# GrumpyZhou/patch2pix

Measured on NVIDIA H100. Metric: image-pairs/sec, higher is better.
Workload: dtype f16 tensor-core operands (mid: 3-pass hi/lo split on the risk band, 1-pass elsewhere, fine: 1-pass, correlation + NC conv: 3-pass), f32 accumulate

## Files before the change

### include/p2p_b200.h

```cpp
#ifndef P2P_B200_H_
#define P2P_B200_H_

#include <stdint.h>

#ifdef __cplusplus
extern "C" {
#endif

#define P2P_API __attribute__((visibility("default")))

typedef struct p2p_handle_s* p2p_handle_t;

typedef struct p2p_bn_s {
  const float* weight;
  const float* bias;
  const float* running_mean;
  const float* running_var;
} p2p_bn_t;

typedef struct p2p_regressor_weights_s {
  const float* conv0_weight;
  p2p_bn_t conv1_bn;
  const float* conv2_weight;
  p2p_bn_t conv3_bn;
  const float* fc0_weight;
  const float* fc0_bias;
  p2p_bn_t fc1_bn;
  const float* fc3_weight;
  const float* fc3_bias;
  p2p_bn_t fc4_bn;
  const float* fc6_weight;
  const float* fc6_bias;
  float bn_eps;
} p2p_regressor_weights_t;

P2P_API const char* p2p_last_error(void);
P2P_API int p2p_version(void);

P2P_API int p2p_create(int device, p2p_handle_t* out);
P2P_API int p2p_destroy(p2p_handle_t h);

P2P_API int p2p_set_ncn_weights(p2p_handle_t h, const float* w1, const float* b1, const float* w2, const float* b2);

P2P_API int p2p_set_regressor_weights(p2p_handle_t h, int which, const p2p_regressor_weights_t* w);

P2P_API int p2p_set_option(p2p_handle_t h, const char* key, int value);
P2P_API int p2p_get_option(p2p_handle_t h, const char* key, int* value);
P2P_API int p2p_launch_count(p2p_handle_t h, long long* count);

enum {
  P2P_PROF_L2NORM = 0, P2P_PROF_CORR = 1, P2P_PROF_MUTUAL = 2, P2P_PROF_NC = 3, P2P_PROF_PROPOSALS = 4,
  P2P_PROF_PREP = 5, P2P_PROF_GATHER_MID = 6, P2P_PROF_CONV1_MID = 7, P2P_PROF_CONV2_MID = 8, P2P_PROF_FC_MID = 9,
  P2P_PROF_GATHER_FINE = 10, P2P_PROF_CONV1_FINE = 11, P2P_PROF_CONV2_FINE = 12, P2P_PROF_FC_FINE = 13,
  P2P_PROF_GATHER_BAND = 14, P2P_PROF_CONV1_BAND = 15, P2P_PROF_CONV2_BAND = 16, P2P_PROF_FC_BAND = 17,
  P2P_PROF_FLAG = 18, P2P_PROF_KINDS = 19
};
P2P_API int p2p_profile_read(p2p_handle_t h, float* ms_by_kind, int* count_by_kind, int nkinds);

P2P_API int p2p_coarse(p2p_handle_t h, const float* feat1, const float* feat2, int c, int h1, int w1, int h2, int w2,
               int ksize, float* corr4d_out, uint8_t* delta_code_out, float* pooled_out, float* ncn_out,
               void* stream);

P2P_API int p2p_coarse_nhwc16(p2p_handle_t h, const void* feat1_nhwc16, const void* feat2_nhwc16, int c, int h1, int w1, int h2,
               int w2, int ksize, float* corr4d_out, uint8_t* delta_code_out, float* pooled_out, float* ncn_out,
               void* stream);

P2P_API int p2p_delta_unpack(p2p_handle_t h, const uint8_t* code, long long n, int ksize, int64_t* di, int64_t* dj,
                     int64_t* dk, int64_t* dl, void* stream);
P2P_API int p2p_delta_pack(p2p_handle_t h, const int64_t* di, const int64_t* dj, const int64_t* dk, const int64_t* dl,
                   long long n, int ksize, uint8_t* code, void* stream);

P2P_API int p2p_mutual_matching(p2p_handle_t h, const float* in, int nA, int nB, float* out, void* stream);
P2P_API int p2p_neigh_consensus(p2p_handle_t h, const float* in, int hA, int wA, int hB, int wB, float* out, void* stream);

P2P_API int p2p_proposals(p2p_handle_t h, const float* corr4d, const uint8_t* delta_code, int hA, int wA, int hB, int wB,
                  int ksize, int upsample, int center, int do_softmax, int64_t* matches_out, float* scores_out,
                  void* stream);

P2P_API int p2p_unique_rows(p2p_handle_t h, const int64_t* rows, int n, int mutual, const float* scores, float thres,
                    int32_t* ids_out, int32_t* count_out, void* stream);

P2P_API int p2p_select_anchor(p2p_handle_t h, const int64_t* rows, const float* scores, const int32_t* ids,
                      const int32_t* sel, int m, int panc, int pshift, int64_t* matches_out, float* scores_out,
                      int64_t* anchors_out, void* stream);

P2P_API int p2p_refine_prepare(p2p_handle_t h, const float* const* feats1, const float* const* feats2, int H1, int W1,
                       int H2, int W2, void* stream);
P2P_API int p2p_refine_prepare_nhwc16(p2p_handle_t h, const void* const* feats1, const void* const* feats2, int H1, int W1,
                       int H2, int W2, void* stream);
P2P_API int p2p_refine(p2p_handle_t h, int which, const void* matches_in, int is_float, int n, float* matches_out,
               float* probs_out, void* stream);

P2P_API int p2p_finalize_matches(p2p_handle_t h, const float* fine, const float* scores, const int64_t* coarse, int n,
                         float io_thres, const double* upscale4, double* packed_out, void* stream);

P2P_API int p2p_preprocess_image(p2p_handle_t h, const uint8_t* rgb_hwc, int ho, int wo, int ht, int wt, float* out_chw,
                         uint8_t* resized_hwc_out, void* stream);

P2P_API int p2p_find_model(p2p_handle_t h, int model, const double* rows, int row_stride, int n, const double* n_dev,
                   double px_th, double conf, int max_iters, unsigned long long seed, double* model_out, uint8_t* mask_out,
                   int32_t* n_inliers_out, void* stream);
P2P_API int p2p_sampson_distance(p2p_handle_t h, const double* rows, int row_stride, int n, const double* F,
                         double* dist_out, void* stream);
P2P_API int p2p_epipolar_histograms(p2p_handle_t h, const double* rows, int row_stride, int n, const double* n_dev,
                                    int coarse_col, const double* F, const uint8_t* mask, const double* edges,
                                    int n_edges, int32_t* counts_out, void* stream);
P2P_API int p2p_overlap_scores(p2p_handle_t h, const int64_t* point3D_ids, const int64_t* offsets,
                               const int64_t* offsets_host, int n_images, int words, uint32_t* bits_out,
                               int32_t* counts_out, double* scores_out, void* stream);
P2P_API int p2p_test_hypotheses(p2p_handle_t h, int model, const double* rows, int row_stride, int n, double px_th,
                        unsigned long long seed, int count, double* models_out, int32_t* counts_out, void* stream);
P2P_API int p2p_test_degeneracy(p2p_handle_t h, const double* rows, int row_stride, int n, double px_th,
                                unsigned long long seed, int count, int32_t* triplet_out, double* H_out, void* stream);

P2P_API int p2p_find_essential(p2p_handle_t h, const double* rows, int row_stride, int n, const double* n_dev,
                               const double* intr, double px_th, double conf, int max_iters, unsigned long long seed,
                               double* E_out, uint8_t* mask_out, int32_t* n_inliers_out, void* stream);
P2P_API int p2p_recover_pose(p2p_handle_t h, const double* rows, int row_stride, int n, const double* n_dev,
                             const double* intr, const double* E, const uint8_t* mask_in, double dist_th,
                             double* Rt_out, uint8_t* mask_out, int32_t* n_good_out, void* stream);
P2P_API int p2p_test_essential_hypotheses(p2p_handle_t h, const double* rows, int row_stride, int n, const double* intr,
                                          double px_th, unsigned long long seed, int count, double* models_out,
                                          int32_t* counts_out, void* stream);

P2P_API int p2p_find_model_batch(p2p_handle_t h, int model, const double* rows, int row_stride, const int64_t* offsets,
                                 const int64_t* offsets_host, int K, const double* n_dev, double px_th, double conf,
                                 int max_iters, unsigned long long seed, double* models_out, uint8_t* mask_out,
                                 int32_t* n_inliers_out, void* stream);
P2P_API int p2p_find_essential_batch(p2p_handle_t h, const double* rows, int row_stride, const int64_t* offsets,
                                     const int64_t* offsets_host, int K, const double* n_dev, const double* intr,
                                     double px_th, double conf, int max_iters, unsigned long long seed, double* E_out,
                                     uint8_t* mask_out, int32_t* n_inliers_out, void* stream);
P2P_API int p2p_recover_pose_batch(p2p_handle_t h, const double* rows, int row_stride, const int64_t* offsets,
                                   const int64_t* offsets_host, int K, const double* n_dev, const double* intr,
                                   const double* E, const uint8_t* mask_in, double dist_th, double* Rt_out,
                                   uint8_t* mask_out, int32_t* n_good_out, void* stream);
P2P_API int p2p_batch_chunk_pairs(p2p_handle_t h, int entry, int* pairs_out);

P2P_API int p2p_test_gemm(p2p_handle_t h, const float* a, const float* b, float* c, int M, int N, int K, int passes,
                  int seg_len, float in_scale, void* stream);

#ifdef __cplusplus
}
#endif
#endif
```

### patch2pix_b200/_lib.py

```python
import ctypes as C
import os

import torch

_HERE = os.path.dirname(os.path.abspath(__file__))
LIB_PATH = os.path.join(_HERE, 'libp2p_b200.so')
_lib = None


class BN(C.Structure):
    _fields_ = [('weight', C.c_void_p), ('bias', C.c_void_p), ('running_mean', C.c_void_p), ('running_var', C.c_void_p)]


class RegressorWeights(C.Structure):
    _fields_ = [('conv0_weight', C.c_void_p), ('conv1_bn', BN), ('conv2_weight', C.c_void_p), ('conv3_bn', BN),
                ('fc0_weight', C.c_void_p), ('fc0_bias', C.c_void_p), ('fc1_bn', BN),
                ('fc3_weight', C.c_void_p), ('fc3_bias', C.c_void_p), ('fc4_bn', BN),
                ('fc6_weight', C.c_void_p), ('fc6_bias', C.c_void_p), ('bn_eps', C.c_float)]


_P, _I, _LL, _F = C.c_void_p, C.c_int, C.c_longlong, C.c_float
_SIGNATURES = {
    'p2p_last_error': (C.c_char_p, []),
    'p2p_version': (_I, []),
    'p2p_create': (_I, [_I, C.POINTER(_P)]),
    'p2p_destroy': (_I, [_P]),
    'p2p_set_ncn_weights': (_I, [_P, _P, _P, _P, _P]),
    'p2p_set_regressor_weights': (_I, [_P, _I, C.POINTER(RegressorWeights)]),
    'p2p_set_option': (_I, [_P, C.c_char_p, _I]),
    'p2p_get_option': (_I, [_P, C.c_char_p, C.POINTER(_I)]),
    'p2p_launch_count': (_I, [_P, C.POINTER(_LL)]),
    'p2p_coarse': (_I, [_P, _P, _P, _I, _I, _I, _I, _I, _I, _P, _P, _P, _P, _P]),
    'p2p_coarse_nhwc16': (_I, [_P, _P, _P, _I, _I, _I, _I, _I, _I, _P, _P, _P, _P, _P]),
    'p2p_delta_unpack': (_I, [_P, _P, _LL, _I, _P, _P, _P, _P, _P]),
    'p2p_delta_pack': (_I, [_P, _P, _P, _P, _P, _LL, _I, _P, _P]),
    'p2p_mutual_matching': (_I, [_P, _P, _I, _I, _P, _P]),
    'p2p_neigh_consensus': (_I, [_P, _P, _I, _I, _I, _I, _P, _P]),
    'p2p_proposals': (_I, [_P, _P, _P, _I, _I, _I, _I, _I, _I, _I, _I, _P, _P, _P]),
    'p2p_unique_rows': (_I, [_P, _P, _I, _I, _P, _F, _P, _P, _P]),
    'p2p_select_anchor': (_I, [_P, _P, _P, _P, _P, _I, _I, _I, _P, _P, _P, _P]),
    'p2p_refine_prepare': (_I, [_P, C.POINTER(_P), C.POINTER(_P), _I, _I, _I, _I, _P]),
    'p2p_refine_prepare_nhwc16': (_I, [_P, C.POINTER(_P), C.POINTER(_P), _I, _I, _I, _I, _P]),
    'p2p_refine': (_I, [_P, _I, _P, _I, _I, _P, _P, _P]),
    'p2p_finalize_matches': (_I, [_P, _P, _P, _P, _I, _F, C.POINTER(C.c_double), _P, _P]),
    'p2p_preprocess_image': (_I, [_P, _P, _I, _I, _I, _I, _P, _P, _P]),
    'p2p_profile_read': (_I, [_P, C.POINTER(C.c_float), C.POINTER(_I), _I]),
    'p2p_test_gemm': (_I, [_P, _P, _P, _P, _I, _I, _I, _I, _I, _F, _P]),
    'p2p_find_model': (_I, [_P, _I, _P, _I, _I, _P, C.c_double, C.c_double, _I, C.c_ulonglong, _P, _P, _P, _P]),
    'p2p_sampson_distance': (_I, [_P, _P, _I, _I, _P, _P, _P]),
    'p2p_epipolar_histograms': (_I, [_P, _P, _I, _I, _P, _I, C.POINTER(C.c_double), _P, C.POINTER(C.c_double), _I, _P,
                                     _P]),
    'p2p_overlap_scores': (_I, [_P, _P, _P, C.POINTER(C.c_int64), _I, _I, _P, _P, _P, _P]),
    'p2p_test_hypotheses': (_I, [_P, _I, _P, _I, _I, C.c_double, C.c_ulonglong, _I, _P, _P, _P]),
    'p2p_test_degeneracy': (_I, [_P, _P, _I, _I, C.c_double, C.c_ulonglong, _I, _P, _P, _P]),
    'p2p_find_essential': (_I, [_P, _P, _I, _I, _P, _P, C.c_double, C.c_double, _I, C.c_ulonglong, _P, _P, _P, _P]),
    'p2p_recover_pose': (_I, [_P, _P, _I, _I, _P, _P, _P, _P, C.c_double, _P, _P, _P, _P]),
    'p2p_test_essential_hypotheses': (_I, [_P, _P, _I, _I, _P, C.c_double, C.c_ulonglong, _I, _P, _P, _P]),
    'p2p_find_model_batch': (_I, [_P, _I, _P, _I, _P, C.POINTER(C.c_int64), _I, _P, C.c_double, C.c_double, _I,
                                  C.c_ulonglong, _P, _P, _P, _P]),
    'p2p_find_essential_batch': (_I, [_P, _P, _I, _P, C.POINTER(C.c_int64), _I, _P, _P, C.c_double, C.c_double, _I,
                                      C.c_ulonglong, _P, _P, _P, _P]),
    'p2p_recover_pose_batch': (_I, [_P, _P, _I, _P, C.POINTER(C.c_int64), _I, _P, _P, _P, _P, C.c_double, _P, _P, _P,
                                    _P]),
    'p2p_batch_chunk_pairs': (_I, [_P, _I, C.POINTER(_I)]),
}
EXPORTED_SYMBOLS = tuple(_SIGNATURES)
PROF_KINDS = ('l2norm', 'corr', 'mutual', 'nc', 'proposals', 'prep', 'gather_mid', 'conv1_mid', 'conv2_mid', 'fc_mid',
              'gather_fine', 'conv1_fine', 'conv2_fine', 'fc_fine', 'gather_band', 'conv1_band', 'conv2_band', 'fc_band',
              'flag')


def load():
    global _lib
    if _lib is None:
        if not os.path.exists(LIB_PATH):
            raise RuntimeError(f'{LIB_PATH} not found: the CUDA extension is required (no CPU fallback). '
                               f'Build it with `python -m patch2pix_b200.build`.')
        lib = C.CDLL(LIB_PATH)
        for name, (res, args) in _SIGNATURES.items():
            fn = getattr(lib, name)
            fn.restype = res
            fn.argtypes = args
        _lib = lib
    return _lib


def check(rc):
    if rc != 0:
        msg = load().p2p_last_error()
        raise RuntimeError(f'libp2p_b200 error {rc}: {msg.decode() if msg else "?"}')


def ptr(t):
    return None if t is None else C.c_void_p(t.data_ptr())


def stream_ptr(device):
    return C.c_void_p(torch.cuda.current_stream(device).cuda_stream)


class Handle:

    def __init__(self, device):
        device = torch.device(device)
        if device.type != 'cuda':
            raise RuntimeError('patch2pix_b200 runs on CUDA (sm_90a) devices only; got device ' + str(device))
        self.device = torch.device('cuda', device.index if device.index is not None else torch.cuda.current_device())
        self.lib = load()
        h = C.c_void_p()
        check(self.lib.p2p_create(self.device.index, C.byref(h)))
        self.h = h
        for kv in filter(None, os.environ.get('P2P_OPTIONS', '').split(',')):
            k, _, v = kv.partition('=')
            self.set_option(k.strip(), int(v))

    def __del__(self):
        try:
            if getattr(self, 'h', None):
                self.lib.p2p_destroy(self.h)
                self.h = None
        except Exception:
            pass

    def set_option(self, key, value):
        check(self.lib.p2p_set_option(self.h, key.encode(), int(value)))

    def get_option(self, key):
        v = C.c_int()
        check(self.lib.p2p_get_option(self.h, key.encode(), C.byref(v)))
        return v.value

    def launch_count(self):
        v = C.c_longlong()
        check(self.lib.p2p_launch_count(self.h, C.byref(v)))
        return v.value

    def stream(self):
        return stream_ptr(self.device)

    def profile_read(self):
        n = len(PROF_KINDS)
        ms = (C.c_float * n)()
        cnt = (C.c_int * n)()
        check(self.lib.p2p_profile_read(self.h, ms, cnt, n))
        return {PROF_KINDS[i]: (ms[i], cnt[i]) for i in range(n)}


_default_handles = {}


def default_handle(device):
    device = torch.device(device)
    idx = device.index if device.index is not None else torch.cuda.current_device()
    if idx not in _default_handles:
        _default_handles[idx] = Handle(torch.device('cuda', idx))
    return _default_handles[idx]
```

### patch2pix_b200/csrc/api.cu

```cuda
#include <math.h>
#include <stdlib.h>

#include <algorithm>
#include <vector>

#include "../../include/p2p_b200.h"
#include "kernels.h"
#include "umma_gemm.h"

namespace p2p {

static thread_local std::string g_last_error;
void set_last_error(const std::string& msg) { g_last_error = msg; }
long long g_launch_count = 0;

int ensure_dyn_smem(const void* kernel, int bytes) {
  struct Key { const void* k; int dev; };
  static thread_local std::vector<std::pair<Key, int>> granted;
  int dev = 0;
  cudaGetDevice(&dev);
  for (auto& g : granted)
    if (g.first.k == kernel && g.first.dev == dev) {
      if (g.second >= bytes) return 0;
      if (cudaFuncSetAttribute(kernel, cudaFuncAttributeMaxDynamicSharedMemorySize, bytes) != cudaSuccess) {
        set_last_error(std::string("cudaFuncSetAttribute(MaxDynamicSharedMemorySize) failed: ") + cudaGetErrorString(cudaGetLastError()));
        return -2;
      }
      g.second = bytes;
      return 0;
    }
  if (cudaFuncSetAttribute(kernel, cudaFuncAttributeMaxDynamicSharedMemorySize, bytes) != cudaSuccess) {
    set_last_error(std::string("cudaFuncSetAttribute(MaxDynamicSharedMemorySize) failed: ") + cudaGetErrorString(cudaGetLastError()));
    return -2;
  }
  granted.push_back({Key{kernel, dev}, bytes});
  return 0;
}

int Arena::reserve(size_t bytes) {
  off = 0;
  if (bytes <= cap) return 0;
  if (base != nullptr) {
    cudaDeviceSynchronize();
    cudaFree(base);
    base = nullptr;
    cap = 0;
  }
  bytes = align_up(bytes + (bytes >> 3), 1 << 20);
  if (cudaMalloc(&base, bytes) != cudaSuccess) {
    cudaGetLastError();
    set_last_error("out of device memory reserving " + std::to_string(bytes >> 20) + " MiB of scratch");
    return -3;
  }
  cap = bytes;
  return 0;
}
void Arena::release() {
  if (base != nullptr) cudaFree(base);
  base = nullptr;
  cap = off = 0;
}

struct Regressor {
  bool set = false;
  __half *w1_hi = nullptr, *w1_lo = nullptr;
  __half *w2_hi = nullptr, *w2_lo = nullptr;
  float *scale1 = nullptr, *bias1 = nullptr, *scale2 = nullptr, *bias2 = nullptr;
  float y_scale = 1.f;
  FcWeights fc = {nullptr, nullptr, nullptr, nullptr, nullptr, nullptr};
  __half *f1_hi = nullptr, *f1_lo = nullptr, *f2_hi = nullptr, *f2_lo = nullptr;
  float *fa1 = nullptr, *fa2 = nullptr;
  KStep steps1[kConv1Steps];
  KStep steps2[kConv2Steps];
  KStep *d_steps1 = nullptr, *d_steps2 = nullptr;
  char* blob = nullptr;
};

}

using namespace p2p;

struct p2p_handle_s {
  int device = 0;
  int num_sms = 132;
  int opt_mid_passes = 3, opt_fine_passes = 1, opt_corr_passes = 3, opt_seg_len = 3, opt_gemm_impl = 0, opt_num_sms = 0;
  int opt_mid_band = 26;
  int opt_fc_impl = 1;
  int opt_fuse_gather = 3;
  int opt_share_windows = 1;
  const int* last_band_count = nullptr;
  int* share_rows = nullptr;
  bool last_mid_shared = false;
  unsigned long long* band_totals = nullptr;
  bool nc_set = false;
  float *nc_w1p = nullptr, *nc_b1p = nullptr, *nc_w2p = nullptr;
  float nc_b2 = 0.f;
  NcUmmaWeights ncw;
  void* dbg_nc[4] = {nullptr, nullptr, nullptr, nullptr};
  int opt_unique_impl = 1;
  int* uniq_rank = nullptr;
  int opt_nc_l2_mode = 0;
  int opt_nc_impl = 1;
  Regressor reg[2];
  Arena coarse, refine, feat, misc, uniq, pre, verify;
  std::vector<PreprocessCoefs> pre_coefs;
  PairFeatures pf[2];
  bool prepared = false;
  int opt_profile = 0;
  struct ProfEntry { cudaEvent_t a, b; int kind; };
  std::vector<ProfEntry> prof;
  std::vector<cudaEvent_t> event_pool;
};

namespace {

struct DeviceGuard {
  int prev = -1;
  bool ok = true;
  explicit DeviceGuard(int dev) {
    if (cudaGetDevice(&prev) != cudaSuccess) ok = false;
    if (ok && prev != dev && cudaSetDevice(dev) != cudaSuccess) ok = false;
  }
  ~DeviceGuard() {
    if (prev >= 0) cudaSetDevice(prev);
  }
};

#define P2P_ENTER(h)                                                  \
  P2P_REQUIRE((h) != nullptr, "null handle");                         \
  DeviceGuard _guard((h)->device);                                    \
  if (!_guard.ok) {                                                   \
    set_last_error("cannot select CUDA device of the handle");        \
    return -2;                                                        \
  }

float pow2_floor_scale(float maxabs, float target_hi) {
  if (!(maxabs > 0.f) || !isfinite(maxabs)) return 1.f;
  int e;
  frexpf(maxabs, &e);
  int et;
  frexpf(target_hi, &et);
  return ldexpf(1.f, et - 1 - e);
}

void split_half(float v, __half& hi, __half& lo) {
  hi = __float2half_rn(v);
  lo = __float2half_rn(v - __half2float(hi));
}

template <typename T>
T* carve(char*& p, size_t count) {
  T* r = reinterpret_cast<T*>(p);
  p += align_up(count * sizeof(T), 256);
  return r;
}

void fold_bn(const p2p_bn_t& bn, int n, float eps, std::vector<float>& g, std::vector<float>& b) {
  g.resize(n);
  b.resize(n);
  for (int i = 0; i < n; ++i) {
    g[i] = bn.weight[i] / sqrtf(bn.running_var[i] + eps);
    b[i] = bn.bias[i] - bn.running_mean[i] * g[i];
  }
}

int tap_plane(int t, int& start) {
  if (t == 0) { start = -1; return 0; }
  if (t == 1) { start = 0; return 1; }
  start = 0;
  return 0;
}

int pack_regressor(p2p_handle_s* h, Regressor& R, const p2p_regressor_weights_t& w) {
  const int K1 = kConv1Steps * 64, K2 = kConv2Steps * 64;
  std::vector<float> g1, b1, g2, b2, gf1, bf1, gf2, bf2;
  fold_bn(w.conv1_bn, 512, w.bn_eps, g1, b1);
  fold_bn(w.conv3_bn, 512, w.bn_eps, g2, b2);
  fold_bn(w.fc1_bn, 512, w.bn_eps, gf1, bf1);
  fold_bn(w.fc4_bn, 256, w.bn_eps, gf2, bf2);

  std::vector<__half> w1h((size_t)512 * K1), w1l((size_t)512 * K1), w2h((size_t)512 * K2), w2l((size_t)512 * K2);
  std::vector<float> sc1(512), sc2(512), bi1(b1), bi2(b2);
  float max_bound = 0.f;
  std::vector<float> sw1(512), sw2(512);
  for (int o = 0; o < 512; ++o) {
    const float* wo = w.conv0_weight + (size_t)o * 518 * 9;
    float m = 0.f;
    double tapn[9] = {0};
    for (int c = 0; c < 518; ++c)
      for (int t = 0; t < 9; ++t) {
        const float v = wo[c * 9 + t] * g1[o];
        m = fmaxf(m, fabsf(v));
        tapn[t] += (double)v * v;
      }
    float bound = fabsf(b1[o]);
    for (int t = 0; t < 9; ++t) bound += 1.41421357f * (float)sqrt(tapn[t]);
    max_bound = fmaxf(max_bound, bound);
    sw1[o] = pow2_floor_scale(m, 1024.f);
    sc1[o] = 1.f / (kActScale * sw1[o]);
    __half* dh = w1h.data() + (size_t)o * K1;
    __half* dl = w1l.data() + (size_t)o * K1;
    for (int s = 0; s < 72; ++s) {
      const int tap = s / 8, chunk = s % 8;
      for (int kk = 0; kk < 64; ++kk) {
        const int c512 = chunk * 64 + kk;
        const int orig = (c512 / 256) * 259 + 3 + (c512 % 256);
        split_half(wo[orig * 9 + tap] * g1[o] * sw1[o], dh[s * 64 + kk], dl[s * 64 + kk]);
      }
    }
    for (int kk = 0; kk < 64; ++kk) {
      float v = 0.f;
      if (kk < 54) {
        const int tap = kk / 6, r = kk % 6;
        const int orig = (r / 3) * 259 + (r % 3);
        v = wo[orig * 9 + tap] * g1[o] * sw1[o];
      }
      split_half(v, dh[72 * 64 + kk], dl[72 * 64 + kk]);
    }
  }
  R.y_scale = pow2_floor_scale(max_bound, 32768.f);
  for (int o = 0; o < 512; ++o) {
    const float* wo = w.conv2_weight + (size_t)o * 512 * 9;
    float m = 0.f;
    for (int i = 0; i < 512 * 9; ++i) m = fmaxf(m, fabsf(wo[i] * g2[o]));
    sw2[o] = pow2_floor_scale(m, 1024.f);
    sc2[o] = 1.f / (R.y_scale * sw2[o]);
    __half* dh = w2h.data() + (size_t)o * K2;
    __half* dl = w2l.data() + (size_t)o * K2;
    for (int s = 0; s < 72; ++s) {
      const int tap = s / 8, chunk = s % 8;
      for (int kk = 0; kk < 64; ++kk)
        split_half(wo[(chunk * 64 + kk) * 9 + tap] * g2[o] * sw2[o], dh[s * 64 + kk], dl[s * 64 + kk]);
    }
  }
  for (int s = 0; s < 72; ++s) {
    const int tap = s / 8, chunk = s % 8, ty = tap / 3, tx = tap % 3;
    int sx, sy;
    const int px = tap_plane(tx, sx), py = tap_plane(ty, sy);
    R.steps1[s] = KStep{(short)(chunk * 64), (signed char)sx, (signed char)sy, (signed char)(py * 2 + px), 0, 0, s * 64};
    R.steps2[s] = KStep{(short)(chunk * 64), (signed char)(tx - 1), (signed char)(ty - 1), 0, 0, 0, s * 64};
  }
  R.steps1[72] = KStep{0, 0, 0, 0, 1, 0, 72 * 64};
  std::vector<float> f1t((size_t)512 * 512), f1b(512), f2t((size_t)512 * 256), f2b(256), f3t(256 * 5), f3b(5);
  for (int o = 0; o < 512; ++o) {
    for (int k = 0; k < 512; ++k) f1t[(size_t)k * 512 + o] = w.fc0_weight[(size_t)o * 512 + k] * gf1[o];
    f1b[o] = w.fc0_bias[o] * gf1[o] + bf1[o];
  }
  for (int o = 0; o < 256; ++o) {
    for (int k = 0; k < 512; ++k) f2t[(size_t)k * 256 + o] = w.fc3_weight[(size_t)o * 512 + k] * gf2[o];
    f2b[o] = w.fc3_bias[o] * gf2[o] + bf2[o];
  }
  for (int o = 0; o < 5; ++o) {
    for (int k = 0; k < 256; ++k) f3t[k * 5 + o] = w.fc6_weight[o * 256 + k];
    f3b[o] = w.fc6_bias[o];
  }
  std::vector<__half> f1h((size_t)512 * 512), f1l((size_t)512 * 512), f2h((size_t)256 * 512), f2l((size_t)256 * 512);
  std::vector<float> fa1(512), fa2(256);
  for (int o = 0; o < 512; ++o) {
    float m = 0.f;
    for (int k = 0; k < 512; ++k) m = fmaxf(m, fabsf(w.fc0_weight[(size_t)o * 512 + k] * gf1[o]));
    const float sw = pow2_floor_scale(m, 1024.f);
    fa1[o] = 1.f / (kFcActScale * sw);
    for (int k = 0; k < 512; ++k)
      split_half(w.fc0_weight[(size_t)o * 512 + k] * gf1[o] * sw, f1h[(size_t)o * 512 + k], f1l[(size_t)o * 512 + k]);
  }
  for (int o = 0; o < 256; ++o) {
    float m = 0.f;
    for (int k = 0; k < 512; ++k) m = fmaxf(m, fabsf(w.fc3_weight[(size_t)o * 512 + k] * gf2[o]));
    const float sw = pow2_floor_scale(m, 1024.f);
    fa2[o] = 1.f / (kFcActScale * sw);
    for (int k = 0; k < 512; ++k)
      split_half(w.fc3_weight[(size_t)o * 512 + k] * gf2[o] * sw, f2h[(size_t)o * 512 + k], f2l[(size_t)o * 512 + k]);
  }
  const size_t total = 2 * 1024 * 1024 + 65536 + 4 * align_up((size_t)512 * K1 * 2, 256) + 8 * 4096 + align_up(f1t.size() * 4, 256) +
                       align_up(f2t.size() * 4, 256) + 8 * 8192 + 65536;
  if (R.blob == nullptr) {
    if (cudaMalloc(&R.blob, total) != cudaSuccess) {
      cudaGetLastError();
      set_last_error("out of device memory packing regressor weights");
      return -3;
    }
  }
  char* p = R.blob;
  R.w1_hi = carve<__half>(p, (size_t)512 * K1);
  R.w1_lo = carve<__half>(p, (size_t)512 * K1);
  R.w2_hi = carve<__half>(p, (size_t)512 * K2);
  R.w2_lo = carve<__half>(p, (size_t)512 * K2);
  R.scale1 = carve<float>(p, 512);
  R.bias1 = carve<float>(p, 512);
  R.scale2 = carve<float>(p, 512);
  R.bias2 = carve<float>(p, 512);
  R.fc.w1t = carve<float>(p, f1t.size());
  R.fc.b1 = carve<float>(p, 512);
  R.fc.w2t = carve<float>(p, f2t.size());
  R.fc.b2 = carve<float>(p, 256);
  R.fc.w3t = carve<float>(p, f3t.size());
  R.fc.b3 = carve<float>(p, 5);
  R.d_steps1 = carve<KStep>(p, kConv1Steps);
  R.d_steps2 = carve<KStep>(p, kConv2Steps);
  R.f1_hi = carve<__half>(p, f1h.size());
  R.f1_lo = carve<__half>(p, f1l.size());
  R.f2_hi = carve<__half>(p, f2h.size());
  R.f2_lo = carve<__half>(p, f2l.size());
  R.fa1 = carve<float>(p, 512);
  R.fa2 = carve<float>(p, 256);
#define UP(dst, src, bytes) P2P_CUDA_OK(cudaMemcpy(dst, src, bytes, cudaMemcpyHostToDevice))
  UP(R.w1_hi, w1h.data(), w1h.size() * 2);
  UP(R.w1_lo, w1l.data(), w1l.size() * 2);
  UP(R.w2_hi, w2h.data(), w2h.size() * 2);
  UP(R.w2_lo, w2l.data(), w2l.size() * 2);
  UP(R.scale1, sc1.data(), 2048);
  UP(R.bias1, bi1.data(), 2048);
  UP(R.scale2, sc2.data(), 2048);
  UP(R.bias2, bi2.data(), 2048);
  UP(R.fc.w1t, f1t.data(), f1t.size() * 4);
  UP(R.fc.b1, f1b.data(), 2048);
  UP(R.fc.w2t, f2t.data(), f2t.size() * 4);
  UP(R.fc.b2, f2b.data(), 1024);
  UP(R.fc.w3t, f3t.data(), f3t.size() * 4);
  UP(R.fc.b3, f3b.data(), 20);
  UP(R.d_steps1, R.steps1, sizeof(R.steps1));
  UP(R.d_steps2, R.steps2, sizeof(R.steps2));
  UP(R.f1_hi, f1h.data(), f1h.size() * 2);
  UP(R.f1_lo, f1l.data(), f1l.size() * 2);
  UP(R.f2_hi, f2h.data(), f2h.size() * 2);
  UP(R.f2_lo, f2l.data(), f2l.size() * 2);
  UP(R.fa1, fa1.data(), 2048);
  UP(R.fa2, fa2.data(), 1024);
#undef UP
  R.set = true;
  (void)h;
  return 0;
}

int sms(const p2p_handle_s* h) { return h->opt_num_sms > 0 ? h->opt_num_sms : h->num_sms; }

struct ProfScope {
  p2p_handle_s* h;
  cudaStream_t st;
  cudaEvent_t a = nullptr, b = nullptr;
  int kind;
  static cudaEvent_t get(p2p_handle_s* h) {
    if (!h->event_pool.empty()) {
      cudaEvent_t e = h->event_pool.back();
      h->event_pool.pop_back();
      return e;
    }
    cudaEvent_t e = nullptr;
    cudaEventCreate(&e);
    return e;
  }
  ProfScope(p2p_handle_s* h_, int kind_, cudaStream_t st_) : h(h_), st(st_), kind(kind_) {
    if (h->opt_profile) {
      a = get(h);
      b = get(h);
      cudaEventRecord(a, st);
    }
  }
  ~ProfScope() {
    if (a != nullptr) {
      cudaEventRecord(b, st);
      h->prof.push_back({a, b, kind});
    }
  }
};

}

extern "C" {

const char* p2p_last_error(void) { return g_last_error.c_str(); }
int p2p_version(void) { return 100; }

int p2p_create(int device, p2p_handle_t* out) {
  P2P_REQUIRE(out != nullptr, "out is null");
  int ndev = 0;
  P2P_CUDA_OK(cudaGetDeviceCount(&ndev));
  P2P_REQUIRE(device >= 0 && device < ndev, "device index out of range");
  cudaDeviceProp prop;
  P2P_CUDA_OK(cudaGetDeviceProperties(&prop, device));
  if (prop.major != 9 || prop.minor != 0) {
    set_last_error(std::string("libp2p_b200 targets sm_90a (H100) only; device is sm_") + std::to_string(prop.major) +
                   std::to_string(prop.minor));
    return -2;
  }
  p2p_handle_s* h = new p2p_handle_s();
  h->device = device;
  h->num_sms = prop.multiProcessorCount;
  {
    DeviceGuard g(device);
    if (cudaMalloc(&h->band_totals, 2 * sizeof(unsigned long long)) == cudaSuccess)
      cudaMemset(h->band_totals, 0, 2 * sizeof(unsigned long long));
    else
      h->band_totals = nullptr;
    if (cudaMalloc(&h->share_rows, sizeof(int)) == cudaSuccess)
      cudaMemset(h->share_rows, 0, sizeof(int));
    else
      h->share_rows = nullptr;
  }
  *out = h;
  return 0;
}

int p2p_destroy(p2p_handle_t h) {
  if (h == nullptr) return 0;
  DeviceGuard g(h->device);
  cudaDeviceSynchronize();
  h->coarse.release();
  h->refine.release();
  h->feat.release();
  h->misc.release();
  h->uniq.release();
  h->pre.release();
  h->verify.release();
  for (auto& c : h->pre_coefs)
    if (c.d) cudaFree(c.d);
  for (auto& e : h->prof) { cudaEventDestroy(e.a); cudaEventDestroy(e.b); }
  for (auto e : h->event_pool) cudaEventDestroy(e);
  if (h->nc_w1p) cudaFree(h->nc_w1p);
  if (h->ncw.blob) cudaFree(h->ncw.blob);
  if (h->band_totals) cudaFree(h->band_totals);
  if (h->share_rows) cudaFree(h->share_rows);
  if (h->uniq_rank) cudaFree(h->uniq_rank);
  for (int i = 0; i < 2; ++i)
    if (h->reg[i].blob) cudaFree(h->reg[i].blob);
  delete h;
  return 0;
}

int p2p_set_ncn_weights(p2p_handle_t h, const float* w1, const float* b1, const float* w2, const float* b2) {
  P2P_ENTER(h);
  P2P_REQUIRE(w1 && b1 && w2 && b2, "null weight pointer");
  std::vector<float> w1p(81 * 32), b1p(32), w2p(81 * 32);
  for (int a = 0; a < 3; ++a)
    for (int b = 0; b < 3; ++b)
      for (int d = 0; d < 3; ++d)
        for (int e = 0; e < 3; ++e) {
          const int tap = ((a * 3 + b) * 3 + d) * 3 + e;
          for (int c = 0; c < 16; ++c) {
            w1p[tap * 32 + c] = w1[((a * 16 + c) * 1 + 0) * 27 + (b * 3 + d) * 3 + e];
            w1p[tap * 32 + 16 + c] = w1[((d * 16 + c) * 1 + 0) * 27 + (e * 3 + a) * 3 + b];
            w2p[tap * 32 + c] = w2[((a * 1 + 0) * 16 + c) * 27 + (b * 3 + d) * 3 + e];
            w2p[tap * 32 + 16 + c] = w2[((d * 1 + 0) * 16 + c) * 27 + (e * 3 + a) * 3 + b];
          }
        }
  for (int c = 0; c < 16; ++c) b1p[c] = b1p[16 + c] = b1[c];
  if (h->nc_w1p == nullptr) P2P_CUDA_OK(cudaMalloc(&h->nc_w1p, sizeof(float) * (81 * 32 * 2 + 32)));
  h->nc_w2p = h->nc_w1p + 81 * 32;
  h->nc_b1p = h->nc_w2p + 81 * 32;
  P2P_CUDA_OK(cudaMemcpy(h->nc_w1p, w1p.data(), sizeof(float) * 81 * 32, cudaMemcpyHostToDevice));
  P2P_CUDA_OK(cudaMemcpy(h->nc_w2p, w2p.data(), sizeof(float) * 81 * 32, cudaMemcpyHostToDevice));
  P2P_CUDA_OK(cudaMemcpy(h->nc_b1p, b1p.data(), sizeof(float) * 32, cudaMemcpyHostToDevice));
  h->nc_b2 = b2[0];
  {
    int rc = nc_umma_pack(w1p.data(), b1p.data(), w2p.data(), h->ncw);
    if (rc) return rc;
  }
  h->nc_set = true;
  return 0;
}

int p2p_set_regressor_weights(p2p_handle_t h, int which, const p2p_regressor_weights_t* w) {
  P2P_ENTER(h);
  P2P_REQUIRE(which == 0 || which == 1, "which must be 0 (mid) or 1 (fine)");
  P2P_REQUIRE(w != nullptr && w->conv0_weight && w->conv2_weight && w->fc0_weight && w->fc3_weight && w->fc6_weight,
              "null weight pointer");
  return pack_regressor(h, h->reg[which], *w);
}

static int* option_slot(p2p_handle_t h, const char* key) {
  if (!strcmp(key, "mid_passes")) return &h->opt_mid_passes;
  if (!strcmp(key, "fine_passes")) return &h->opt_fine_passes;
  if (!strcmp(key, "corr_passes")) return &h->opt_corr_passes;
  if (!strcmp(key, "seg_len")) return &h->opt_seg_len;
  if (!strcmp(key, "gemm_impl")) return &h->opt_gemm_impl;
  if (!strcmp(key, "num_sms")) return &h->opt_num_sms;
  if (!strcmp(key, "profile")) return &h->opt_profile;
  if (!strcmp(key, "mid_band")) return &h->opt_mid_band;
  if (!strcmp(key, "fuse_gather")) return &h->opt_fuse_gather;
  if (!strcmp(key, "share_windows")) return &h->opt_share_windows;
  if (!strcmp(key, "fc_impl")) return &h->opt_fc_impl;
  if (!strcmp(key, "nc_impl")) return &h->opt_nc_impl;
  if (!strcmp(key, "nc_l2_mode")) return &h->opt_nc_l2_mode;
  if (!strcmp(key, "unique_impl")) return &h->opt_unique_impl;
  return nullptr;
}

int p2p_set_option(p2p_handle_t h, const char* key, int value) {
  P2P_REQUIRE(h != nullptr && key != nullptr, "null argument");
  int* s = option_slot(h, key);
  P2P_REQUIRE(s != nullptr, std::string("unknown option ") + key);
  if (s == &h->opt_mid_passes || s == &h->opt_fine_passes) P2P_REQUIRE(value == 1 || value == 3, "passes must be 1 or 3");
  if (s == &h->opt_corr_passes) P2P_REQUIRE(value == 0 || value == 1 || value == 3, "corr_passes must be 0, 1 or 3");
  if (s == &h->opt_share_windows) P2P_REQUIRE(value == 0 || value == 1, "share_windows must be 0 or 1");
  P2P_REQUIRE(value >= 0, "option values are non-negative");
  *s = value;
  return 0;
}

int p2p_get_option(p2p_handle_t h, const char* key, int* value) {
  P2P_REQUIRE(h != nullptr && key != nullptr && value != nullptr, "null argument");
  if (!strcmp(key, "band_rows")) {
    *value = 0;
    if (h->last_band_count != nullptr) {
      DeviceGuard g(h->device);
      P2P_CUDA_OK(cudaDeviceSynchronize());
      P2P_CUDA_OK(cudaMemcpy(value, h->last_band_count, sizeof(int), cudaMemcpyDeviceToHost));
    }
    return 0;
  }
  if (!strcmp(key, "shared_rows")) {
    *value = 0;
    if (h->last_mid_shared && h->share_rows != nullptr) {
      DeviceGuard g(h->device);
      P2P_CUDA_OK(cudaDeviceSynchronize());
      P2P_CUDA_OK(cudaMemcpy(value, h->share_rows, sizeof(int), cudaMemcpyDeviceToHost));
    }
    return 0;
  }
  if (!strcmp(key, "band_rows_total") || !strcmp(key, "band_calls_rows_total")) {
    *value = 0;
    if (h->band_totals != nullptr) {
      DeviceGuard g(h->device);
      P2P_CUDA_OK(cudaDeviceSynchronize());
      unsigned long long t[2] = {0, 0};
      P2P_CUDA_OK(cudaMemcpy(t, h->band_totals, sizeof(t), cudaMemcpyDeviceToHost));
      const bool rows = !strcmp(key, "band_calls_rows_total");
      *value = (int)(rows ? t[1] : t[0]);
      if (rows) P2P_CUDA_OK(cudaMemset(h->band_totals, 0, sizeof(t)));
    }
    return 0;
  }
  int* s = option_slot(h, key);
  P2P_REQUIRE(s != nullptr, std::string("unknown option ") + key);
  *value = *s;
  return 0;
}

int p2p_launch_count(p2p_handle_t h, long long* count) {
  P2P_REQUIRE(h != nullptr && count != nullptr, "null argument");
  *count = g_launch_count;
  return 0;
}

int p2p_profile_read(p2p_handle_t h, float* ms_by_kind, int* count_by_kind, int nkinds) {
  P2P_ENTER(h);
  P2P_REQUIRE(ms_by_kind && count_by_kind && nkinds >= P2P_PROF_KINDS, "need room for P2P_PROF_KINDS entries");
  for (int i = 0; i < nkinds; ++i) {
    ms_by_kind[i] = 0.f;
    count_by_kind[i] = 0;
  }
  for (auto& e : h->prof) {
    P2P_CUDA_OK(cudaEventSynchronize(e.b));
    float ms = 0.f;
    P2P_CUDA_OK(cudaEventElapsedTime(&ms, e.a, e.b));
    ms_by_kind[e.kind] += ms;
    count_by_kind[e.kind] += 1;
    h->event_pool.push_back(e.a);
    h->event_pool.push_back(e.b);
  }
  h->prof.clear();
  return 0;
}

static int corr_umma(p2p_handle_s* h, const __half* a_hi, const __half* a_lo, const __half* b_hi, const __half* b_lo,
                     int C, int n1, int n2, int n1pad, int n2pad, int ksize, float* out, uint8_t* code,
                     cudaStream_t st) {
  UmmaGemmParams p;
  memset(&p, 0, sizeof(p));
  const uint64_t ad[5] = {(uint64_t)C, 1, 1, 1, (uint64_t)n1pad};
  const uint64_t as[4] = {(uint64_t)C * 2, (uint64_t)C * 2, (uint64_t)C * 2, (uint64_t)C * 2};
  const uint32_t ab[5] = {64, 1, 1, 1, 128};
  const uint64_t bd[2] = {(uint64_t)C, (uint64_t)n2pad};
  const uint64_t bs[1] = {(uint64_t)C * 2};
  const uint32_t bb[2] = {64, 128};
  int rc;
  if ((rc = make_tmap_fp16(&p.a_main_hi, a_hi, 5, ad, as, ab))) return rc;
  if ((rc = make_tmap_fp16(&p.b_hi, b_hi, 2, bd, bs, bb))) return rc;
  if (h->opt_corr_passes == 3) {
    if ((rc = make_tmap_fp16(&p.a_main_lo, a_lo, 5, ad, as, ab))) return rc;
    if ((rc = make_tmap_fp16(&p.b_lo, b_lo, 2, bd, bs, bb))) return rc;
  }
  p.a_rgb_hi = p.a_main_hi;
  p.a_rgb_lo = p.a_main_hi;
  p.nsteps = C / 64;
  for (int s = 0; s < p.nsteps; ++s) p.steps[s] = KStep{(short)(s * 64), 0, 0, 0, 0, 0, s * 64};
  p.m_tiles = n1pad / 128;
  p.n_tiles = n2pad / 256;
  p.a_units_per_tile = 128;
  p.seg_len = h->opt_seg_len > 0 ? 1 : 0;
  p.epi.c = out;
  p.epi.alpha = 1.f / (kActScale * kActScale);
  if (ksize == 2) {
    p.epi.code = code;
    p.epi.np1 = n1 / 4;
    p.epi.np2 = n2 / 4;
    return launch_umma_gemm(p, EPI_CORR, h->opt_corr_passes, sms(h), st);
  }
  p.epi.ldc = n2;
  p.epi.m_rows = n1;
  p.epi.n_cols = n2;
  return launch_umma_gemm(p, EPI_PLAIN, h->opt_corr_passes, sms(h), st);
}

static int coarse_impl(p2p_handle_t h, const float* feat1, const float* feat2, int fmt, int c, int h1, int w1, int h2, int w2,
                       int ksize, float* corr4d_out, uint8_t* delta_code_out, float* pooled_out, float* ncn_out,
                       void* stream) {
  P2P_ENTER(h);
  cudaStream_t st = reinterpret_cast<cudaStream_t>(stream);
  P2P_REQUIRE(h->nc_set, "p2p_set_ncn_weights has not been called");
  P2P_REQUIRE(feat1 && feat2 && corr4d_out, "null tensor pointer");
  P2P_REQUIRE(ksize == 1 || ksize == 2, "ksize must be 1 or 2");
  P2P_REQUIRE(c > 0 && h1 > 0 && w1 > 0 && h2 > 0 && w2 > 0, "empty feature map");
  if (ksize == 2) {
    P2P_REQUIRE(h1 % 2 == 0 && w1 % 2 == 0 && h2 % 2 == 0 && w2 % 2 == 0, "ksize 2 needs even feature sizes");
    P2P_REQUIRE(delta_code_out != nullptr, "delta_code_out is required for ksize 2");
  }
  const int n1 = h1 * w1, n2 = h2 * w2;
  const int hA = h1 / ksize, wA = w1 / ksize, hB = h2 / ksize, wB = w2 / ksize;
  const int nA = hA * wA, nB = hB * wB;
  const size_t V = (size_t)nA * nB;
  const bool tc = h->opt_corr_passes > 0;
  if (tc) P2P_REQUIRE(c % 64 == 0 && c / 64 <= kMaxKSteps, "tensor-core correlation needs C % 64 == 0");
  P2P_REQUIRE(fmt == 0 || tc, "channels-last fp16 features need the tensor-core correlation (corr_passes 1 or 3)");
  const int n1pad = (int)align_up(n1, 128), n2pad = (int)align_up(n2, 256);
  size_t need = 4 * V * 4 + nc_umma_scratch_bytes(V) + nc_umma_xp_bytes(hA, wA, hB, wB) + (size_t)(nA + nB) * 8 + (1 << 16);
  need += tc ? (size_t)(n1pad + n2pad) * c * 4 : (size_t)(n1 + n2) * c * 4;
  int rc = h->coarse.reserve(need);
  if (rc) return rc;
  Arena& A = h->coarse;
  float* pooled = pooled_out ? pooled_out : (float*)A.take(V * 4);
  float* m1 = (float*)A.take(V * 4);
  float* nc = ncn_out ? ncn_out : (float*)A.take(V * 4);
  float* hidden = (float*)A.take(V * 128);
  float* partial = (float*)A.take(18 * V * 4);
  uint32_t* xp = (uint32_t*)A.take(nc_umma_xp_bytes(hA, wA, hB, wB));
  float* rowmax = (float*)A.take((size_t)nA * 4);
  unsigned int* colmax = (unsigned int*)A.take((size_t)nB * 4 + 16);
  unsigned int* xmax = colmax != nullptr ? colmax + nB : nullptr;
  if (tc) {
    __half* a_hi = (__half*)A.take((size_t)n1pad * c * 2);
    __half* a_lo = (__half*)A.take((size_t)n1pad * c * 2);
    __half* b_hi = (__half*)A.take((size_t)n2pad * c * 2);
    __half* b_lo = (__half*)A.take((size_t)n2pad * c * 2);
    P2P_REQUIRE(a_hi && a_lo && b_hi && b_lo && hidden && colmax, "scratch carve failed");
    const bool lo = h->opt_corr_passes == 3;
    {
      ProfScope ps(h, P2P_PROF_L2NORM, st);
      if (fmt == 1)
        rc = launch_l2norm_perm_kmajor_pair_nhwc16(reinterpret_cast<const __half*>(feat1), reinterpret_cast<const __half*>(feat2),
                                                   a_hi, lo ? a_lo : nullptr, b_hi, lo ? b_lo : nullptr, c, h1, w1, h2, w2, ksize, st);
      else
        rc = launch_l2norm_perm_kmajor_pair(feat1, feat2, a_hi, lo ? a_lo : nullptr, b_hi, lo ? b_lo : nullptr, c, h1, w1, h2,
                                            w2, ksize, st);
      if (rc) return rc;
    }
    ProfScope ps(h, P2P_PROF_CORR, st);
    if ((rc = corr_umma(h, a_hi, a_lo, b_hi, b_lo, c, n1, n2, n1pad, n2pad, ksize, pooled, delta_code_out, st)))
      return rc;
  } else {
    float* fa = (float*)A.take((size_t)n1 * c * 4);
    float* fb = (float*)A.take((size_t)n2 * c * 4);
    P2P_REQUIRE(fa && fb && hidden && colmax, "scratch carve failed");
    {
      ProfScope ps(h, P2P_PROF_L2NORM, st);
      if ((rc = launch_l2norm_perm(feat1, fa, c, h1, w1, ksize, st))) return rc;
      if ((rc = launch_l2norm_perm(feat2, fb, c, h2, w2, ksize, st))) return rc;
    }
    ProfScope ps(h, P2P_PROF_CORR, st);
    if ((rc = launch_corr_pool_simt(fa, fb, c, n1, n2, ksize, pooled, delta_code_out, st))) return rc;
  }
  P2P_REQUIRE(partial != nullptr && xmax != nullptr && xp != nullptr, "scratch carve failed");
  if (h->opt_nc_impl == 1) {
    {
      ProfScope ps(h, P2P_PROF_MUTUAL, st);
      if ((rc = launch_mutual_matching(pooled, nA, nB, rowmax, colmax, m1, xmax, st))) return rc;
    }
    {
      ProfScope ps(h, P2P_PROF_NC, st);
      if ((rc = launch_neigh_consensus_umma(m1, hA, wA, hB, wB, h->ncw, h->nc_b1p, h->nc_b2, xmax, xp, (__half*)hidden, partial,
                                            nc, rowmax, colmax, h->opt_nc_l2_mode, sms(h), st)))
        return rc;
    }
    ProfScope ps(h, P2P_PROF_MUTUAL, st);
    return launch_mutual_apply(nc, nA, nB, rowmax, colmax, corr4d_out, nullptr, st);
  }
  {
    ProfScope ps(h, P2P_PROF_MUTUAL, st);
    if ((rc = launch_mutual_matching(pooled, nA, nB, rowmax, colmax, m1, nullptr, st))) return rc;
  }
  {
    ProfScope ps(h, P2P_PROF_NC, st);
    if ((rc = launch_neigh_consensus(m1, hA, wA, hB, wB, h->nc_w1p, h->nc_b1p, h->nc_w2p, h->nc_b2, hidden, nc, st)))
      return rc;
  }
  ProfScope ps(h, P2P_PROF_MUTUAL, st);
  if ((rc = launch_mutual_matching(nc, nA, nB, rowmax, colmax, corr4d_out, nullptr, st))) return rc;
  return 0;
}

int p2p_coarse(p2p_handle_t h, const float* feat1, const float* feat2, int c, int h1, int w1, int h2, int w2,
               int ksize, float* corr4d_out, uint8_t* delta_code_out, float* pooled_out, float* ncn_out,
               void* stream) {
  return coarse_impl(h, feat1, feat2, 0, c, h1, w1, h2, w2, ksize, corr4d_out, delta_code_out, pooled_out, ncn_out, stream);
}

int p2p_coarse_nhwc16(p2p_handle_t h, const void* feat1_nhwc16, const void* feat2_nhwc16, int c, int h1, int w1, int h2, int w2,
                      int ksize, float* corr4d_out, uint8_t* delta_code_out, float* pooled_out, float* ncn_out,
                      void* stream) {
  return coarse_impl(h, reinterpret_cast<const float*>(feat1_nhwc16), reinterpret_cast<const float*>(feat2_nhwc16), 1, c, h1, w1,
                     h2, w2, ksize, corr4d_out, delta_code_out, pooled_out, ncn_out, stream);
}

int p2p_delta_unpack(p2p_handle_t h, const uint8_t* code, long long n, int ksize, int64_t* di, int64_t* dj,
                     int64_t* dk, int64_t* dl, void* stream) {
  P2P_ENTER(h);
  P2P_REQUIRE(code && di && dj && dk && dl && n >= 0 && ksize >= 1 && ksize <= 3, "bad argument");
  if (n == 0) return 0;
  return launch_delta_unpack(code, (size_t)n, ksize, (long long*)di, (long long*)dj, (long long*)dk, (long long*)dl,
                             reinterpret_cast<cudaStream_t>(stream));
}

int p2p_delta_pack(p2p_handle_t h, const int64_t* di, const int64_t* dj, const int64_t* dk, const int64_t* dl,
                   long long n, int ksize, uint8_t* code, void* stream) {
  P2P_ENTER(h);
  P2P_REQUIRE(code && di && dj && dk && dl && n >= 0 && ksize >= 1 && ksize <= 3, "bad argument");
  if (n == 0) return 0;
  return launch_delta_pack((const long long*)di, (const long long*)dj, (const long long*)dk, (const long long*)dl,
                           (size_t)n, ksize, code, reinterpret_cast<cudaStream_t>(stream));
}

int p2p_mutual_matching(p2p_handle_t h, const float* in, int nA, int nB, float* out, void* stream) {
  P2P_ENTER(h);
  P2P_REQUIRE(in && out && nA > 0 && nB > 0, "bad argument");
  int rc = h->misc.reserve((size_t)(nA + nB) * 4 + 4096);
  if (rc) return rc;
  float* rowmax = (float*)h->misc.take((size_t)nA * 4);
  unsigned int* colmax = (unsigned int*)h->misc.take((size_t)nB * 4);
  return launch_mutual_matching(in, nA, nB, rowmax, colmax, out, nullptr, reinterpret_cast<cudaStream_t>(stream));
}

int p2p_neigh_consensus(p2p_handle_t h, const float* in, int hA, int wA, int hB, int wB, float* out, void* stream) {
  P2P_ENTER(h);
  P2P_REQUIRE(h->nc_set, "p2p_set_ncn_weights has not been called");
  P2P_REQUIRE(in && out && hA > 0 && wA > 0 && hB > 0 && wB > 0, "bad argument");
  const size_t V = (size_t)hA * wA * hB * wB;
  int rc = h->misc.reserve(nc_umma_scratch_bytes(V) + nc_umma_xp_bytes(hA, wA, hB, wB) + 8192);
  if (rc) return rc;
  float* hidden = (float*)h->misc.take(V * 128);
  float* partial = (float*)h->misc.take(18 * V * 4);
  uint32_t* xp = (uint32_t*)h->misc.take(nc_umma_xp_bytes(hA, wA, hB, wB));
  unsigned int* xmax = (unsigned int*)h->misc.take(16);
  P2P_REQUIRE(hidden && partial && xmax && xp, "scratch carve failed");
  h->dbg_nc[0] = hidden; h->dbg_nc[1] = partial; h->dbg_nc[2] = xp; h->dbg_nc[3] = xmax;
  cudaStream_t st = reinterpret_cast<cudaStream_t>(stream);
  if (h->opt_nc_impl == 1) {
    if ((rc = launch_absmax(in, V, xmax, st))) return rc;
    return launch_neigh_consensus_umma(in, hA, wA, hB, wB, h->ncw, h->nc_b1p, h->nc_b2, xmax, xp, (__half*)hidden, partial, out,
                                       nullptr, nullptr, h->opt_nc_l2_mode, sms(h), st);
  }
  return launch_neigh_consensus(in, hA, wA, hB, wB, h->nc_w1p, h->nc_b1p, h->nc_w2p, h->nc_b2, hidden, out, st);
}

P2P_API int p2p_debug_nc_scratch(p2p_handle_t h, int which, void* host_dst, size_t bytes) {
  P2P_ENTER(h);
  P2P_REQUIRE(which >= 0 && which < 4 && host_dst != nullptr && h->dbg_nc[which] != nullptr, "bad argument");
  P2P_CUDA_OK(cudaDeviceSynchronize());
  P2P_CUDA_OK(cudaMemcpy(host_dst, h->dbg_nc[which], bytes, cudaMemcpyDeviceToHost));
  return 0;
}

int p2p_proposals(p2p_handle_t h, const float* corr4d, const uint8_t* delta_code, int hA, int wA, int hB, int wB,
                  int ksize, int upsample, int center, int do_softmax, int64_t* matches_out, float* scores_out,
                  void* stream) {
  P2P_ENTER(h);
  P2P_REQUIRE(corr4d && matches_out && scores_out, "null tensor pointer");
  P2P_REQUIRE(hA > 0 && wA > 0 && hB > 0 && wB > 0 && ksize >= 1 && ksize <= 3 && upsample > 0, "bad dims");
  P2P_REQUIRE(ksize == 1 || delta_code != nullptr, "delta_code is required for ksize > 1");
  ProfScope ps(h, P2P_PROF_PROPOSALS, reinterpret_cast<cudaStream_t>(stream));
  return launch_proposals(corr4d, ksize > 1 ? delta_code : nullptr, hA, wA, hB, wB, ksize, upsample, center,
                          do_softmax, (long long*)matches_out, scores_out, reinterpret_cast<cudaStream_t>(stream));
}

int p2p_unique_rows(p2p_handle_t h, const int64_t* rows, int n, int mutual, const float* scores, float thres,
                    int32_t* ids_out, int32_t* count_out, void* stream) {
  P2P_ENTER(h);
  P2P_REQUIRE(rows && ids_out && count_out, "null tensor pointer");
  unsigned char* scratch = nullptr;
  const size_t sb = unique_rows_scratch_bytes(n);
  if (sb > 0) {
    int rc = h->uniq.reserve(sb + 4096);
    if (rc) return rc;
    scratch = (unsigned char*)h->uniq.take(sb);
  }
  if (h->uniq_rank == nullptr && h->opt_unique_impl == 1) {
    P2P_CUDA_OK(cudaMalloc(&h->uniq_rank, unique_rank_scratch_bytes()));
    P2P_CUDA_OK(cudaMemset(h->uniq_rank, 0, unique_rank_scratch_bytes()));
  }
  ProfScope ps(h, P2P_PROF_PROPOSALS, reinterpret_cast<cudaStream_t>(stream));
  return launch_unique_rows((const long long*)rows, n, mutual, scores, thres, ids_out, count_out, scratch,
                            h->opt_unique_impl == 1 ? h->uniq_rank : nullptr, reinterpret_cast<cudaStream_t>(stream));
}

int p2p_select_anchor(p2p_handle_t h, const int64_t* rows, const float* scores, const int32_t* ids, const int32_t* sel,
                      int m, int panc, int pshift, int64_t* matches_out, float* scores_out, int64_t* anchors_out,
                      void* stream) {
  P2P_ENTER(h);
  P2P_REQUIRE(m >= 0 && rows != nullptr, "bad argument");
  P2P_REQUIRE(panc == 1 || panc == 8, "panc must be 1 or 8 (networks/patch2pix.py:377-402)");
  P2P_REQUIRE(scores_out == nullptr || scores != nullptr, "scores_out needs scores");
  P2P_REQUIRE(panc == 1 || anchors_out != nullptr, "anchors_out is required for panc 8");
  ProfScope ps(h, P2P_PROF_PROPOSALS, reinterpret_cast<cudaStream_t>(stream));
  return launch_select_anchor((const long long*)rows, scores, ids, sel, m, panc, pshift, (long long*)matches_out,
                              scores_out, (long long*)anchors_out, reinterpret_cast<cudaStream_t>(stream));
}

static int refine_prepare_impl(p2p_handle_t h, const float* const* feats1, const float* const* feats2, int fmt, int H1, int W1,
                               int H2, int W2, void* stream) {
  P2P_ENTER(h);
  cudaStream_t st = reinterpret_cast<cudaStream_t>(stream);
  P2P_REQUIRE(feats1 && feats2, "null feature list");
  for (int l = 0; l < 4; ++l) P2P_REQUIRE(feats1[l] && feats2[l], "null feature level");
  P2P_REQUIRE(H1 >= 8 && W1 >= 8 && H2 >= 8 && W2 >= 8 && H1 % 8 == 0 && W1 % 8 == 0 && H2 % 8 == 0 && W2 % 8 == 0,
              "image sizes must be positive multiples of 8");
  const int Hs[2] = {H1, H2}, Ws[2] = {W1, W2};
  size_t need = 1 << 16;
  for (int s = 0; s < 2; ++s) {
    const size_t px = (size_t)Hs[s] * Ws[s];
    need += (px / 4 * 64 + px / 16 * 64 + px / 64 * 128) * 6 + (px + px / 4 + px / 16 + px / 64) * 4 + 32768;
  }
  const bool want_map = h->opt_fuse_gather == 3;
  if (want_map)
    for (int s = 0; s < 2; ++s) need += (size_t)(Hs[s] + 2 * kMapPad) * (Ws[s] + 2 * kMapPad) * (512 + 8) + 4096;
  int rc = h->feat.reserve(need);
  if (rc) return rc;
  const int chans[3] = {64, 64, 128};
  for (int s = 0; s < 2; ++s) {
    PairFeatures& pf = h->pf[s];
    for (int l = 0; l < 4; ++l) {
      const int ds = 1 << l;
      pf.nsq[l] = (float*)h->feat.take((size_t)(Hs[s] / ds) * (Ws[s] / ds) * 4);
      P2P_REQUIRE(pf.nsq[l] != nullptr, "scratch carve failed");
    }
    for (int l = 0; l < 3; ++l) {
      const int ds = 2 << l;
      pf.nhwc[l] = (float*)h->feat.take((size_t)(Hs[s] / ds) * (Ws[s] / ds) * chans[l] * 4);
      pf.nhwc16[l] = (__half*)h->feat.take((size_t)(Hs[s] / ds) * (Ws[s] / ds) * chans[l] * 2);
      P2P_REQUIRE(pf.nhwc[l] != nullptr && pf.nhwc16[l] != nullptr, "scratch carve failed");
    }
    pf.wmap = pf.rgbn = nullptr;
    if (want_map) {
      const size_t pxp = (size_t)(Hs[s] + 2 * kMapPad) * (Ws[s] + 2 * kMapPad);
      pf.wmap = (__half*)h->feat.take(pxp * 512);
      pf.rgbn = (__half*)h->feat.take(pxp * 8);
      P2P_REQUIRE(pf.wmap != nullptr && pf.rgbn != nullptr, "scratch carve failed");
    }
  }
  {
    ProfScope ps(h, P2P_PROF_PREP, st);
    if ((rc = launch_feature_prep_pair(feats1, feats2, Hs, Ws, h->pf, fmt, st))) return rc;
    if (want_map && (rc = launch_window_map(h->pf, st))) return rc;
  }
  h->prepared = true;
  return 0;
}

int p2p_refine_prepare(p2p_handle_t h, const float* const* feats1, const float* const* feats2, int H1, int W1,
                       int H2, int W2, void* stream) {
  return refine_prepare_impl(h, feats1, feats2, 0, H1, W1, H2, W2, stream);
}

int p2p_refine_prepare_nhwc16(p2p_handle_t h, const void* const* feats1, const void* const* feats2, int H1, int W1,
                              int H2, int W2, void* stream) {
  return refine_prepare_impl(h, reinterpret_cast<const float* const*>(feats1), reinterpret_cast<const float* const*>(feats2), 1,
                             H1, W1, H2, W2, stream);
}

namespace {

struct RefineBuffers {
  __half *p_hi, *p_lo, *r_hi, *r_lo, *y_hi, *y_lo;
  __half *q_hi, *q_lo, *h1_hi, *h1_lo, *h2_hi, *h2_lo;
  float *pooled, *raw;
  int *rowmap, *d_count;
  int *sh_prefix, *sh_cont, *sh_unsh, *sh_cnt;
  float* part;
  __half* r_unsh;
  int npad;
};

int image_steps(const Regressor& R, int si, KStep* out) {
  int k = 0;
  for (int s = 0; s < 72; ++s)
    if ((R.steps1[s].c0 >> 6) >> 2 == si) out[k++] = R.steps1[s];
  return k;
}

int run_regressor(p2p_handle_s* h, Regressor& R, int which, int passes, const RefineBuffers& B, const void* matches_in,
                  int is_float, int n, const int* rowmap, const int* d_count, float* matches_out, float* probs_out,
                  float* raw_out, cudaStream_t st) {
  const bool lo = passes == 3;
  const int kb = rowmap != nullptr ? P2P_PROF_GATHER_BAND : (which == 0 ? P2P_PROF_GATHER_MID : P2P_PROF_GATHER_FINE);
  int rc;
  const bool mapped = passes == 1 && rowmap == nullptr && h->opt_fuse_gather == 3 && h->opt_gemm_impl == 0;
  const bool fused = passes == 1 && rowmap == nullptr && h->opt_fuse_gather && h->opt_gemm_impl == 0 && !mapped;
  if (mapped) P2P_REQUIRE(h->pf[0].wmap != nullptr && h->pf[1].wmap != nullptr,
                          "fuse_gather = 3 needs p2p_refine_prepare to have run with the same option");
  const bool share = mapped && which == 0 && h->opt_share_windows;
  if (which == 0 && rowmap == nullptr) h->last_mid_shared = share;
  if (!fused && !mapped) {
    ProfScope ps(h, kb, st);
    if ((rc = launch_patch_gather(h->pf[0], h->pf[1], matches_in, is_float, n, B.p_hi, lo ? B.p_lo : nullptr, B.r_hi,
                                  lo ? B.r_lo : nullptr, rowmap, d_count, st)))
      return rc;
  }
  if (h->opt_gemm_impl == 1) {
    P2P_REQUIRE(rowmap == nullptr, "the CUDA-core checker GEMM does not support row subsets");
    GemmOperands g1 = {B.p_hi, B.p_lo, B.r_hi, B.r_lo, R.w1_hi, R.w1_lo, 4, kConv1Steps * 64, n, passes, R.d_steps1, kConv1Steps};
    ConvEpilogue e1 = {R.scale1, R.bias1, 0, R.y_scale, B.y_hi, lo ? B.y_lo : nullptr, nullptr};
    {
      ProfScope ps(h, kb + 1, st);
      if ((rc = launch_conv_gemm_simt(g1, e1, st))) return rc;
    }
    ProfScope ps(h, kb + 2, st);
    GemmOperands g2 = {B.y_hi, B.y_lo, nullptr, nullptr, R.w2_hi, R.w2_lo, 1, kConv2Steps * 64, n, passes, R.d_steps2, kConv2Steps};
    ConvEpilogue e2 = {R.scale2, R.bias2, 1, 1.f, nullptr, nullptr, B.pooled};
    if ((rc = launch_conv_gemm_simt(g2, e2, st))) return rc;
  } else {
    UmmaGemmParams p;
    memset(&p, 0, sizeof(p));
    const uint32_t abox[5] = {64, 8, 8, 1, 2};
    const uint32_t bbox[2] = {64, 128};
    const uint64_t npad = (uint64_t)B.npad;
    {
      const uint64_t ad[5] = {512, 8, 8, 4, npad};
      const uint64_t as[4] = {1024, 8192, 65536, 262144};
      const uint64_t rd[5] = {64, 8, 8, 1, npad};
      const uint64_t rs[4] = {128, 1024, 8192, 8192};
      const uint64_t bd[2] = {(uint64_t)kConv1Steps * 64, 512};
      const uint64_t bs[1] = {(uint64_t)kConv1Steps * 64 * 2};
      if ((rc = make_tmap_fp16(&p.a_main_hi, B.p_hi, 5, ad, as, abox))) return rc;
      if ((rc = make_tmap_fp16(&p.a_rgb_hi, B.r_hi, 5, rd, rs, abox))) return rc;
      if ((rc = make_tmap_fp16(&p.b_hi, R.w1_hi, 2, bd, bs, bbox))) return rc;
      if ((rc = make_tmap_fp16(&p.a_main_lo, lo ? B.p_lo : B.p_hi, 5, ad, as, abox))) return rc;
      if ((rc = make_tmap_fp16(&p.a_rgb_lo, lo ? B.r_lo : B.r_hi, 5, rd, rs, abox))) return rc;
      if ((rc = make_tmap_fp16(&p.b_lo, R.w1_lo, 2, bd, bs, bbox))) return rc;
      p.nsteps = kConv1Steps;
      memcpy(p.steps, R.steps1, sizeof(R.steps1));
      p.m_tiles = (n + 1) / 2;
      p.n_tiles = 2;
      p.a_units_per_tile = 2;
      p.seg_len = lo ? h->opt_seg_len : 0;
      p.d_units = d_count;
      p.epi.scale = R.scale1;
      p.epi.bias = R.bias1;
      p.epi.y_scale = R.y_scale;
      p.epi.y_hi = B.y_hi;
      p.epi.y_lo = lo ? B.y_lo : nullptr;
      p.epi.pooled = B.pooled;
      p.epi.n_patches = n;
      if (fused) {
        for (int s2 = 0; s2 < 2; ++s2) {
          p.fg.img[s2] = h->pf[s2].img;
          for (int l = 0; l < 3; ++l) p.fg.nhwc16[s2][l] = h->pf[s2].nhwc16[l];
          for (int l = 0; l < 4; ++l) p.fg.nsq[s2][l] = h->pf[s2].nsq[l];
          p.fg.H[s2] = h->pf[s2].H;
          p.fg.W[s2] = h->pf[s2].W;
        }
        p.fg.matches = matches_in;
        p.fg.is_float = is_float;
      }
      if (mapped) {
        for (int s2 = 0; s2 < 2; ++s2) {
          const uint64_t Wp = (uint64_t)h->pf[s2].W + 2 * kMapPad, Hp = (uint64_t)h->pf[s2].H + 2 * kMapPad;
          const uint64_t md[3] = {256, Wp, Hp};
          const uint64_t ms[2] = {512, Wp * 512};
          const uint32_t mb[3] = {64, 16, 16};
          const uint32_t me[3] = {1, 2, 2};
          if ((rc = make_tmap_fp16(&p.wm.map[s2], h->pf[s2].wmap, 3, md, ms, mb, me))) return rc;
          p.wm.rgbn[s2] = h->pf[s2].rgbn;
          p.wm.H[s2] = h->pf[s2].H;
          p.wm.W[s2] = h->pf[s2].W;
        }
        p.wm.matches = matches_in;
        p.wm.is_float = is_float;
        ProfScope ps(h, kb, st);
        if (share) {
          P2P_REQUIRE(B.part != nullptr && B.r_unsh != nullptr, "share_windows: buffers not carved");
          if ((rc = launch_window_share_classify(p.wm, n, B.sh_prefix, B.sh_cont, B.sh_unsh, B.sh_cnt, h->share_rows, st)))
            return rc;
          if ((rc = launch_window_rgb(p.wm, n, B.npad, B.r_hi, st, B.sh_cont, B.sh_cnt + 3))) return rc;
          if ((rc = launch_window_rgb(p.wm, n, B.npad, B.r_unsh, st, B.sh_unsh, B.sh_cnt + 6))) return rc;
        } else if ((rc = launch_window_rgb(p.wm, n, B.npad, B.r_hi, st))) {
          return rc;
        }
      }
      ProfScope ps(h, kb + 1, st);
      const int amode = mapped ? AMODE_WINDOW : (fused ? AMODE_GATHER : AMODE_TMA);
      if (share) {
        float* part = B.part;
        KStep img[2][36];
        image_steps(R, 0, img[0]);
        image_steps(R, 1, img[1]);
        UmmaGemmParams q = p;
        memcpy(q.steps, img[1], sizeof(img[1]));
        memcpy(q.steps + 36, img[0], sizeof(img[0]));
        q.nsteps = 36;
        q.m_tiles = (n / 4 + 3) / 2;
        q.d_units = B.sh_cnt;
        q.ws = WindowShare{B.sh_prefix, B.sh_cnt + 1, 36, part, nullptr};
        if ((rc = launch_umma_gemm(q, EPI_CONV1, passes, sms(h), st, amode))) return rc;
        memcpy(q.steps, img[0], sizeof(img[0]));
        q.steps[36] = R.steps1[72];
        memcpy(q.steps + 37, img[1], sizeof(img[1]));
        q.steps[73] = R.steps1[72];
        q.nsteps = 37;
        q.m_tiles = (n + 1) / 2;
        q.d_units = B.sh_cnt + 3;
        q.ws = WindowShare{B.sh_cont, B.sh_cnt + 4, 37, nullptr, part};
        if ((rc = launch_umma_gemm(q, EPI_CONV1, passes, sms(h), st, amode))) return rc;
        q = p;
        if ((rc = make_tmap_fp16(&q.a_rgb_hi, B.r_unsh, 5, rd, rs, abox))) return rc;
        q.d_units = B.sh_cnt + 6;
        q.ws = WindowShare{B.sh_unsh, nullptr, 0, nullptr, nullptr};
        if ((rc = launch_umma_gemm(q, EPI_CONV1, passes, sms(h), st, amode))) return rc;
      } else if ((rc = launch_umma_gemm(p, EPI_CONV1, passes, sms(h), st, amode))) {
        return rc;
      }
    }
    {
      const uint64_t ad[5] = {512, 8, 8, 1, npad};
      const uint64_t as[4] = {1024, 8192, 65536, 65536};
      const uint64_t bd[2] = {(uint64_t)kConv2Steps * 64, 512};
      const uint64_t bs[1] = {(uint64_t)kConv2Steps * 64 * 2};
      if ((rc = make_tmap_fp16(&p.a_main_hi, B.y_hi, 5, ad, as, abox))) return rc;
      if ((rc = make_tmap_fp16(&p.a_main_lo, lo ? B.y_lo : B.y_hi, 5, ad, as, abox))) return rc;
      if ((rc = make_tmap_fp16(&p.b_hi, R.w2_hi, 2, bd, bs, bbox))) return rc;
      if ((rc = make_tmap_fp16(&p.b_lo, R.w2_lo, 2, bd, bs, bbox))) return rc;
      p.a_rgb_hi = p.a_main_hi;
      p.a_rgb_lo = p.a_main_lo;
      p.nsteps = kConv2Steps;
      memcpy(p.steps, R.steps2, sizeof(R.steps2));
      p.epi.scale = R.scale2;
      p.epi.bias = R.bias2;
      p.epi.pooled = B.pooled;
      ProfScope ps(h, kb + 2, st);
      if ((rc = launch_umma_gemm(p, EPI_CONV2, passes, sms(h), st))) return rc;
    }
  }
  ProfScope ps(h, kb + 3, st);
  if (h->opt_fc_impl == 0 || h->opt_gemm_impl == 1)
    return launch_fc_parse(B.pooled, R.fc, matches_in, is_float, n, h->pf[0].W, h->pf[0].H, h->pf[1].W, h->pf[1].H,
                           matches_out, probs_out, raw_out, rowmap, d_count, st);
  if ((rc = launch_pooled_split(B.pooled, n, B.q_hi, B.q_lo, d_count, st))) return rc;
  const uint64_t m128 = align_up(n, 128);
  const uint32_t abx[5] = {64, 1, 1, 1, 128};
  const uint32_t bbx[2] = {64, 128};
  for (int layer = 0; layer < 2; ++layer) {
    UmmaGemmParams p;
    memset(&p, 0, sizeof(p));
    const int nout = layer == 0 ? 512 : 256;
    const uint64_t ad[5] = {512, 1, 1, 1, m128};
    const uint64_t as[4] = {1024, 1024, 1024, 1024};
    const uint64_t bd[2] = {512, (uint64_t)nout};
    const uint64_t bs[1] = {1024};
    const __half* a_hi = layer == 0 ? B.q_hi : B.h1_hi;
    const __half* a_lo = layer == 0 ? B.q_lo : B.h1_lo;
    if ((rc = make_tmap_fp16(&p.a_main_hi, a_hi, 5, ad, as, abx))) return rc;
    if ((rc = make_tmap_fp16(&p.a_main_lo, a_lo, 5, ad, as, abx))) return rc;
    if ((rc = make_tmap_fp16(&p.b_hi, layer == 0 ? R.f1_hi : R.f2_hi, 2, bd, bs, bbx))) return rc;
    if ((rc = make_tmap_fp16(&p.b_lo, layer == 0 ? R.f1_lo : R.f2_lo, 2, bd, bs, bbx))) return rc;
    p.a_rgb_hi = p.a_main_hi;
    p.a_rgb_lo = p.a_main_lo;
    p.nsteps = 8;
    for (int s2 = 0; s2 < 8; ++s2) p.steps[s2] = KStep{(short)(s2 * 64), 0, 0, 0, 0, 0, s2 * 64};
    p.m_tiles = (int)(m128 / 128);
    p.n_tiles = nout / 256;
    p.a_units_per_tile = 128;
    p.seg_len = 2;
    p.d_units = d_count;
    p.epi.scale = layer == 0 ? R.fa1 : R.fa2;
    p.epi.bias = layer == 0 ? R.fc.b1 : R.fc.b2;
    p.epi.y_scale = kFcActScale;
    p.epi.y_hi = layer == 0 ? B.h1_hi : B.h2_hi;
    p.epi.y_lo = layer == 0 ? B.h1_lo : B.h2_lo;
    p.epi.ldc = nout;
    p.epi.n_patches = n;
    if ((rc = launch_umma_gemm(p, EPI_FC, 3, sms(h), st))) return rc;
  }
  return launch_fc3_parse(B.h2_hi, B.h2_lo, R.fc.w3t, R.fc.b3, matches_in, is_float, n, h->pf[0].W, h->pf[0].H,
                          h->pf[1].W, h->pf[1].H, matches_out, probs_out, raw_out, rowmap, d_count, st);
}

}

int p2p_refine(p2p_handle_t h, int which, const void* matches_in, int is_float, int n, float* matches_out,
               float* probs_out, void* stream) {
  P2P_ENTER(h);
  cudaStream_t st = reinterpret_cast<cudaStream_t>(stream);
  P2P_REQUIRE(which == 0 || which == 1, "which must be 0 (mid) or 1 (fine)");
  P2P_REQUIRE(h->reg[which].set, "p2p_set_regressor_weights has not been called for this regressor");
  P2P_REQUIRE(h->prepared, "p2p_refine_prepare has not been called");
  P2P_REQUIRE(n >= 0, "negative match count");
  if (n == 0) return 0;
  P2P_REQUIRE(matches_in && matches_out && probs_out, "null tensor pointer");
  Regressor& R = h->reg[which];
  const int passes = which == 0 ? h->opt_mid_passes : h->opt_fine_passes;
  const bool band = which == 0 && passes == 3 && h->opt_mid_band > 0 && h->opt_gemm_impl == 0;
  const int npad = (int)align_up(n, 2);
  const size_t pbytes = (size_t)npad * kPatchPos * kMainCh * 2, rbytes = (size_t)npad * 4096 * 2,
               ybytes = (size_t)npad * 64 * 512 * 2, qbytes = (size_t)npad * 512 * 4;
  const size_t n128 = align_up(n, 128);
  const size_t shbytes = ((size_t)n * 2 + n / 4 + 2 + 8) * 4;
  const bool share_bufs = which == 0 && h->opt_share_windows;
  const size_t partbytes = share_bufs ? ((size_t)n / 4 + 2) * 64 * 512 * 4 : 0, runshbytes = share_bufs ? rbytes : 0;
  int rc = h->refine.reserve(2 * (pbytes + rbytes + ybytes) + qbytes + (size_t)n * 24 + n128 * (512 + 512 + 256) * 4 +
                             shbytes + partbytes + runshbytes + (1 << 16));
  if (rc) return rc;
  Arena& A = h->refine;
  RefineBuffers B;
  B.npad = npad;
  B.p_hi = (__half*)A.take(pbytes);
  B.p_lo = (__half*)A.take(pbytes);
  B.r_hi = (__half*)A.take(rbytes);
  B.r_lo = (__half*)A.take(rbytes);
  B.y_hi = (__half*)A.take(ybytes);
  B.y_lo = (__half*)A.take(ybytes);
  B.pooled = (float*)A.take(qbytes);
  B.q_hi = (__half*)A.take(n128 * 512 * 2);
  B.q_lo = (__half*)A.take(n128 * 512 * 2);
  B.h1_hi = (__half*)A.take(n128 * 512 * 2);
  B.h1_lo = (__half*)A.take(n128 * 512 * 2);
  B.h2_hi = (__half*)A.take(n128 * 256 * 2);
  B.h2_lo = (__half*)A.take(n128 * 256 * 2);
  B.raw = (float*)A.take((size_t)n * 5 * 4);
  B.rowmap = (int*)A.take((size_t)n * 4 + 16);
  B.sh_cnt = (int*)A.take(shbytes);
  B.part = share_bufs ? (float*)A.take(partbytes) : nullptr;
  B.r_unsh = share_bufs ? (__half*)A.take(runshbytes) : nullptr;
  P2P_REQUIRE(B.p_hi && B.p_lo && B.r_hi && B.r_lo && B.y_hi && B.y_lo && B.pooled && B.raw && B.rowmap && B.q_hi &&
                  B.q_lo && B.h1_hi && B.h1_lo && B.h2_hi && B.h2_lo && B.sh_cnt &&
                  (!share_bufs || (B.part && B.r_unsh)),
              "scratch carve failed");
  B.sh_prefix = B.sh_cnt + 8;
  B.sh_cont = B.sh_prefix + n / 4 + 2;
  B.sh_unsh = B.sh_cont + n;
  B.d_count = B.rowmap + n;
  if (which == 0) h->last_band_count = band ? B.d_count : nullptr;
  if (!band)
    return run_regressor(h, R, which, passes, B, matches_in, is_float, n, nullptr, nullptr, matches_out, probs_out,
                         nullptr, st);
  if ((rc = run_regressor(h, R, which, 1, B, matches_in, is_float, n, nullptr, nullptr, matches_out, probs_out, B.raw,
                          st)))
    return rc;
  {
    ProfScope ps(h, P2P_PROF_FLAG, st);
    if ((rc = launch_flag_risky(matches_in, is_float, B.raw, n, h->opt_mid_band * 1e-3f, 0.02f, h->pf[0].W, h->pf[0].H,
                                h->pf[1].W, h->pf[1].H, B.rowmap, B.d_count, h->band_totals, st)))
      return rc;
  }
  return run_regressor(h, R, which, 3, B, matches_in, is_float, n, B.rowmap, B.d_count, matches_out, probs_out,
                       nullptr, st);
}

int p2p_finalize_matches(p2p_handle_t h, const float* fine, const float* scores, const int64_t* coarse, int n, float io_thres,
                         const double* upscale4, double* packed_out, void* stream) {
  P2P_ENTER(h);
  P2P_REQUIRE(scores && coarse && upscale4 && packed_out && n >= 0, "bad argument");
  return launch_finalize_matches(fine, scores, (const long long*)coarse, n, io_thres, upscale4, packed_out,
                                 reinterpret_cast<cudaStream_t>(stream));
}

int p2p_preprocess_image(p2p_handle_t h, const uint8_t* rgb_hwc, int ho, int wo, int ht, int wt, float* out_chw,
                         uint8_t* resized_hwc_out, void* stream) {
  P2P_ENTER(h);
  P2P_REQUIRE(rgb_hwc && out_chw && ho > 0 && wo > 0 && ht > 0 && wt > 0, "bad argument");
  P2P_REQUIRE((long long)ho * wo < (1ll << 28) && (long long)ht * wt < (1ll << 28), "image too large");
  const PreprocessCoefs* C = nullptr;
  for (const auto& c : h->pre_coefs)
    if (c.ho == ho && c.wo == wo && c.ht == ht && c.wt == wt) C = &c;
  if (C == nullptr) {
    if (h->pre_coefs.size() >= 32) {
      P2P_CUDA_OK(cudaDeviceSynchronize());
      if (h->pre_coefs.front().d) cudaFree(h->pre_coefs.front().d);
      h->pre_coefs.erase(h->pre_coefs.begin());
    }
    PreprocessCoefs c;
    int rc = preprocess_build_coefs(ho, wo, ht, wt, c);
    if (rc) return rc;
    h->pre_coefs.push_back(c);
    C = &h->pre_coefs.back();
  }
  int rc = h->pre.reserve((size_t)ho * wt * 3 + 4096);
  if (rc) return rc;
  uint8_t* tmp = (uint8_t*)h->pre.take((size_t)ho * wt * 3);
  P2P_REQUIRE(tmp != nullptr, "scratch carve failed");
  const float mean[3] = {0.485f, 0.456f, 0.406f}, stdv[3] = {0.229f, 0.224f, 0.225f};
  return launch_preprocess(rgb_hwc, *C, mean, stdv, out_chw, resized_hwc_out, tmp, reinterpret_cast<cudaStream_t>(stream));
}

int p2p_find_model(p2p_handle_t h, int model, const double* rows, int row_stride, int n, const double* n_dev, double px_th,
                   double conf, int max_iters, unsigned long long seed, double* model_out, uint8_t* mask_out,
                   int32_t* n_inliers_out, void* stream) {
  P2P_ENTER(h);
  P2P_REQUIRE(model >= 0 && model <= 2, "model must be 0 (F), 1 (H) or 2 (F with the DEGENSAC degeneracy check)");
  P2P_REQUIRE(model_out && mask_out && n_inliers_out && (rows || n == 0), "null tensor pointer");
  P2P_REQUIRE(n >= 0 && n <= (1 << 26) && row_stride >= 4, "bad row count or stride");
  P2P_REQUIRE(px_th > 0.0 && isfinite(px_th), "px_th must be positive");
  P2P_REQUIRE(conf > 0.0 && conf < 1.0, "conf must lie in (0, 1)");
  P2P_REQUIRE(max_iters > 0 && max_iters <= (1 << 24), "max_iters must lie in [1, 2^24]");
  int rc = h->verify.reserve(verify_scratch_bytes(1, n, true) + 4096);
  if (rc) return rc;
  void* scratch = h->verify.take(verify_scratch_bytes(1, n, true));
  return launch_find_model(model, single_pair(rows, row_stride, n, n_dev), px_th, conf, max_iters, seed, scratch,
                           model_out, mask_out, n_inliers_out, reinterpret_cast<cudaStream_t>(stream));
}

static int check_batch(const double* rows, int row_stride, const int64_t* offsets, const int64_t* offsets_host, int K) {
  P2P_REQUIRE(K >= 0, "K must be non-negative");
  P2P_REQUIRE(row_stride >= 4, "row_stride must be at least 4");
  if (K == 0) return 0;
  P2P_REQUIRE(offsets && offsets_host, "null offsets pointer");
  P2P_REQUIRE(offsets_host[0] >= 0, "offsets must be non-negative");
  for (int k = 0; k < K; ++k) {
    const int64_t len = offsets_host[k + 1] - offsets_host[k];
    P2P_REQUIRE(len >= 0, "offsets must be non-decreasing");
    P2P_REQUIRE(len <= (1 << 26), "a pair has more than 2^26 rows");
  }
  P2P_REQUIRE(offsets_host[K] - offsets_host[0] < ((int64_t)1 << 31), "a batch must have fewer than 2^31 rows");
  P2P_REQUIRE(rows || offsets_host[K] == offsets_host[0], "null rows pointer");
  return 0;
}

static PairBatch batch_chunk(const double* rows, int row_stride, const int64_t* offsets, const int64_t* offsets_host,
                             const double* n_dev, int k0, int pairs) {
  return PairBatch{rows, row_stride, reinterpret_cast<const long long*>(offsets) + k0, 0,
                   n_dev ? n_dev + k0 : nullptr, (long long)offsets_host[k0],
                   (long long)(offsets_host[k0 + pairs] - offsets_host[k0]), pairs};
}

static size_t batch_scratch(const int64_t* offsets_host, int K, int chunk, size_t (*bytes)(int, long long)) {
  size_t need = 0;
  for (int k0 = 0; k0 < K; k0 += chunk) {
    const int pairs = std::min(chunk, K - k0);
    need = std::max(need, bytes(pairs, (long long)(offsets_host[k0 + pairs] - offsets_host[k0])));
  }
  return need;
}

int p2p_batch_chunk_pairs(p2p_handle_t h, int entry, int* pairs_out) {
  P2P_ENTER(h);
  P2P_REQUIRE(pairs_out != nullptr, "null pointer");
  P2P_REQUIRE(entry >= 0 && entry <= 2, "entry must be 0 (find_model), 1 (find_essential) or 2 (recover_pose)");
  *pairs_out = entry == 0 ? verify_chunk_pairs() : entry == 1 ? essential_chunk_pairs() : pose_chunk_pairs();
  return 0;
}

int p2p_find_model_batch(p2p_handle_t h, int model, const double* rows, int row_stride, const int64_t* offsets,
                         const int64_t* offsets_host, int K, const double* n_dev, double px_th, double conf, int max_iters,
                         unsigned long long seed, double* models_out, uint8_t* mask_out, int32_t* n_inliers_out,
                         void* stream) {
  P2P_ENTER(h);
  P2P_REQUIRE(model >= 0 && model <= 2, "model must be 0 (F), 1 (H) or 2 (F with the DEGENSAC degeneracy check)");
  int rc = check_batch(rows, row_stride, offsets, offsets_host, K);
  if (rc) return rc;
  P2P_REQUIRE(px_th > 0.0 && isfinite(px_th), "px_th must be positive");
  P2P_REQUIRE(conf > 0.0 && conf < 1.0, "conf must lie in (0, 1)");
  P2P_REQUIRE(max_iters > 0 && max_iters <= (1 << 24), "max_iters must lie in [1, 2^24]");
  if (K == 0) return 0;
  P2P_REQUIRE(models_out && mask_out && n_inliers_out, "null tensor pointer");
  const int chunk = verify_chunk_pairs();
  const size_t need = batch_scratch(offsets_host, K, chunk, [](int p, long long r) { return verify_scratch_bytes(p, r, true); });
  if ((rc = h->verify.reserve(need + 4096))) return rc;
  void* scratch = h->verify.take(need);
  for (int k0 = 0; k0 < K; k0 += chunk) {
    const PairBatch B = batch_chunk(rows, row_stride, offsets, offsets_host, n_dev, k0, std::min(chunk, K - k0));
    if ((rc = launch_find_model(model, B, px_th, conf, max_iters, seed, scratch, models_out + 9 * (size_t)k0, mask_out,
                                n_inliers_out + k0, reinterpret_cast<cudaStream_t>(stream))))
      return rc;
  }
  return 0;
}

int p2p_sampson_distance(p2p_handle_t h, const double* rows, int row_stride, int n, const double* F, double* dist_out,
                         void* stream) {
  P2P_ENTER(h);
  P2P_REQUIRE(F && dist_out && (rows || n == 0), "null tensor pointer");
  P2P_REQUIRE(n >= 0 && row_stride >= 4, "bad row count or stride");
  return launch_sampson_distance(rows, row_stride, n, F, dist_out, reinterpret_cast<cudaStream_t>(stream));
}

int p2p_epipolar_histograms(p2p_handle_t h, const double* rows, int row_stride, int n, const double* n_dev,
                            int coarse_col, const double* F, const uint8_t* mask, const double* edges, int n_edges,
                            int32_t* counts_out, void* stream) {
  P2P_ENTER(h);
  P2P_REQUIRE(F && edges && counts_out && (rows || n == 0), "null pointer");
  P2P_REQUIRE(n >= 0 && row_stride >= 4, "bad row count or stride");
  P2P_REQUIRE(coarse_col == -1 || (coarse_col >= 0 && coarse_col + 4 <= row_stride),
              "coarse_col must be -1 or a column with 4 columns of the row from it");
  P2P_REQUIRE(n_edges >= 2 && n_edges <= kMaxHistEdges, "n_edges must be in 2..16");
  EpiHistArgs a{};
  for (int j = 0; j < 9; ++j) a.F[j] = F[j];
  for (int i = 0; i < n_edges; ++i) {
    P2P_REQUIRE(std::isfinite(edges[i]) && (i == 0 || edges[i] > edges[i - 1]), "edges must be finite and increasing");
    a.edges[i] = edges[i];
  }
  a.n_edges = n_edges;
  return launch_epipolar_histograms(rows, row_stride, n, n_dev, coarse_col, mask, a, counts_out,
                                    reinterpret_cast<cudaStream_t>(stream));
}

int p2p_overlap_scores(p2p_handle_t h, const int64_t* point3D_ids, const int64_t* offsets,
                       const int64_t* offsets_host, int n_images, int words, uint32_t* bits_out, int32_t* counts_out,
                       double* scores_out, void* stream) {
  P2P_ENTER(h);
  P2P_REQUIRE(n_images >= 0 && n_images <= kMaxOverlapImages, "n_images must be in 0 .. 2^20");
  P2P_REQUIRE(words >= 0 && words <= (int)((kMaxOverlapPoints + 31) / 32), "words must be in 0 .. 2^26");
  P2P_REQUIRE(offsets_host != nullptr, "offsets_host is null");
  if (n_images == 0) return 0;
  P2P_REQUIRE(offsets && counts_out && scores_out && (bits_out || words == 0), "null pointer");
  P2P_REQUIRE(offsets_host[0] >= 0, "offsets must be non-negative");
  for (int i = 0; i < n_images; ++i) {
    const int64_t len = offsets_host[i + 1] - offsets_host[i];
    P2P_REQUIRE(len >= 0, "offsets must be non-decreasing");
    P2P_REQUIRE(len <= kMaxOverlapPoints, "an image has 2^31 or more 2D points");
    P2P_REQUIRE((len + 31) / 32 <= words, "words is smaller than ceil(n2d / 32) of an image");
  }
  P2P_REQUIRE(point3D_ids || offsets_host[n_images] == offsets_host[0], "point3D_ids is null");
  return launch_overlap_scores(reinterpret_cast<const long long*>(point3D_ids),
                               reinterpret_cast<const long long*>(offsets), n_images, words,
                               reinterpret_cast<unsigned*>(bits_out), counts_out, scores_out,
                               reinterpret_cast<cudaStream_t>(stream));
}

int p2p_test_hypotheses(p2p_handle_t h, int model, const double* rows, int row_stride, int n, double px_th,
                        unsigned long long seed, int count, double* models_out, int32_t* counts_out, void* stream) {
  P2P_ENTER(h);
  P2P_REQUIRE(model == 0 || model == 1, "model must be 0 (F) or 1 (H)");
  P2P_REQUIRE(rows && models_out && counts_out && count > 0 && row_stride >= 4, "bad argument");
  P2P_REQUIRE(n >= (model == 0 ? 7 : 4) && n <= (1 << 26), "fewer rows than a minimal sample");
  int rc = h->verify.reserve(verify_scratch_bytes(1, n, false) + 4096);
  if (rc) return rc;
  void* scratch = h->verify.take(verify_scratch_bytes(1, n, false));
  return launch_test_hypotheses(model, rows, row_stride, n, px_th, seed, count, scratch, models_out, counts_out,
                                reinterpret_cast<cudaStream_t>(stream));
}

int p2p_test_degeneracy(p2p_handle_t h, const double* rows, int row_stride, int n, double px_th, unsigned long long seed,
                        int count, int32_t* triplet_out, double* H_out, void* stream) {
  P2P_ENTER(h);
  P2P_REQUIRE(rows && triplet_out && H_out && count > 0 && count <= (1 << 20) && row_stride >= 4, "bad argument");
  P2P_REQUIRE(n >= 7 && n <= (1 << 26), "fewer rows than a minimal sample");
  P2P_REQUIRE(px_th > 0.0 && isfinite(px_th), "px_th must be positive");
  int rc = h->verify.reserve(verify_degeneracy_scratch_bytes(n, count) + 4096);
  if (rc) return rc;
  void* scratch = h->verify.take(verify_degeneracy_scratch_bytes(n, count));
  return launch_test_degeneracy(rows, row_stride, n, px_th, seed, count, scratch, triplet_out, H_out,
                                reinterpret_cast<cudaStream_t>(stream));
}

static bool intrinsics_ok(const double* intr, Intrinsics& K) {
  if (intr == nullptr) return false;
  for (int i = 0; i < 8; ++i)
    if (!isfinite(intr[i])) return false;
  K = Intrinsics{intr[0], intr[1], intr[2], intr[3], intr[4], intr[5], intr[6], intr[7]};
  return K.fx1 > 0.0 && K.fy1 > 0.0 && K.fx2 > 0.0 && K.fy2 > 0.0;
}

int p2p_find_essential(p2p_handle_t h, const double* rows, int row_stride, int n, const double* n_dev, const double* intr,
                       double px_th, double conf, int max_iters, unsigned long long seed, double* E_out, uint8_t* mask_out,
                       int32_t* n_inliers_out, void* stream) {
  P2P_ENTER(h);
  P2P_REQUIRE(E_out && mask_out && n_inliers_out && (rows || n == 0), "null tensor pointer");
  P2P_REQUIRE(n >= 0 && n <= (1 << 26) && row_stride >= 4, "bad row count or stride");
  Intrinsics K;
  P2P_REQUIRE(intrinsics_ok(intr, K), "intr must be 8 finite values with positive focal lengths");
  P2P_REQUIRE(px_th > 0.0 && isfinite(px_th), "px_th must be positive");
  P2P_REQUIRE(conf > 0.0 && conf < 1.0, "conf must lie in (0, 1)");
  P2P_REQUIRE(max_iters > 0 && max_iters <= (1 << 24), "max_iters must lie in [1, 2^24]");
  int rc = h->verify.reserve(essential_scratch_bytes(1, n, true) + 4096);
  if (rc) return rc;
  void* scratch = h->verify.take(essential_scratch_bytes(1, n, true));
  return launch_find_essential(single_pair(rows, row_stride, n, n_dev), nullptr, K, px_th, conf, max_iters, seed, scratch,
                               E_out, mask_out, n_inliers_out, reinterpret_cast<cudaStream_t>(stream));
}

int p2p_find_essential_batch(p2p_handle_t h, const double* rows, int row_stride, const int64_t* offsets,
                             const int64_t* offsets_host, int K, const double* n_dev, const double* intr, double px_th,
                             double conf, int max_iters, unsigned long long seed, double* E_out, uint8_t* mask_out,
                             int32_t* n_inliers_out, void* stream) {
  P2P_ENTER(h);
  int rc = check_batch(rows, row_stride, offsets, offsets_host, K);
  if (rc) return rc;
  P2P_REQUIRE(px_th > 0.0 && isfinite(px_th), "px_th must be positive");
  P2P_REQUIRE(conf > 0.0 && conf < 1.0, "conf must lie in (0, 1)");
  P2P_REQUIRE(max_iters > 0 && max_iters <= (1 << 24), "max_iters must lie in [1, 2^24]");
  if (K == 0) return 0;
  P2P_REQUIRE(intr && E_out && mask_out && n_inliers_out, "null tensor pointer");
  const int chunk = essential_chunk_pairs();
  const size_t need =
      batch_scratch(offsets_host, K, chunk, [](int p, long long r) { return essential_scratch_bytes(p, r, true); });
  if ((rc = h->verify.reserve(need + 4096))) return rc;
  void* scratch = h->verify.take(need);
  for (int k0 = 0; k0 < K; k0 += chunk) {
    const PairBatch B = batch_chunk(rows, row_stride, offsets, offsets_host, n_dev, k0, std::min(chunk, K - k0));
    if ((rc = launch_find_essential(B, intr + 8 * (size_t)k0, Intrinsics{}, px_th, conf, max_iters, seed, scratch,
                                    E_out + 9 * (size_t)k0, mask_out, n_inliers_out + k0,
                                    reinterpret_cast<cudaStream_t>(stream))))
      return rc;
  }
  return 0;
}

int p2p_recover_pose(p2p_handle_t h, const double* rows, int row_stride, int n, const double* n_dev, const double* intr,
                     const double* E, const uint8_t* mask_in, double dist_th, double* Rt_out, uint8_t* mask_out,
                     int32_t* n_good_out, void* stream) {
  P2P_ENTER(h);
  P2P_REQUIRE(E && Rt_out && mask_out && n_good_out && (rows || n == 0), "null tensor pointer");
  P2P_REQUIRE(n >= 0 && n <= (1 << 26) && row_stride >= 4, "bad row count or stride");
  Intrinsics K;
  P2P_REQUIRE(intrinsics_ok(intr, K), "intr must be 8 finite values with positive focal lengths");
  P2P_REQUIRE(dist_th > 0.0 && isfinite(dist_th), "dist_th must be positive");
  int rc = h->verify.reserve(pose_scratch_bytes(1, n) + 4096);
  if (rc) return rc;
  void* scratch = h->verify.take(pose_scratch_bytes(1, n));
  return launch_recover_pose(single_pair(rows, row_stride, n, n_dev), nullptr, K, E, mask_in, dist_th, scratch, Rt_out,
                             mask_out, n_good_out, reinterpret_cast<cudaStream_t>(stream));
}

int p2p_recover_pose_batch(p2p_handle_t h, const double* rows, int row_stride, const int64_t* offsets,
                           const int64_t* offsets_host, int K, const double* n_dev, const double* intr, const double* E,
                           const uint8_t* mask_in, double dist_th, double* Rt_out, uint8_t* mask_out, int32_t* n_good_out,
                           void* stream) {
  P2P_ENTER(h);
  int rc = check_batch(rows, row_stride, offsets, offsets_host, K);
  if (rc) return rc;
  P2P_REQUIRE(dist_th > 0.0 && isfinite(dist_th), "dist_th must be positive");
  if (K == 0) return 0;
  P2P_REQUIRE(intr && E && Rt_out && mask_out && n_good_out, "null tensor pointer");
  const int chunk = pose_chunk_pairs();
  const size_t need = batch_scratch(offsets_host, K, chunk, [](int p, long long r) { return pose_scratch_bytes(p, r); });
  if ((rc = h->verify.reserve(need + 4096))) return rc;
  void* scratch = h->verify.take(need);
  for (int k0 = 0; k0 < K; k0 += chunk) {
    const PairBatch B = batch_chunk(rows, row_stride, offsets, offsets_host, n_dev, k0, std::min(chunk, K - k0));
    if ((rc = launch_recover_pose(B, intr + 8 * (size_t)k0, Intrinsics{}, E + 9 * (size_t)k0, mask_in, dist_th, scratch,
                                  Rt_out + 12 * (size_t)k0, mask_out, n_good_out + k0,
                                  reinterpret_cast<cudaStream_t>(stream))))
      return rc;
  }
  return 0;
}

int p2p_test_essential_hypotheses(p2p_handle_t h, const double* rows, int row_stride, int n, const double* intr,
                                  double px_th, unsigned long long seed, int count, double* models_out,
                                  int32_t* counts_out, void* stream) {
  P2P_ENTER(h);
  P2P_REQUIRE(rows && models_out && counts_out && count > 0 && row_stride >= 4, "bad argument");
  P2P_REQUIRE(n >= 5 && n <= (1 << 26), "fewer rows than a minimal sample");
  Intrinsics K;
  P2P_REQUIRE(intrinsics_ok(intr, K), "intr must be 8 finite values with positive focal lengths");
  P2P_REQUIRE(px_th > 0.0 && isfinite(px_th), "px_th must be positive");
  int rc = h->verify.reserve(essential_scratch_bytes(1, n, false) + 4096);
  if (rc) return rc;
  void* scratch = h->verify.take(essential_scratch_bytes(1, n, false));
  return launch_test_essential_hypotheses(rows, row_stride, n, K, px_th, seed, count, scratch, models_out, counts_out,
                                          reinterpret_cast<cudaStream_t>(stream));
}

int p2p_test_gemm(p2p_handle_t h, const float* a, const float* b, float* c, int M, int N, int K, int passes,
                  int seg_len, float in_scale, void* stream) {
  P2P_ENTER(h);
  cudaStream_t st = reinterpret_cast<cudaStream_t>(stream);
  P2P_REQUIRE(a && b && c && M > 0 && N > 0 && K > 0, "bad argument");
  P2P_REQUIRE(K % 64 == 0 && K / 64 <= kMaxKSteps, "K must be a multiple of 64 and at most 6144");
  P2P_REQUIRE(passes == 1 || passes == 3, "passes must be 1 or 3");
  const int mpad = (int)align_up(M, 128), npad = (int)align_up(N, 256);
  const size_t ab = (size_t)mpad * K * 2, bb = (size_t)npad * K * 2;
  int rc = h->misc.reserve(2 * (ab + bb) + (1 << 16));
  if (rc) return rc;
  __half* a_hi = (__half*)h->misc.take(ab);
  __half* a_lo = (__half*)h->misc.take(ab);
  __half* b_hi = (__half*)h->misc.take(bb);
  __half* b_lo = (__half*)h->misc.take(bb);
  P2P_CUDA_OK(cudaMemsetAsync(a_hi, 0, 2 * ab, st));
  P2P_CUDA_OK(cudaMemsetAsync(b_hi, 0, 2 * bb, st));
  if ((rc = launch_split_rows(a, a_hi, a_lo, (size_t)M * K, in_scale, st))) return rc;
  if ((rc = launch_split_rows(b, b_hi, b_lo, (size_t)N * K, in_scale, st))) return rc;
  UmmaGemmParams p;
  memset(&p, 0, sizeof(p));
  const uint64_t ad[5] = {(uint64_t)K, 1, 1, 1, (uint64_t)mpad};
  const uint64_t as[4] = {(uint64_t)K * 2, (uint64_t)K * 2, (uint64_t)K * 2, (uint64_t)K * 2};
  const uint32_t abx[5] = {64, 1, 1, 1, 128};
  const uint64_t bd[2] = {(uint64_t)K, (uint64_t)npad};
  const uint64_t bs[1] = {(uint64_t)K * 2};
  const uint32_t bbx[2] = {64, 128};
  if ((rc = make_tmap_fp16(&p.a_main_hi, a_hi, 5, ad, as, abx))) return rc;
  if ((rc = make_tmap_fp16(&p.a_main_lo, a_lo, 5, ad, as, abx))) return rc;
  if ((rc = make_tmap_fp16(&p.b_hi, b_hi, 2, bd, bs, bbx))) return rc;
  if ((rc = make_tmap_fp16(&p.b_lo, b_lo, 2, bd, bs, bbx))) return rc;
  p.a_rgb_hi = p.a_main_hi;
  p.a_rgb_lo = p.a_main_lo;
  p.nsteps = K / 64;
  for (int s = 0; s < p.nsteps; ++s) p.steps[s] = KStep{(short)(s * 64), 0, 0, 0, 0, 0, s * 64};
  p.m_tiles = mpad / 128;
  p.n_tiles = npad / 256;
  p.a_units_per_tile = 128;
  p.seg_len = seg_len;
  p.epi.c = c;
  p.epi.ldc = N;
  p.epi.m_rows = M;
  p.epi.n_cols = N;
  p.epi.alpha = 1.f / (in_scale * in_scale);
  return launch_umma_gemm(p, EPI_PLAIN, passes, sms(h), st);
}

}
```

### patch2pix_b200/csrc/umma_gemm.cu

```cuda
#include <cuda.h>

#include <vector>

#include "kernels.h"
#include "umma_gemm.h"
#include "umma_ptx.cuh"

namespace p2p {

__device__ __forceinline__ size_t part_offset(int unit, int row64, int col) {
  return (((size_t)unit * 2 + (col >> 8)) * 64 + row64) * 256 + (col & 255);
}
__device__ __forceinline__ int part_unit(int slot, int split_slot, int split_unit) {
  return slot < split_slot ? slot >> 2 : split_unit + ((slot - split_slot) >> 2);
}
__device__ __forceinline__ void share_piece(const WindowShare& ws, int split_slot, int split_unit, int n_patches, int m_tile,
                                            int row, int col0, float* srow) {
  const int n = m_tile * 2 + (row >> 6);
  if (n >= n_patches) return;
  if (ws.part_out != nullptr) {
    float4* dst = reinterpret_cast<float4*>(ws.part_out + part_offset(n, row & 63, col0));
#pragma unroll 1
    for (int q = 0; q < 8; ++q) dst[q] = make_float4(srow[4 * q], srow[4 * q + 1], srow[4 * q + 2], srow[4 * q + 3]);
  } else {
    const float4* src = reinterpret_cast<const float4*>(ws.part_in + part_offset(part_unit(n, split_slot, split_unit), row & 63, col0));
    float4 a8[8];
#pragma unroll
    for (int q = 0; q < 8; ++q) a8[q] = __ldg(src + q);
#pragma unroll
    for (int q = 0; q < 8; ++q) {
      const float4 a = a8[q];
      srow[4 * q] += a.x;
      srow[4 * q + 1] += a.y;
      srow[4 * q + 2] += a.z;
      srow[4 * q + 3] += a.w;
    }
  }
}

template <int EPI, bool SHARE>
__device__ __forceinline__ void epilogue_piece(const UmmaEpilogue& e, const WindowShare& ws, int n_patches, int m_tile,
                                               int row, int col0, const float* v) {
  if (EPI == EPI_PLAIN) {
    const int r = m_tile * 128 + row;
    if (r < e.m_rows) {
      float* dst = e.c + (size_t)r * e.ldc + col0;
#pragma unroll
      for (int i = 0; i < 32; ++i)
        if (col0 + i < e.n_cols) dst[i] = v[i] * e.alpha;
    }
  } else if (EPI == EPI_CONV1) {
    const int n = m_tile * 2 + (row >> 6);
    if (n < n_patches) {
      const int r = SHARE && ws.slot_row != nullptr ? __ldg(ws.slot_row + n) : n;
      __align__(16) __half h[32];
      __align__(16) __half l[32];
#pragma unroll
      for (int i = 0; i < 32; ++i) {
        const float y = fmaf(v[i], __ldg(e.scale + col0 + i), __ldg(e.bias + col0 + i)) * e.y_scale;
        h[i] = __float2half_rn(y);
        l[i] = __float2half_rn(y - __half2float(h[i]));
      }
      const size_t o = ((size_t)r * 64 + (row & 63)) * 512 + col0;
#pragma unroll
      for (int q = 0; q < 4; ++q) reinterpret_cast<uint4*>(e.y_hi + o)[q] = reinterpret_cast<const uint4*>(h)[q];
      if (e.y_lo != nullptr) {
#pragma unroll
        for (int q = 0; q < 4; ++q) reinterpret_cast<uint4*>(e.y_lo + o)[q] = reinterpret_cast<const uint4*>(l)[q];
      }
      if (e.pooled != nullptr && (row & 63) == 0) {
        float4* z = reinterpret_cast<float4*>(e.pooled + (size_t)r * 512 + col0);
#pragma unroll
        for (int q = 0; q < 8; ++q) z[q] = make_float4(0.f, 0.f, 0.f, 0.f);
      }
    }
  } else if (EPI == EPI_CONV2) {
    const int n = m_tile * 2 + (row >> 6);
    const int lane = threadIdx.x & 31;
    unsigned int mine = 0;
#pragma unroll
    for (int i = 0; i < 32; ++i) {
      const float y = fmaxf(fmaf(v[i], __ldg(e.scale + col0 + i), __ldg(e.bias + col0 + i)), 0.f);
      const unsigned int m = __reduce_max_sync(0xffffffffu, __float_as_uint(y));
      if (lane == i) mine = m;
    }
    if (n < n_patches) atomicMax(reinterpret_cast<unsigned int*>(e.pooled) + (size_t)n * 512 + col0 + lane, mine);
  } else if (EPI == EPI_FC) {
    const int r = m_tile * 128 + row;
    if (r < n_patches) {
      __align__(16) __half h[32];
      __align__(16) __half l[32];
#pragma unroll
      for (int i = 0; i < 32; ++i) {
        const float y = fminf(fmaxf(fmaf(v[i], __ldg(e.scale + col0 + i), __ldg(e.bias + col0 + i)), 0.f) * e.y_scale, 65504.f);
        h[i] = __float2half_rn(y);
        l[i] = __float2half_rn(y - __half2float(h[i]));
      }
      const size_t o = (size_t)r * e.ldc + col0;
#pragma unroll
      for (int q = 0; q < 4; ++q) {
        reinterpret_cast<uint4*>(e.y_hi + o)[q] = reinterpret_cast<const uint4*>(h)[q];
        reinterpret_cast<uint4*>(e.y_lo + o)[q] = reinterpret_cast<const uint4*>(l)[q];
      }
    }
  } else if (EPI == EPI_CORR) {
    const int lane = threadIdx.x & 31;
    const int pa = m_tile * 128 + row;
    const int ca = pa >> 2, mi = pa & 3;
#pragma unroll
    for (int cell = 0; cell < 8; ++cell) {
      float best = v[cell * 4];
      int code = mi * 4;
#pragma unroll
      for (int j = 1; j < 4; ++j)
        if (v[cell * 4 + j] > best) {
          best = v[cell * 4 + j];
          code = mi * 4 + j;
        }
#pragma unroll
      for (int o = 1; o <= 2; o <<= 1) {
        const float b2 = __shfl_xor_sync(0xffffffffu, best, o);
        const int c2 = __shfl_xor_sync(0xffffffffu, code, o);
        if (b2 > best || (b2 == best && c2 < code)) {
          best = b2;
          code = c2;
        }
      }
      const int cb = (col0 >> 2) + cell;
      if ((lane & 3) == 0 && ca < e.np1 && cb < e.np2) {
        e.c[(size_t)ca * e.np2 + cb] = best * e.alpha;
        e.code[(size_t)ca * e.np2 + cb] = (uint8_t)code;
      }
    }
  }
}

constexpr int kATile = 128 * 128;
constexpr int kBTile = 128 * 128;
constexpr int kEpiPitch = 65;
constexpr int kEpiBytes = 64 * kEpiPitch * 4;
constexpr int kMaxSmemPerBlock = 232448;

template <int PASSES, bool SEGMENTED, int AMODE>
struct GemmCfg {
  static constexpr int NOP = PASSES == 3 ? 2 : 1;
  static constexpr int THREADS = AMODE == AMODE_GATHER ? 512 : 384;
  static constexpr int BN = PASSES == 1 && !SEGMENTED && THREADS == 384 ? 256 : 128;
  static constexpr int B_BYTES = BN * 128;
  static constexpr int STAGE_BYTES = NOP * (kATile + B_BYTES);
  static constexpr int STAGES = PASSES == 3 ? 3 : (THREADS == 512 ? 4 : (BN == 256 ? 4 : 6));
  static constexpr int SMEM = STAGES * STAGE_BYTES + 2 * kEpiBytes + 1024;
  static constexpr int FG = AMODE == AMODE_GATHER ? 16 : 1;
  static constexpr int STATIC_SMEM = 3 * STAGES * 8 + 2 * 2 * FG * FG * 4 + 2 * 4 * 4;
  static_assert(SMEM + STATIC_SMEM <= kMaxSmemPerBlock, "shared memory over the per-block limit");
  static constexpr int LAUNCH_REGS = (65536 / THREADS) & ~7;
  static constexpr int PRODUCER_REGS = THREADS == 512 || BN == 256 ? 24 : 40;
  static constexpr int AUX_REGS = THREADS == 512 ? 128 : 0;
  static constexpr int CONSUMER_REGS = THREADS == 512 ? 176 : (BN == 256 ? 240 : 232);
  static_assert(PRODUCER_REGS + 2 * CONSUMER_REGS + AUX_REGS <= THREADS / 128 * LAUNCH_REGS, "register budget overcommitted");
  static_assert(PRODUCER_REGS <= LAUNCH_REGS && CONSUMER_REGS >= LAUNCH_REGS && AUX_REGS <= LAUNCH_REGS, "setmaxnreg direction");
};

__device__ __forceinline__ int fg_clamp(int v, int ds, int full) {
  if (v < 0) return 0;
  const int q = v / ds, m = full / ds - 1;
  return q < m ? q : m;
}

__device__ __forceinline__ void named_bar(int id, int threads) {
  asm volatile("bar.sync %0, %1;" ::"r"(id), "r"(threads) : "memory");
}

__device__ __forceinline__ int window_origin(const WindowMaps& wm, int n, int j) {
  int v;
  if (wm.is_float) v = (int)reinterpret_cast<const float*>(wm.matches)[(size_t)n * 4 + j];
  else v = (int)reinterpret_cast<const long long*>(wm.matches)[(size_t)n * 4 + j];
  const int lim = (j & 1) ? wm.H[j >> 1] : wm.W[j >> 1];
  v = v < -7 ? -7 : (v > lim + 8 ? lim + 8 : v);
  return v - 8 + kMapPad;
}

__device__ __forceinline__ int window_row(const WindowShare& ws, int s, int n_units) {
  if (s >= n_units) s = 0;
  return ws.slot_row != nullptr ? __ldg(ws.slot_row + s) : s;
}

template <int PASSES, bool SEGMENTED, int EPI, int AMODE>
__global__ void __launch_bounds__(GemmCfg<PASSES, SEGMENTED, AMODE>::THREADS, 1) umma_gemm_kernel(const __grid_constant__ UmmaGemmParams p) {
  static_assert(AMODE == AMODE_TMA || (PASSES == 1 && !SEGMENTED && EPI == EPI_CONV1), "fused A operand: conv1, 1-pass only");
  using Cfg = GemmCfg<PASSES, SEGMENTED, AMODE>;
  constexpr int STAGES = Cfg::STAGES, NOP = Cfg::NOP, STAGE_BYTES = Cfg::STAGE_BYTES;
  constexpr int BN = Cfg::BN, B_BYTES = Cfg::B_BYTES, NACC = BN / 2;

  extern __shared__ uint8_t smem_raw[];
  uint8_t* smem = reinterpret_cast<uint8_t*>((reinterpret_cast<uintptr_t>(smem_raw) + 1023) & ~(uintptr_t)1023);
  float* epi_smem = reinterpret_cast<float*>(smem + STAGES * STAGE_BYTES);
  __shared__ __align__(8) uint64_t full_bar[STAGES];
  __shared__ __align__(8) uint64_t ready_bar[STAGES];
  __shared__ __align__(8) uint64_t empty_bar[STAGES];
  constexpr int FG = Cfg::FG;
  __shared__ float fg_dinv[2][2][FG][FG];
  __shared__ int fg_org[2][4];

  const int warp = threadIdx.x >> 5, lane = threadIdx.x & 31;
  int m_tiles = p.m_tiles;
  int n_units = p.epi.n_patches;
  if (p.d_units != nullptr) {
    n_units = __ldg(p.d_units);
    m_tiles = (n_units + p.a_units_per_tile - 1) / p.a_units_per_tile;
  }
  const int n_col_tiles = p.n_tiles * (256 / BN);
  const int total_tiles = m_tiles * n_col_tiles;
  const int nsteps = p.nsteps;
  const int seg_len = SEGMENTED ? p.seg_len : nsteps;
  int split_tile = total_tiles, split_unit = 0;
  if (AMODE == AMODE_WINDOW && p.ws.d_split != nullptr) {
    split_tile = __ldg(p.ws.d_split);
    split_unit = __ldg(p.ws.d_split + 1);
  }

  if (warp == 0 && lane == 0) {
    tma_prefetch_desc(&p.b_hi);
    if (AMODE == AMODE_TMA) tma_prefetch_desc(&p.a_main_hi);
    if (AMODE == AMODE_WINDOW) {
      tma_prefetch_desc(&p.wm.map[0]);
      tma_prefetch_desc(&p.wm.map[1]);
      tma_prefetch_desc(&p.a_rgb_hi);
    }
    if (PASSES == 3) {
      tma_prefetch_desc(&p.a_main_lo);
      tma_prefetch_desc(&p.b_lo);
    }
  }
  if (warp == 1 && lane == 0) {
    for (int i = 0; i < STAGES; ++i) {
      mbar_init(&full_bar[i], AMODE == AMODE_GATHER ? 5 : 1);
      mbar_init(&ready_bar[i], 3);
      mbar_init(&empty_bar[i], 2);
    }
    fence_barrier_init();
  }
  __syncthreads();

  const int wgi = warpgroup_index();
  if (wgi == 0) {
    setmaxnreg_dec<Cfg::PRODUCER_REGS>();
    if (warp == 0 && lane == 0) {
      int it = 0;
      auto load_b = [&](const CUtensorMap* map, uint64_t* bar, uint8_t* dst, int bk, int brow) {
#pragma unroll
        for (int h = 0; h < BN / 128; ++h) tma_load_2d(map, bar, dst + h * kBTile, bk, brow + h * 128);
      };
      for (int tile = blockIdx.x; tile < total_tiles; tile += gridDim.x) {
        const int m_tile = tile / n_col_tiles, brow = (tile - m_tile * n_col_tiles) * BN;
        const int a4 = m_tile * p.a_units_per_tile;
        const int kofs = m_tile < split_tile ? 0 : p.ws.class_steps;
        if (AMODE == AMODE_WINDOW && p.ws.part_in != nullptr) {
#pragma unroll 1
          for (int pp = 0; pp < 2; ++pp)
            if (m_tile * 2 + pp < n_units)
              bulk_prefetch_l2(p.ws.part_in + part_offset(part_unit(m_tile * 2 + pp, 2 * split_tile, split_unit), 0, brow),
                               64 * 256 * 4);
        }
        int o[2][4];
        if (AMODE == AMODE_WINDOW) {
#pragma unroll
          for (int pp = 0; pp < 2; ++pp) {
            const int row = window_row(p.ws, m_tile * 2 + pp, n_units);
#pragma unroll
            for (int j = 0; j < 4; ++j) o[pp][j] = window_origin(p.wm, row, j);
          }
        }
        for (int ks = 0; ks < nsteps; ++ks, ++it) {
          const int s = it % STAGES;
          mbar_wait(&empty_bar[s], ((uint32_t)(it / STAGES) & 1u) ^ 1u);
          const KStep k = p.steps[ks + kofs];
          uint8_t* st = smem + (size_t)s * STAGE_BYTES;
          if (AMODE == AMODE_GATHER) {
            mbar_expect_tx(&full_bar[s], B_BYTES);
            load_b(&p.b_hi, &full_bar[s], st + kATile, k.bk, brow);
          } else if (AMODE == AMODE_WINDOW) {
            mbar_expect_tx(&full_bar[s], STAGE_BYTES);
            load_b(&p.b_hi, &full_bar[s], st + kATile, k.bk, brow);
            if (k.kind == 0) {
              const int ty = (k.plane & 2) ? 1 : (k.y < 0 ? 0 : 2), tx = (k.plane & 1) ? 1 : (k.x < 0 ? 0 : 2);
              const int chunk = k.c0 >> 6, si = chunk >> 2, c0 = (chunk & 3) * 64;
#pragma unroll
              for (int pp = 0; pp < 2; ++pp)
                tma_load_3d(&p.wm.map[si], &full_bar[s], st + pp * 8192, c0, o[pp][2 * si] - 1 + tx, o[pp][2 * si + 1] - 1 + ty);
            } else {
              tma_load_5d(&p.a_rgb_hi, &full_bar[s], st, 0, 0, 0, 0, a4);
            }
          } else {
            mbar_expect_tx(&full_bar[s], STAGE_BYTES);
            if (k.kind == 0) {
              tma_load_5d(&p.a_main_hi, &full_bar[s], st, k.c0, k.x, k.y, k.plane, a4);
              if (PASSES == 3) tma_load_5d(&p.a_main_lo, &full_bar[s], st + kATile, k.c0, k.x, k.y, k.plane, a4);
            } else {
              tma_load_5d(&p.a_rgb_hi, &full_bar[s], st, 0, 0, 0, 0, a4);
              if (PASSES == 3) tma_load_5d(&p.a_rgb_lo, &full_bar[s], st + kATile, 0, 0, 0, 0, a4);
            }
            load_b(&p.b_hi, &full_bar[s], st + NOP * kATile, k.bk, brow);
            if (PASSES == 3) load_b(&p.b_lo, &full_bar[s], st + NOP * kATile + B_BYTES, k.bk, brow);
          }
        }
      }
    } else if (AMODE == AMODE_WINDOW && warp > 0) {
      const int t = threadIdx.x - 32;
      int it = 0;
      for (int tile = blockIdx.x; tile < total_tiles; tile += gridDim.x) {
        const int kofs = tile / n_col_tiles < split_tile ? 0 : p.ws.class_steps;
        for (int ks = 0; ks < nsteps; ++ks, ++it) {
          const int s = it % STAGES;
          mbar_wait(&full_bar[s], (uint32_t)(it / STAGES) & 1u);
          const KStep k = p.steps[ks + kofs];
          const bool zx = k.kind == 0 && !(k.plane & 1) && k.x < 0, zy = k.kind == 0 && !(k.plane & 2) && k.y < 0;
          if (zx || zy) {
            uint8_t* st = smem + (size_t)s * STAGE_BYTES;
            for (int i = t; i < 256; i += 96) {
              const int j = i >> 3, pp = (j >> 3) & 1, r8 = j & 7;
              const int row = pp * 64 + (j < 16 ? r8 * 8 : r8);
              if (j < 16 ? zx : zy) *reinterpret_cast<uint4*>(st + row * 128 + (i & 7) * 16) = make_uint4(0, 0, 0, 0);
            }
            fence_proxy_async();
          }
          __syncwarp();
          if (lane == 0) mbar_arrive(&ready_bar[s]);
        }
      }
    }
  } else if (wgi < 3) {
    setmaxnreg_inc<Cfg::CONSUMER_REGS>();
    const int wg = wgi - 1, wl = warp & 3;
    const bool leader = threadIdx.x % 128 == 0;
    uint64_t* ready = AMODE == AMODE_WINDOW ? ready_bar : full_bar;
    float* stg = epi_smem + wg * (64 * kEpiPitch);
    float acc[NACC];
    float tot[SEGMENTED ? NACC : 1];
    int it = 0;
    for (int tile = blockIdx.x; tile < total_tiles; tile += gridDim.x) {
      const int m_tile = tile / n_col_tiles, col0 = (tile - m_tile * n_col_tiles) * BN;
      if (SEGMENTED) {
#pragma unroll
        for (int i = 0; i < NACC; ++i) tot[i] = 0.f;
      }
      for (int ks = 0; ks < nsteps; ++ks, ++it) {
        const int s = it % STAGES;
        mbar_wait(&ready[s], (uint32_t)(it / STAGES) & 1u);
        const uint32_t sa = smem_u32(smem + (size_t)s * STAGE_BYTES);
        const uint64_t a_hi = make_sw128_desc(sa + wg * 8192);
        const uint64_t b_hi = make_sw128_desc(sa + NOP * kATile);
        uint32_t accf = (ks % seg_len) == 0 ? 0u : 1u;
        wgmma_fence();
        if (PASSES == 3) {
          const uint64_t a_lo = make_sw128_desc(sa + kATile + wg * 8192);
          const uint64_t b_lo = make_sw128_desc(sa + NOP * kATile + B_BYTES);
#pragma unroll
          for (int kk = 0; kk < 4; ++kk) {
            wgmma_f16<BN>(acc, a_lo + 2 * kk, b_hi + 2 * kk, accf);
            accf = 1u;
          }
#pragma unroll
          for (int kk = 0; kk < 4; ++kk) wgmma_f16<BN>(acc, a_hi + 2 * kk, b_lo + 2 * kk, 1u);
        }
#pragma unroll
        for (int kk = 0; kk < 4; ++kk) {
          wgmma_f16<BN>(acc, a_hi + 2 * kk, b_hi + 2 * kk, accf);
          accf = 1u;
        }
        wgmma_commit();
        const bool seg_end = SEGMENTED && ((ks + 1) % seg_len) == 0 && (ks + 1) < nsteps;
        const bool prev_pending = SEGMENTED ? (ks % seg_len) != 0 : ks != 0;
        if (seg_end) {
          wgmma_wait<0>();
          wgmma_fence_regs<NACC>(acc);
#pragma unroll
          for (int i = 0; i < NACC; ++i) tot[i] += acc[i];
        } else {
          wgmma_wait<1>();
        }
        mbar_arrive_if(&empty_bar[(s + STAGES - 1) % STAGES], leader && prev_pending);
        mbar_arrive_if(&empty_bar[s], leader && seg_end);
      }
      wgmma_wait<0>();
      wgmma_fence_regs<NACC>(acc);
      mbar_arrive_if(&empty_bar[(it + STAGES - 1) % STAGES], leader);
      if (SEGMENTED) {
#pragma unroll
        for (int i = 0; i < NACC; ++i) tot[i] += acc[i];
      }
      const float* res = SEGMENTED ? tot : acc;
      const int fr = 16 * wl + (lane >> 2), fc = 2 * (lane & 3);
      const int er = (wl & 1) * 32 + lane, ec = (wl >> 1) * 32;
#pragma unroll
      for (int c64 = 0; c64 < BN / 64; ++c64) {
        named_bar(1 + wg, 128);
#pragma unroll
        for (int j = 0; j < 8; ++j) {
          const float* d = res + 4 * (c64 * 8 + j);
          float* o = stg + fr * kEpiPitch + 8 * j + fc;
          o[0] = d[0];
          o[1] = d[1];
          o[8 * kEpiPitch] = d[2];
          o[8 * kEpiPitch + 1] = d[3];
        }
        named_bar(1 + wg, 128);
        if (AMODE == AMODE_WINDOW && (p.ws.part_out != nullptr || p.ws.part_in != nullptr)) {
          share_piece(p.ws, 2 * split_tile, split_unit, n_units, m_tile, wg * 64 + er, col0 + c64 * 64 + ec,
                      stg + er * kEpiPitch + ec);
          if (p.ws.part_out != nullptr) continue;
        }
        float v[32];
#pragma unroll
        for (int i = 0; i < 32; ++i) v[i] = stg[er * kEpiPitch + ec + i];
        epilogue_piece<EPI, AMODE == AMODE_WINDOW>(p.epi, p.ws, n_units, m_tile, wg * 64 + er, col0 + c64 * 64 + ec, v);
      }
    }
  } else if (AMODE == AMODE_GATHER) {
    if constexpr (Cfg::AUX_REGS < Cfg::LAUNCH_REGS) setmaxnreg_dec<Cfg::AUX_REGS>();
    const int ptid = threadIdx.x - 384;
    const int l8 = ptid & 7, r16 = ptid >> 3;
    const FusedGather& g = p.fg;
    int it = 0;
    for (int tile = blockIdx.x; tile < total_tiles; tile += gridDim.x) {
      const int m_tile = tile / n_col_tiles;
      named_bar(3, 128);
      if (ptid < 8) {
        const int pp = ptid >> 2, j = ptid & 3;
        const int n = m_tile * 2 + pp;
        int v = 0;
        if (n < n_units) {
          if (g.is_float)
            v = (int)reinterpret_cast<const float*>(g.matches)[(size_t)n * 4 + j];
          else
            v = (int)reinterpret_cast<const long long*>(g.matches)[(size_t)n * 4 + j];
        }
        fg_org[pp][j] = v - 8;
      }
      named_bar(3, 128);
      for (int i = ptid; i < 1024; i += 128) {
        const int pp = i >> 9, si = (i >> 8) & 1, wy = (i >> 4) & 15, wx = i & 15;
        const int X = fg_org[pp][2 * si] + wx, Y = fg_org[pp][2 * si + 1] + wy;
        float t = 0.f;
#pragma unroll
        for (int l = 0; l < 4; ++l) {
          const int ds = 1 << l;
          const int xi = fg_clamp(X, ds, g.W[si]), yi = fg_clamp(Y, ds, g.H[si]);
          t += __ldg(g.nsq[si][l] + (size_t)yi * (g.W[si] / ds) + xi);
        }
        fg_dinv[pp][si][wy][wx] = (m_tile * 2 + pp < n_units) ? __fdiv_rn(kActScale, sqrtf(t + 1e-6f)) : 0.f;
      }
      named_bar(3, 128);
      for (int ks = 0; ks < nsteps; ++ks, ++it) {
        const int s = it % STAGES;
        const uint32_t ph = (uint32_t)(it / STAGES) & 1u;
        const KStep k = p.steps[ks];
        uint8_t* at = smem + (size_t)s * STAGE_BYTES;
        if (k.kind == 0) {
          const int ty = (k.plane & 2) ? 1 : (k.y < 0 ? 0 : 2), tx = (k.plane & 1) ? 1 : (k.x < 0 ? 0 : 2);
          const int chunk = k.c0 >> 6, si = chunk >> 2, jj = chunk & 3;
          const int lvl = jj == 0 ? 0 : (jj == 1 ? 1 : 2);
          const int sh = lvl + 1, C = lvl == 2 ? 128 : 64;
          const int coff = (jj == 3 ? 64 : 0) + l8 * 8;
          const __half* fmap = g.nhwc16[si][lvl];
          const float* nsq = g.nsq[si][lvl + 1];
          const int wl = g.W[si] >> sh, hl = g.H[si] >> sh;
          uint4 vals[8];
          float sc[8];
#pragma unroll
          for (int ps = 0; ps < 8; ++ps) {
            const int row = ps * 16 + r16;
            const int pp = row >> 6, wy = 2 * ((row >> 3) & 7) - 1 + ty, wx = 2 * (row & 7) - 1 + tx;
            const int X = fg_org[pp][2 * si] + wx, Y = fg_org[pp][2 * si + 1] + wy;
            const int xi = X < 0 ? 0 : min(X >> sh, wl - 1), yi = Y < 0 ? 0 : min(Y >> sh, hl - 1);
            const int px = yi * wl + xi;
            vals[ps] = __ldg(reinterpret_cast<const uint4*>(fmap + (size_t)px * C + coff));
            const float dv = (wy >= 0 && wx >= 0) ? fg_dinv[pp][si][wy & 15][wx & 15] : 0.f;
            sc[ps] = dv * sqrtf(__ldg(nsq + px) + 1e-30f);
          }
          mbar_wait(&empty_bar[s], ph ^ 1u);
#pragma unroll
          for (int ps = 0; ps < 8; ++ps) {
            const int row = ps * 16 + r16;
            __half2* h2 = reinterpret_cast<__half2*>(&vals[ps]);
#pragma unroll
            for (int q = 0; q < 4; ++q) {
              const float2 f = __half22float2(h2[q]);
              h2[q] = __floats2half2_rn(f.x * sc[ps], f.y * sc[ps]);
            }
            *reinterpret_cast<uint4*>(at + row * 128 + ((l8 ^ (row & 7)) << 4)) = vals[ps];
          }
        } else {
          mbar_wait(&empty_bar[s], ph ^ 1u);
#pragma unroll 1
          for (int ps = 0; ps < 8; ++ps) {
            const int row = ps * 16 + r16;
            const int pp = row >> 6, oy = (row >> 3) & 7, ox = row & 7;
            __align__(16) __half hv[8];
#pragma unroll
            for (int i = 0; i < 8; ++i) {
              const int kk = l8 * 8 + i;
              float v = 0.f;
              if (kk < 54) {
                const int tap = kk / 6, r = kk - tap * 6;
                const int si = r / 3, ch = r - si * 3;
                const int wx = 2 * ox - 1 + tap % 3, wy = 2 * oy - 1 + tap / 3;
                if (wx >= 0 && wy >= 0) {
                  const int xi = fg_clamp(fg_org[pp][2 * si] + wx, 1, g.W[si]);
                  const int yi = fg_clamp(fg_org[pp][2 * si + 1] + wy, 1, g.H[si]);
                  v = __ldg(g.img[si] + ((size_t)ch * g.H[si] + yi) * g.W[si] + xi) * fg_dinv[pp][si][wy][wx];
                }
              }
              hv[i] = __float2half_rn(v);
            }
            *reinterpret_cast<uint4*>(at + row * 128 + ((l8 ^ (row & 7)) << 4)) = *reinterpret_cast<const uint4*>(hv);
          }
        }
        fence_proxy_async();
        __syncwarp();
        if (lane == 0) mbar_arrive(&full_bar[s]);
      }
    }
  }
}

__global__ void __launch_bounds__(256) window_rgb_kernel(const __grid_constant__ WindowMaps wm, int n_units, int npad,
                                                         __half* __restrict__ out, const int* __restrict__ slot_row,
                                                         const int* __restrict__ d_count) {
  const int row = blockIdx.x * 256 + threadIdx.x;
  if (row >= npad * 64) return;
  const int n = row >> 6, oy = (row >> 3) & 7, ox = row & 7;
  if (d_count != nullptr) {
    n_units = __ldg(d_count);
    if (n >= n_units + (n_units & 1)) return;
  }
  __align__(16) __half hv[64];
#pragma unroll
  for (int i = 0; i < 64; ++i) hv[i] = __float2half_rn(0.f);
  if (n < n_units) {
    const int r = slot_row != nullptr ? __ldg(slot_row + n) : n;
#pragma unroll
    for (int si = 0; si < 2; ++si) {
      const int bx = window_origin(wm, r, 2 * si), by = window_origin(wm, r, 2 * si + 1);
      const int Wp = wm.W[si] + 2 * kMapPad;
#pragma unroll
      for (int tap = 0; tap < 9; ++tap) {
        const int wx = 2 * ox - 1 + tap % 3, wy = 2 * oy - 1 + tap / 3;
        if (wx >= 0 && wy >= 0) {
          const uint2 q = __ldg(reinterpret_cast<const uint2*>(wm.rgbn[si] + ((size_t)(by + wy) * Wp + bx + wx) * 4));
          const __half* hq = reinterpret_cast<const __half*>(&q);
          hv[tap * 6 + si * 3 + 0] = hq[0];
          hv[tap * 6 + si * 3 + 1] = hq[1];
          hv[tap * 6 + si * 3 + 2] = hq[2];
        }
      }
    }
  }
  uint4* dst = reinterpret_cast<uint4*>(out + (size_t)row * 64);
#pragma unroll
  for (int c = 0; c < 8; ++c) dst[c] = reinterpret_cast<const uint4*>(hv)[c];
}

int launch_window_rgb(const WindowMaps& wm, int n, int npad, __half* out, cudaStream_t st, const int* slot_row,
                      const int* d_count) {
  P2P_REQUIRE(n >= 0 && npad >= n, "window rgb: bad patch count");
  if (npad == 0) return 0;
  window_rgb_kernel<<<(unsigned)cdiv(npad * 64, 256), 256, 0, st>>>(wm, n, npad, out, slot_row, d_count);
  P2P_LAUNCH_OK();
  return 0;
}

__device__ __forceinline__ void block_scan3(const int (&v)[3], int (&ex)[3], int (&tot)[3], int (*s_warp)[32]) {
  const int lane = threadIdx.x & 31, wid = threadIdx.x >> 5;
  int inc[3];
#pragma unroll
  for (int c = 0; c < 3; ++c) {
    inc[c] = v[c];
#pragma unroll
    for (int o = 1; o < 32; o <<= 1) {
      const int t = __shfl_up_sync(0xffffffffu, inc[c], o);
      if (lane >= o) inc[c] += t;
    }
    if (lane == 31) s_warp[c][wid] = inc[c];
  }
  __syncthreads();
#pragma unroll
  for (int c = 0; c < 3; ++c) {
    int woff = 0, t = 0;
    for (int w = 0; w < 32; ++w) {
      const int x = s_warp[c][w];
      if (w < wid) woff += x;
      t += x;
    }
    ex[c] = woff + inc[c] - v[c];
    tot[c] = t;
  }
  __syncthreads();
}

__global__ void __launch_bounds__(1024) window_share_classify_kernel(const __grid_constant__ WindowMaps wm, int n,
                                                                     int* __restrict__ prefix, int* __restrict__ cont,
                                                                     int* __restrict__ unsh, int* __restrict__ cnt,
                                                                     int* __restrict__ shared_out) {
  __shared__ int s_warp[3][32];
  __shared__ int s_base[3];
  __shared__ int s_na;
  const int tid = threadIdx.x, groups = (n + 7) / 8;
  auto shared_half = [&](int g, int h) {
    if (8 * g + 8 > n) return 0;
    const int si = 1 - h, r0 = 8 * g + 4 * h;
    const int x = window_origin(wm, r0, 2 * si), y = window_origin(wm, r0, 2 * si + 1);
    for (int i = 1; i < 4; ++i)
      if (window_origin(wm, r0 + i, 2 * si) != x || window_origin(wm, r0 + i, 2 * si + 1) != y) return 0;
    return 1;
  };
  if (tid == 0) s_na = s_base[0] = s_base[1] = s_base[2] = 0;
  __syncthreads();
  int na = 0;
  for (int g = tid; g < groups; g += 1024) na += shared_half(g, 0);
  atomicAdd(&s_na, na);
  __syncthreads();
  const int nA = s_na, ubase = nA + (nA & 1);
  for (int g0 = 0; g0 < groups; g0 += 1024) {
    const int g = g0 + tid;
    int v[3] = {0, 0, 0};
    if (g < groups) {
      v[0] = shared_half(g, 0);
      v[1] = shared_half(g, 1);
      v[2] = min(8, n - 8 * g) - 4 * (v[0] + v[1]);
    }
    int ex[3], tot[3];
    block_scan3(v, ex, tot, s_warp);
    if (g < groups) {
      const int ia = s_base[0] + ex[0], ib = s_base[1] + ex[1];
      int iu = s_base[2] + ex[2];
      if (v[0]) {
        prefix[ia] = 8 * g;
        for (int i = 0; i < 4; ++i) cont[4 * ia + i] = 8 * g + i;
      }
      if (v[1]) {
        prefix[ubase + ib] = 8 * g + 4;
        for (int i = 0; i < 4; ++i) cont[4 * (nA + ib) + i] = 8 * g + 4 + i;
      }
      for (int r = 8 * g; r < min(8 * g + 8, n); ++r)
        if (!(r - 8 * g < 4 ? v[0] : v[1])) unsh[iu++] = r;
    }
    __syncthreads();
    if (tid == 0)
      for (int c = 0; c < 3; ++c) s_base[c] += tot[c];
    __syncthreads();
  }
  if (tid == 0) {
    const int nB = s_base[1];
    if (nA & 1) prefix[nA] = prefix[nA - 1];
    cnt[0] = ubase + nB;
    cnt[1] = ubase / 2;
    cnt[2] = 0;
    cnt[3] = 4 * (nA + nB);
    cnt[4] = 2 * nA;
    cnt[5] = ubase;
    cnt[6] = s_base[2];
    cnt[7] = 0;
    if (shared_out != nullptr) *shared_out = 4 * (nA + nB);
  }
}

int launch_window_share_classify(const WindowMaps& wm, int n, int* prefix, int* cont, int* unsh, int* cnt, int* shared_out,
                                 cudaStream_t st) {
  P2P_REQUIRE(n >= 0, "window share: bad row count");
  window_share_classify_kernel<<<1, 1024, 0, st>>>(wm, n, prefix, cont, unsh, cnt, shared_out);
  P2P_LAUNCH_OK();
  return 0;
}


typedef CUresult (*PFN_tmapEncodeTiled)(CUtensorMap*, CUtensorMapDataType, cuuint32_t, void*, const cuuint64_t*,
                                        const cuuint64_t*, const cuuint32_t*, const cuuint32_t*, CUtensorMapInterleave,
                                        CUtensorMapSwizzle, CUtensorMapL2promotion, CUtensorMapFloatOOBfill);

static PFN_tmapEncodeTiled get_encode_fn() {
  static PFN_tmapEncodeTiled fn = nullptr;
  if (fn == nullptr) {
    void* p = nullptr;
    cudaDriverEntryPointQueryResult qres;
    if (cudaGetDriverEntryPoint("cuTensorMapEncodeTiled", &p, cudaEnableDefault, &qres) == cudaSuccess &&
        qres == cudaDriverEntryPointSuccess)
      fn = reinterpret_cast<PFN_tmapEncodeTiled>(p);
  }
  return fn;
}

namespace {
struct TmapKey {
  const void* base;
  int rank;
  uint64_t dims[5];
  uint64_t strides[4];
  uint32_t box[5];
  uint32_t es[5];
  bool operator==(const TmapKey& o) const { return memcmp(this, &o, sizeof(TmapKey)) == 0; }
};
struct TmapEntry {
  TmapKey key;
  CUtensorMap map;
};
constexpr int kTmapCacheSize = 128;
thread_local std::vector<TmapEntry> g_tmap_cache;
thread_local int g_tmap_next = 0;
}

int make_tmap_fp16(CUtensorMap* out, const void* base, int rank, const uint64_t* dims, const uint64_t* strides_bytes,
                   const uint32_t* box, const uint32_t* estrides) {
  TmapKey key;
  memset(&key, 0, sizeof(key));
  key.base = base;
  key.rank = rank;
  for (int i = 0; i < rank; ++i) { key.dims[i] = dims[i]; key.box[i] = box[i]; key.es[i] = estrides ? estrides[i] : 1; }
  for (int i = 0; i + 1 < rank; ++i) key.strides[i] = strides_bytes[i];
  for (const TmapEntry& e : g_tmap_cache)
    if (e.key == key) {
      *out = e.map;
      return 0;
    }
  PFN_tmapEncodeTiled fn = get_encode_fn();
  if (fn == nullptr) {
    set_last_error("cuTensorMapEncodeTiled is not available from the driver");
    return -2;
  }
  cuuint64_t gd[5];
  cuuint64_t gs[4];
  cuuint32_t bx[5], es[5];
  for (int i = 0; i < rank; ++i) {
    gd[i] = dims[i];
    bx[i] = box[i];
    es[i] = estrides ? estrides[i] : 1;
  }
  for (int i = 0; i + 1 < rank; ++i) gs[i] = strides_bytes[i];
  const CUresult r = fn(out, CU_TENSOR_MAP_DATA_TYPE_FLOAT16, (cuuint32_t)rank, const_cast<void*>(base), gd, gs, bx, es,
                        CU_TENSOR_MAP_INTERLEAVE_NONE, CU_TENSOR_MAP_SWIZZLE_128B, CU_TENSOR_MAP_L2_PROMOTION_L2_256B,
                        CU_TENSOR_MAP_FLOAT_OOB_FILL_NONE);
  if (r != CUDA_SUCCESS) {
    set_last_error("cuTensorMapEncodeTiled failed with CUresult " + std::to_string((int)r));
    return -2;
  }
  if ((int)g_tmap_cache.size() < kTmapCacheSize) {
    g_tmap_cache.push_back(TmapEntry{key, *out});
  } else {
    g_tmap_cache[g_tmap_next] = TmapEntry{key, *out};
    g_tmap_next = (g_tmap_next + 1) % kTmapCacheSize;
  }
  return 0;
}

template <int PASSES, bool SEGMENTED, int EPI, int AMODE = AMODE_TMA>
static int launch_one(const UmmaGemmParams& p, int num_sms, cudaStream_t st) {
  using Cfg = GemmCfg<PASSES, SEGMENTED, AMODE>;
  auto kern = umma_gemm_kernel<PASSES, SEGMENTED, EPI, AMODE>;
  const int total = p.m_tiles * p.n_tiles * (256 / Cfg::BN);
  const int grid = total < num_sms ? total : num_sms;
  P2P_ENSURE_SMEM(kern, Cfg::SMEM);
  kern<<<grid, Cfg::THREADS, Cfg::SMEM, st>>>(p);
  P2P_LAUNCH_OK();
  return 0;
}

template <int EPI>
static int launch_epi(const UmmaGemmParams& p, int passes, bool seg, int num_sms, cudaStream_t st) {
  if (passes == 3) return seg ? launch_one<3, true, EPI>(p, num_sms, st) : launch_one<3, false, EPI>(p, num_sms, st);
  return seg ? launch_one<1, true, EPI>(p, num_sms, st) : launch_one<1, false, EPI>(p, num_sms, st);
}

int launch_umma_gemm(const UmmaGemmParams& p, int epi, int passes, int num_sms, cudaStream_t st, int amode) {
  P2P_REQUIRE(passes == 1 || passes == 3, "umma gemm: passes must be 1 or 3");
  P2P_REQUIRE(p.nsteps > 0 && p.m_tiles > 0 && p.n_tiles > 0, "umma gemm: empty problem");
  const bool seg = p.seg_len > 0 && p.seg_len < p.nsteps;
  if (amode != AMODE_TMA) {
    P2P_REQUIRE(epi == EPI_CONV1 && passes == 1 && !seg, "the fused A operand is available for 1-pass conv1 only");
    if (amode == AMODE_GATHER) return launch_one<1, false, EPI_CONV1, AMODE_GATHER>(p, num_sms, st);
    P2P_REQUIRE(amode == AMODE_WINDOW, "umma gemm: unknown A mode");
    return launch_one<1, false, EPI_CONV1, AMODE_WINDOW>(p, num_sms, st);
  }
  switch (epi) {
    case EPI_PLAIN: return launch_epi<EPI_PLAIN>(p, passes, seg, num_sms, st);
    case EPI_CONV1: return launch_epi<EPI_CONV1>(p, passes, seg, num_sms, st);
    case EPI_CONV2: return launch_epi<EPI_CONV2>(p, passes, seg, num_sms, st);
    case EPI_CORR: return launch_epi<EPI_CORR>(p, passes, seg, num_sms, st);
    case EPI_FC: return launch_epi<EPI_FC>(p, passes, seg, num_sms, st);
  }
  set_last_error("umma gemm: unknown epilogue");
  return -1;
}

}
```

### patch2pix_b200/csrc/umma_gemm.h

```cpp
#pragma once
#include <cuda.h>

#include "kernels.h"

namespace p2p {

enum { EPI_PLAIN = 0, EPI_CONV1 = 1, EPI_CONV2 = 2, EPI_CORR = 3, EPI_FC = 4 };
enum { AMODE_TMA = 0, AMODE_GATHER = 1, AMODE_WINDOW = 2 };
constexpr int kMaxKSteps = 96;

struct UmmaEpilogue {
  float* c;
  int ldc, m_rows, n_cols;
  float alpha;
  uint8_t* code;
  int np1, np2;
  const float* scale;
  const float* bias;
  float y_scale;
  __half* y_hi;
  __half* y_lo;
  float* pooled;
  int n_patches;
};

struct FusedGather {
  const float* img[2];
  const __half* nhwc16[2][3];
  const float* nsq[2][4];
  int H[2], W[2];
  const void* matches;
  int is_float;
};

struct WindowMaps {
  CUtensorMap map[2];
  const __half* rgbn[2];
  int H[2], W[2];
  const void* matches;
  int is_float;
};

struct WindowShare {
  const int* slot_row;
  const int* d_split;
  int class_steps;
  float* part_out;
  const float* part_in;
};

struct UmmaGemmParams {
  CUtensorMap a_main_hi, a_main_lo, a_rgb_hi, a_rgb_lo, b_hi, b_lo;
  KStep steps[kMaxKSteps];
  int nsteps;
  int m_tiles;
  int n_tiles;
  int a_units_per_tile;
  int seg_len;
  const int* d_units;
  UmmaEpilogue epi;
  FusedGather fg;
  WindowMaps wm;
  WindowShare ws;
};

int make_tmap_fp16(CUtensorMap* out, const void* base, int rank, const uint64_t* dims, const uint64_t* strides_bytes,
                   const uint32_t* box, const uint32_t* estrides = nullptr);
int launch_umma_gemm(const UmmaGemmParams& p, int epi, int passes, int num_sms, cudaStream_t st, int amode = AMODE_TMA);
int launch_window_rgb(const WindowMaps& wm, int n, int npad, __half* out, cudaStream_t st, const int* slot_row = nullptr,
                      const int* d_count = nullptr);
int launch_window_share_classify(const WindowMaps& wm, int n, int* prefix, int* cont, int* unsh, int* cnt, int* shared_out,
                                 cudaStream_t st);

}
```

### patch2pix_b200/csrc/umma_ptx.cuh

```cuda
#pragma once
#include <cuda.h>
#include <cuda_runtime.h>
#include <stdint.h>

namespace p2p {

__device__ __forceinline__ uint32_t smem_u32(const void* p) { return (uint32_t)__cvta_generic_to_shared(p); }

__device__ __forceinline__ void mbar_init(uint64_t* bar, uint32_t count) {
  asm volatile("mbarrier.init.shared::cta.b64 [%0], %1;" ::"r"(smem_u32(bar)), "r"(count));
}
__device__ __forceinline__ void mbar_expect_tx(uint64_t* bar, uint32_t bytes) {
  asm volatile("mbarrier.arrive.expect_tx.shared::cta.b64 _, [%0], %1;" ::"r"(smem_u32(bar)), "r"(bytes) : "memory");
}
__device__ __forceinline__ void mbar_arrive(uint64_t* bar) {
  asm volatile("mbarrier.arrive.shared::cta.b64 _, [%0];" ::"r"(smem_u32(bar)) : "memory");
}
__device__ __forceinline__ void mbar_arrive_if(uint64_t* bar, bool pred) {
  asm volatile(
      "{\n"
      ".reg .pred p;\n"
      "setp.ne.b32 p, %1, 0;\n"
      "@p mbarrier.arrive.shared::cta.b64 _, [%0];\n"
      "}\n" ::"r"(smem_u32(bar)), "r"((uint32_t)pred)
      : "memory");
}
__device__ __forceinline__ void mbar_wait(uint64_t* bar, uint32_t parity) {
  asm volatile(
      "{\n"
      ".reg .pred p;\n"
      ".reg .u32 n;\n"
      ".reg .s64 t0, t1;\n"
      "mbarrier.try_wait.parity.shared::cta.b64 p, [%0], %1;\n"
      "@p bra DONE;\n"
      "mov.u64 t0, %%clock64;\n"
      "ROUND:\n"
      "mov.u32 n, 4096;\n"
      "PROBE:\n"
      "mbarrier.try_wait.parity.shared::cta.b64 p, [%0], %1;\n"
      "@p bra DONE;\n"
      "sub.u32 n, n, 1;\n"
      "setp.ne.u32 p, n, 0;\n"
      "@p bra PROBE;\n"
      "mov.u64 t1, %%clock64;\n"
      "sub.s64 t1, t1, t0;\n"
      "setp.lt.s64 p, t1, 6000000000;\n"
      "@p bra ROUND;\n"
      "trap;\n"
      "DONE:\n"
      "}\n" ::"r"(smem_u32(bar)), "r"(parity)
      : "memory");
}
__device__ __forceinline__ void fence_barrier_init() { asm volatile("fence.mbarrier_init.release.cluster;" ::: "memory"); }
__device__ __forceinline__ void fence_proxy_async() { asm volatile("fence.proxy.async.shared::cta;" ::: "memory"); }

__device__ __forceinline__ void tma_prefetch_desc(const CUtensorMap* m) {
  asm volatile("prefetch.tensormap [%0];" ::"l"(reinterpret_cast<uint64_t>(m)) : "memory");
}
__device__ __forceinline__ void tma_load_2d(const CUtensorMap* m, uint64_t* bar, void* dst, int c0, int c1) {
  asm volatile(
      "cp.async.bulk.tensor.2d.shared::cluster.global.tile.mbarrier::complete_tx::bytes [%0], [%1, {%3, %4}], [%2];"
      ::"r"(smem_u32(dst)), "l"(reinterpret_cast<uint64_t>(m)), "r"(smem_u32(bar)), "r"(c0), "r"(c1)
      : "memory");
}
__device__ __forceinline__ void tma_load_3d(const CUtensorMap* m, uint64_t* bar, void* dst, int c0, int c1, int c2) {
  asm volatile(
      "cp.async.bulk.tensor.3d.shared::cluster.global.tile.mbarrier::complete_tx::bytes [%0], [%1, {%3, %4, %5}], [%2];"
      ::"r"(smem_u32(dst)), "l"(reinterpret_cast<uint64_t>(m)), "r"(smem_u32(bar)), "r"(c0), "r"(c1), "r"(c2)
      : "memory");
}
__device__ __forceinline__ void tma_load_4d(const CUtensorMap* m, uint64_t* bar, void* dst, int c0, int c1, int c2, int c3) {
  asm volatile(
      "cp.async.bulk.tensor.4d.shared::cluster.global.tile.mbarrier::complete_tx::bytes [%0], [%1, {%3, %4, %5, %6}], [%2];"
      ::"r"(smem_u32(dst)), "l"(reinterpret_cast<uint64_t>(m)), "r"(smem_u32(bar)), "r"(c0), "r"(c1), "r"(c2), "r"(c3)
      : "memory");
}
__device__ __forceinline__ void bulk_load(uint64_t* bar, void* dst, const void* src, uint32_t bytes) {
  asm volatile("cp.async.bulk.shared::cluster.global.mbarrier::complete_tx::bytes [%0], [%1], %2, [%3];" ::"r"(smem_u32(dst)),
               "l"(reinterpret_cast<uint64_t>(src)), "r"(bytes), "r"(smem_u32(bar))
               : "memory");
}
__device__ __forceinline__ void tma_load_5d(const CUtensorMap* m, uint64_t* bar, void* dst, int c0, int c1, int c2,
                                            int c3, int c4) {
  asm volatile(
      "cp.async.bulk.tensor.5d.shared::cluster.global.tile.mbarrier::complete_tx::bytes [%0], [%1, {%3, %4, %5, %6, "
      "%7}], [%2];" ::"r"(smem_u32(dst)),
      "l"(reinterpret_cast<uint64_t>(m)), "r"(smem_u32(bar)), "r"(c0), "r"(c1), "r"(c2), "r"(c3), "r"(c4)
      : "memory");
}

__device__ __forceinline__ void tma_store_3d(const CUtensorMap* m, const void* src, int c0, int c1, int c2) {
  asm volatile("cp.async.bulk.tensor.3d.global.shared::cta.bulk_group [%0, {%2, %3, %4}], [%1];" ::"l"(
                   reinterpret_cast<uint64_t>(m)),
               "r"(smem_u32(src)), "r"(c0), "r"(c1), "r"(c2)
               : "memory");
}
__device__ __forceinline__ void bulk_prefetch_l2(const void* src, uint32_t bytes) {
  asm volatile("cp.async.bulk.prefetch.L2.global [%0], %1;" ::"l"(reinterpret_cast<uint64_t>(src)), "r"(bytes) : "memory");
}
__device__ __forceinline__ void bulk_commit_group() { asm volatile("cp.async.bulk.commit_group;" ::: "memory"); }
template <int N>
__device__ __forceinline__ void bulk_wait_group_read() {
  asm volatile("cp.async.bulk.wait_group.read %0;" ::"n"(N) : "memory");
}

__device__ __forceinline__ void wgmma_fence() { asm volatile("wgmma.fence.sync.aligned;" ::: "memory"); }
__device__ __forceinline__ void wgmma_commit() { asm volatile("wgmma.commit_group.sync.aligned;" ::: "memory"); }
template <int N>
__device__ __forceinline__ void wgmma_wait() {
  asm volatile("wgmma.wait_group.sync.aligned %0;" ::"n"(N) : "memory");
}
template <int N>
__device__ __forceinline__ void setmaxnreg_inc() { asm volatile("setmaxnreg.inc.sync.aligned.u32 %0;" ::"n"(N)); }
template <int N>
__device__ __forceinline__ void setmaxnreg_dec() { asm volatile("setmaxnreg.dec.sync.aligned.u32 %0;" ::"n"(N)); }
__device__ __forceinline__ int warpgroup_index() { return __shfl_sync(0xffffffffu, (int)threadIdx.x / 128, 0); }

template <int R>
__device__ __forceinline__ void wgmma_fence_regs(float* d) {
#pragma unroll
  for (int i = 0; i < R; ++i) asm volatile("" : "+f"(d[i])::"memory");
}

template <int N>
__device__ __forceinline__ void wgmma_f16(float* d, uint64_t adesc, uint64_t bdesc, uint32_t accumulate);
template <>
__device__ __forceinline__ void wgmma_f16<16>(float* d, uint64_t adesc, uint64_t bdesc, uint32_t accumulate) {
  asm volatile(
      "{\n"
      ".reg .pred p;\n"
      "setp.ne.b32 p, %10, 0;\n"
      "wgmma.mma_async.sync.aligned.m64n16k16.f32.f16.f16 "
      "{%0, %1, %2, %3, %4, %5, %6, %7}, "
      "%8, %9, p, 1, 1, 0, 0;\n"
      "}\n"
      : "+f"(d[0]), "+f"(d[1]), "+f"(d[2]), "+f"(d[3]), "+f"(d[4]), "+f"(d[5]), "+f"(d[6]), "+f"(d[7])
      : "l"(adesc), "l"(bdesc), "r"(accumulate));
}
template <>
__device__ __forceinline__ void wgmma_f16<32>(float* d, uint64_t adesc, uint64_t bdesc, uint32_t accumulate) {
  asm volatile(
      "{\n"
      ".reg .pred p;\n"
      "setp.ne.b32 p, %18, 0;\n"
      "wgmma.mma_async.sync.aligned.m64n32k16.f32.f16.f16 "
      "{%0, %1, %2, %3, %4, %5, %6, %7, %8, %9, %10, %11, %12, %13, %14, %15}, "
      "%16, %17, p, 1, 1, 0, 0;\n"
      "}\n"
      : "+f"(d[0]), "+f"(d[1]), "+f"(d[2]), "+f"(d[3]), "+f"(d[4]), "+f"(d[5]), "+f"(d[6]), "+f"(d[7]), "+f"(d[8]), "+f"(d[9]), "+f"(d[10]), "+f"(d[11]), "+f"(d[12]), "+f"(d[13]), "+f"(d[14]), "+f"(d[15])
      : "l"(adesc), "l"(bdesc), "r"(accumulate));
}
template <>
__device__ __forceinline__ void wgmma_f16<64>(float* d, uint64_t adesc, uint64_t bdesc, uint32_t accumulate) {
  asm volatile(
      "{\n"
      ".reg .pred p;\n"
      "setp.ne.b32 p, %34, 0;\n"
      "wgmma.mma_async.sync.aligned.m64n64k16.f32.f16.f16 "
      "{%0, %1, %2, %3, %4, %5, %6, %7, %8, %9, %10, %11, %12, %13, %14, %15, %16, %17, %18, %19, %20, %21, %22, %23, %24, %25, %26, %27, %28, %29, %30, %31}, "
      "%32, %33, p, 1, 1, 0, 0;\n"
      "}\n"
      : "+f"(d[0]), "+f"(d[1]), "+f"(d[2]), "+f"(d[3]), "+f"(d[4]), "+f"(d[5]), "+f"(d[6]), "+f"(d[7]), "+f"(d[8]), "+f"(d[9]), "+f"(d[10]), "+f"(d[11]), "+f"(d[12]), "+f"(d[13]), "+f"(d[14]), "+f"(d[15]), "+f"(d[16]), "+f"(d[17]), "+f"(d[18]), "+f"(d[19]), "+f"(d[20]), "+f"(d[21]), "+f"(d[22]), "+f"(d[23]), "+f"(d[24]), "+f"(d[25]), "+f"(d[26]), "+f"(d[27]), "+f"(d[28]), "+f"(d[29]), "+f"(d[30]), "+f"(d[31])
      : "l"(adesc), "l"(bdesc), "r"(accumulate));
}
template <>
__device__ __forceinline__ void wgmma_f16<128>(float* d, uint64_t adesc, uint64_t bdesc, uint32_t accumulate) {
  asm volatile(
      "{\n"
      ".reg .pred p;\n"
      "setp.ne.b32 p, %66, 0;\n"
      "wgmma.mma_async.sync.aligned.m64n128k16.f32.f16.f16 "
      "{%0, %1, %2, %3, %4, %5, %6, %7, %8, %9, %10, %11, %12, %13, %14, %15, %16, %17, %18, %19, %20, %21, %22, %23, %24, %25, %26, %27, %28, %29, %30, %31, %32, %33, %34, %35, %36, %37, %38, %39, %40, %41, %42, %43, %44, %45, %46, %47, %48, %49, %50, %51, %52, %53, %54, %55, %56, %57, %58, %59, %60, %61, %62, %63}, "
      "%64, %65, p, 1, 1, 0, 0;\n"
      "}\n"
      : "+f"(d[0]), "+f"(d[1]), "+f"(d[2]), "+f"(d[3]), "+f"(d[4]), "+f"(d[5]), "+f"(d[6]), "+f"(d[7]), "+f"(d[8]), "+f"(d[9]), "+f"(d[10]), "+f"(d[11]), "+f"(d[12]), "+f"(d[13]), "+f"(d[14]), "+f"(d[15]), "+f"(d[16]), "+f"(d[17]), "+f"(d[18]), "+f"(d[19]), "+f"(d[20]), "+f"(d[21]), "+f"(d[22]), "+f"(d[23]), "+f"(d[24]), "+f"(d[25]), "+f"(d[26]), "+f"(d[27]), "+f"(d[28]), "+f"(d[29]), "+f"(d[30]), "+f"(d[31]), "+f"(d[32]), "+f"(d[33]), "+f"(d[34]), "+f"(d[35]), "+f"(d[36]), "+f"(d[37]), "+f"(d[38]), "+f"(d[39]), "+f"(d[40]), "+f"(d[41]), "+f"(d[42]), "+f"(d[43]), "+f"(d[44]), "+f"(d[45]), "+f"(d[46]), "+f"(d[47]), "+f"(d[48]), "+f"(d[49]), "+f"(d[50]), "+f"(d[51]), "+f"(d[52]), "+f"(d[53]), "+f"(d[54]), "+f"(d[55]), "+f"(d[56]), "+f"(d[57]), "+f"(d[58]), "+f"(d[59]), "+f"(d[60]), "+f"(d[61]), "+f"(d[62]), "+f"(d[63])
      : "l"(adesc), "l"(bdesc), "r"(accumulate));
}
template <>
__device__ __forceinline__ void wgmma_f16<256>(float* d, uint64_t adesc, uint64_t bdesc, uint32_t accumulate) {
  asm volatile(
      "{\n"
      ".reg .pred p;\n"
      "setp.ne.b32 p, %130, 0;\n"
      "wgmma.mma_async.sync.aligned.m64n256k16.f32.f16.f16 "
      "{%0, %1, %2, %3, %4, %5, %6, %7, %8, %9, %10, %11, %12, %13, %14, %15, %16, %17, %18, %19, %20, %21, %22, %23, %24, %25, %26, %27, %28, %29, %30, %31, %32, %33, %34, %35, %36, %37, %38, %39, %40, %41, %42, %43, %44, %45, %46, %47, %48, %49, %50, %51, %52, %53, %54, %55, %56, %57, %58, %59, %60, %61, %62, %63, %64, %65, %66, %67, %68, %69, %70, %71, %72, %73, %74, %75, %76, %77, %78, %79, %80, %81, %82, %83, %84, %85, %86, %87, %88, %89, %90, %91, %92, %93, %94, %95, %96, %97, %98, %99, %100, %101, %102, %103, %104, %105, %106, %107, %108, %109, %110, %111, %112, %113, %114, %115, %116, %117, %118, %119, %120, %121, %122, %123, %124, %125, %126, %127}, "
      "%128, %129, p, 1, 1, 0, 0;\n"
      "}\n"
      : "+f"(d[0]), "+f"(d[1]), "+f"(d[2]), "+f"(d[3]), "+f"(d[4]), "+f"(d[5]), "+f"(d[6]), "+f"(d[7]), "+f"(d[8]), "+f"(d[9]), "+f"(d[10]), "+f"(d[11]), "+f"(d[12]), "+f"(d[13]), "+f"(d[14]), "+f"(d[15]), "+f"(d[16]), "+f"(d[17]), "+f"(d[18]), "+f"(d[19]), "+f"(d[20]), "+f"(d[21]), "+f"(d[22]), "+f"(d[23]), "+f"(d[24]), "+f"(d[25]), "+f"(d[26]), "+f"(d[27]), "+f"(d[28]), "+f"(d[29]), "+f"(d[30]), "+f"(d[31]), "+f"(d[32]), "+f"(d[33]), "+f"(d[34]), "+f"(d[35]), "+f"(d[36]), "+f"(d[37]), "+f"(d[38]), "+f"(d[39]), "+f"(d[40]), "+f"(d[41]), "+f"(d[42]), "+f"(d[43]), "+f"(d[44]), "+f"(d[45]), "+f"(d[46]), "+f"(d[47]), "+f"(d[48]), "+f"(d[49]), "+f"(d[50]), "+f"(d[51]), "+f"(d[52]), "+f"(d[53]), "+f"(d[54]), "+f"(d[55]), "+f"(d[56]), "+f"(d[57]), "+f"(d[58]), "+f"(d[59]), "+f"(d[60]), "+f"(d[61]), "+f"(d[62]), "+f"(d[63]), "+f"(d[64]), "+f"(d[65]), "+f"(d[66]), "+f"(d[67]), "+f"(d[68]), "+f"(d[69]), "+f"(d[70]), "+f"(d[71]), "+f"(d[72]), "+f"(d[73]), "+f"(d[74]), "+f"(d[75]), "+f"(d[76]), "+f"(d[77]), "+f"(d[78]), "+f"(d[79]), "+f"(d[80]), "+f"(d[81]), "+f"(d[82]), "+f"(d[83]), "+f"(d[84]), "+f"(d[85]), "+f"(d[86]), "+f"(d[87]), "+f"(d[88]), "+f"(d[89]), "+f"(d[90]), "+f"(d[91]), "+f"(d[92]), "+f"(d[93]), "+f"(d[94]), "+f"(d[95]), "+f"(d[96]), "+f"(d[97]), "+f"(d[98]), "+f"(d[99]), "+f"(d[100]), "+f"(d[101]), "+f"(d[102]), "+f"(d[103]), "+f"(d[104]), "+f"(d[105]), "+f"(d[106]), "+f"(d[107]), "+f"(d[108]), "+f"(d[109]), "+f"(d[110]), "+f"(d[111]), "+f"(d[112]), "+f"(d[113]), "+f"(d[114]), "+f"(d[115]), "+f"(d[116]), "+f"(d[117]), "+f"(d[118]), "+f"(d[119]), "+f"(d[120]), "+f"(d[121]), "+f"(d[122]), "+f"(d[123]), "+f"(d[124]), "+f"(d[125]), "+f"(d[126]), "+f"(d[127])
      : "l"(adesc), "l"(bdesc), "r"(accumulate));
}

__device__ __forceinline__ uint64_t make_sw128_desc(uint32_t saddr) {
  uint64_t d = 0;
  d |= (uint64_t)((saddr & 0x3FFFFu) >> 4);
  d |= (uint64_t)1 << 16;
  d |= (uint64_t)(1024 >> 4) << 32;
  d |= (uint64_t)1 << 62;
  return d;
}

}
```

Before: 92.47.

## Add register-fragment epilogues for conv1/conv2 GEMMs with async TMA stores

```diff
diff --git a/include/p2p_b200.h b/include/p2p_b200.h
--- a/include/p2p_b200.h
+++ b/include/p2p_b200.h
@@ -140,6 +140,8 @@
 P2P_API int p2p_test_gemm(p2p_handle_t h, const float* a, const float* b, float* c, int M, int N, int K, int passes,
                   int seg_len, float in_scale, void* stream);
 
+P2P_API int p2p_tile_trace_read(p2p_handle_t h, int idx, int* tag, int* tiles, unsigned long long* out, int max_tiles);
+
 #ifdef __cplusplus
 }
 #endif
diff --git a/patch2pix_b200/_lib.py b/patch2pix_b200/_lib.py
--- a/patch2pix_b200/_lib.py
+++ b/patch2pix_b200/_lib.py
@@ -46,6 +46,7 @@
     'p2p_preprocess_image': (_I, [_P, _P, _I, _I, _I, _I, _P, _P, _P]),
     'p2p_profile_read': (_I, [_P, C.POINTER(C.c_float), C.POINTER(_I), _I]),
     'p2p_test_gemm': (_I, [_P, _P, _P, _P, _I, _I, _I, _I, _I, _F, _P]),
+    'p2p_tile_trace_read': (_I, [_P, _I, C.POINTER(_I), C.POINTER(_I), _P, _I]),
     'p2p_find_model': (_I, [_P, _I, _P, _I, _I, _P, C.c_double, C.c_double, _I, C.c_ulonglong, _P, _P, _P, _P]),
     'p2p_sampson_distance': (_I, [_P, _P, _I, _I, _P, _P, _P]),
     'p2p_epipolar_histograms': (_I, [_P, _P, _I, _I, _P, _I, C.POINTER(C.c_double), _P, C.POINTER(C.c_double), _I, _P,
@@ -130,6 +131,17 @@
         check(self.lib.p2p_get_option(self.h, key.encode(), C.byref(v)))
         return v.value
 
+    def tile_traces(self):
+        import numpy as np
+        out = []
+        for i in range(self.get_option('tile_traces')):
+            tag, tiles = C.c_int(), C.c_int()
+            check(self.lib.p2p_tile_trace_read(self.h, i, C.byref(tag), C.byref(tiles), None, 0))
+            buf = np.zeros((tiles.value, 8), dtype=np.uint64)
+            check(self.lib.p2p_tile_trace_read(self.h, i, C.byref(tag), C.byref(tiles), buf.ctypes.data, tiles.value))
+            out.append((tag.value, buf[buf[:, 6] != 0]))
+        return out
+
     def launch_count(self):
         v = C.c_longlong()
         check(self.lib.p2p_launch_count(self.h, C.byref(v)))
diff --git a/patch2pix_b200/csrc/api.cu b/patch2pix_b200/csrc/api.cu
--- a/patch2pix_b200/csrc/api.cu
+++ b/patch2pix_b200/csrc/api.cu
@@ -88,6 +88,16 @@
   int opt_fc_impl = 1;
   int opt_fuse_gather = 3;
   int opt_share_windows = 1;
+  int opt_epi_async = 1;
+  int frag_epi_launches = 0;
+  int opt_tile_trace = 0;
+  unsigned long long* trace_buf = nullptr;
+  size_t trace_used = 0;
+  struct TraceRec {
+    int tag, tiles;
+    size_t off;
+  };
+  std::vector<TraceRec> traces;
   const int* last_band_count = nullptr;
   int* share_rows = nullptr;
   bool last_mid_shared = false;
@@ -335,6 +345,22 @@
 
 int sms(const p2p_handle_s* h) { return h->opt_num_sms > 0 ? h->opt_num_sms : h->num_sms; }
 
+constexpr size_t kTraceCap = (size_t)8 << 20;
+
+int set_trace(p2p_handle_s* h, UmmaGemmParams& p, int tag, cudaStream_t st) {
+  p.trace = nullptr;
+  if (!h->opt_tile_trace) return 0;
+  const int tiles = p.m_tiles * p.n_tiles * 2;
+  const size_t need = (size_t)tiles * kTraceStamps;
+  if (h->trace_buf == nullptr) P2P_CUDA_OK(cudaMalloc(&h->trace_buf, kTraceCap * sizeof(unsigned long long)));
+  if (h->trace_used + need > kTraceCap) return 0;
+  p.trace = h->trace_buf + h->trace_used;
+  P2P_CUDA_OK(cudaMemsetAsync(p.trace, 0, need * sizeof(unsigned long long), st));
+  h->traces.push_back({tag, tiles, h->trace_used});
+  h->trace_used += need;
+  return 0;
+}
+
 struct ProfScope {
   p2p_handle_s* h;
   cudaStream_t st;
@@ -421,6 +447,7 @@
   if (h->ncw.blob) cudaFree(h->ncw.blob);
   if (h->band_totals) cudaFree(h->band_totals);
   if (h->share_rows) cudaFree(h->share_rows);
+  if (h->trace_buf) cudaFree(h->trace_buf);
   if (h->uniq_rank) cudaFree(h->uniq_rank);
   for (int i = 0; i < 2; ++i)
     if (h->reg[i].blob) cudaFree(h->reg[i].blob);
@@ -479,6 +506,8 @@
   if (!strcmp(key, "mid_band")) return &h->opt_mid_band;
   if (!strcmp(key, "fuse_gather")) return &h->opt_fuse_gather;
   if (!strcmp(key, "share_windows")) return &h->opt_share_windows;
+  if (!strcmp(key, "epi_async")) return &h->opt_epi_async;
+  if (!strcmp(key, "tile_trace")) return &h->opt_tile_trace;
   if (!strcmp(key, "fc_impl")) return &h->opt_fc_impl;
   if (!strcmp(key, "nc_impl")) return &h->opt_nc_impl;
   if (!strcmp(key, "nc_l2_mode")) return &h->opt_nc_l2_mode;
@@ -493,6 +522,12 @@
   if (s == &h->opt_mid_passes || s == &h->opt_fine_passes) P2P_REQUIRE(value == 1 || value == 3, "passes must be 1 or 3");
   if (s == &h->opt_corr_passes) P2P_REQUIRE(value == 0 || value == 1 || value == 3, "corr_passes must be 0, 1 or 3");
   if (s == &h->opt_share_windows) P2P_REQUIRE(value == 0 || value == 1, "share_windows must be 0 or 1");
+  if (s == &h->opt_epi_async) P2P_REQUIRE(value == 0 || value == 1, "epi_async must be 0 or 1");
+  if (s == &h->opt_tile_trace) {
+    P2P_REQUIRE(value == 0 || value == 1, "tile_trace must be 0 or 1");
+    h->traces.clear();
+    h->trace_used = 0;
+  }
   P2P_REQUIRE(value >= 0, "option values are non-negative");
   *s = value;
   return 0;
@@ -507,6 +542,14 @@
       P2P_CUDA_OK(cudaDeviceSynchronize());
       P2P_CUDA_OK(cudaMemcpy(value, h->last_band_count, sizeof(int), cudaMemcpyDeviceToHost));
     }
+    return 0;
+  }
+  if (!strcmp(key, "frag_epi_launches")) {
+    *value = h->frag_epi_launches;
+    return 0;
+  }
+  if (!strcmp(key, "tile_traces")) {
+    *value = (int)h->traces.size();
     return 0;
   }
   if (!strcmp(key, "shared_rows")) {
@@ -959,6 +1002,13 @@
       p.epi.y_lo = lo ? B.y_lo : nullptr;
       p.epi.pooled = B.pooled;
       p.epi.n_patches = n;
+      p.frag_epi = !lo && !fused && h->opt_epi_async;
+      if (p.frag_epi) {
+        const uint64_t yd[3] = {512, 64, npad};
+        const uint64_t ys[2] = {1024, 65536};
+        const uint32_t yb[3] = {64, 64, 1};
+        if ((rc = make_tmap_fp16(&p.y_store, B.y_hi, 3, yd, ys, yb))) return rc;
+      }
       if (fused) {
         for (int s2 = 0; s2 < 2; ++s2) {
           p.fg.img[s2] = h->pf[s2].img;
@@ -997,6 +1047,7 @@
       }
       ProfScope ps(h, kb + 1, st);
       const int amode = mapped ? AMODE_WINDOW : (fused ? AMODE_GATHER : AMODE_TMA);
+      const int tg = (rowmap != nullptr ? 2 : which) * 8;
       if (share) {
         float* part = B.part;
         KStep img[2][36];
@@ -1009,6 +1060,7 @@
         q.m_tiles = (n / 4 + 3) / 2;
         q.d_units = B.sh_cnt;
         q.ws = WindowShare{B.sh_prefix, B.sh_cnt + 1, 36, part, nullptr};
+        if ((rc = set_trace(h, q, tg + 1, st))) return rc;
         if ((rc = launch_umma_gemm(q, EPI_CONV1, passes, sms(h), st, amode))) return rc;
         memcpy(q.steps, img[0], sizeof(img[0]));
         q.steps[36] = R.steps1[72];
@@ -1018,15 +1070,19 @@
         q.m_tiles = (n + 1) / 2;
         q.d_units = B.sh_cnt + 3;
         q.ws = WindowShare{B.sh_cont, B.sh_cnt + 4, 37, nullptr, part};
+        if ((rc = set_trace(h, q, tg + 2, st))) return rc;
         if ((rc = launch_umma_gemm(q, EPI_CONV1, passes, sms(h), st, amode))) return rc;
         q = p;
         if ((rc = make_tmap_fp16(&q.a_rgb_hi, B.r_unsh, 5, rd, rs, abox))) return rc;
         q.d_units = B.sh_cnt + 6;
         q.ws = WindowShare{B.sh_unsh, nullptr, 0, nullptr, nullptr};
+        if ((rc = set_trace(h, q, tg + 3, st))) return rc;
         if ((rc = launch_umma_gemm(q, EPI_CONV1, passes, sms(h), st, amode))) return rc;
-      } else if ((rc = launch_umma_gemm(p, EPI_CONV1, passes, sms(h), st, amode))) {
-        return rc;
+      } else {
+        if ((rc = set_trace(h, p, tg, st))) return rc;
+        if ((rc = launch_umma_gemm(p, EPI_CONV1, passes, sms(h), st, amode))) return rc;
       }
+      h->frag_epi_launches += p.frag_epi ? (share ? 3 : 1) : 0;
     }
     {
       const uint64_t ad[5] = {512, 8, 8, 1, npad};
@@ -1044,8 +1100,10 @@
       p.epi.scale = R.scale2;
       p.epi.bias = R.bias2;
       p.epi.pooled = B.pooled;
+      if ((rc = set_trace(h, p, (rowmap != nullptr ? 2 : which) * 8 + 4, st))) return rc;
       ProfScope ps(h, kb + 2, st);
       if ((rc = launch_umma_gemm(p, EPI_CONV2, passes, sms(h), st))) return rc;
+      h->frag_epi_launches += p.frag_epi;
     }
   }
   ProfScope ps(h, kb + 3, st);
@@ -1512,7 +1570,24 @@
   p.epi.m_rows = M;
   p.epi.n_cols = N;
   p.epi.alpha = 1.f / (in_scale * in_scale);
+  if ((rc = set_trace(h, p, 24, st))) return rc;
   return launch_umma_gemm(p, EPI_PLAIN, passes, sms(h), st);
 }
 
-}
+int p2p_tile_trace_read(p2p_handle_t h, int idx, int* tag, int* tiles, unsigned long long* out, int max_tiles) {
+  P2P_ENTER(h);
+  P2P_REQUIRE(tag != nullptr && tiles != nullptr, "null argument");
+  P2P_REQUIRE(idx >= 0 && idx < (int)h->traces.size(), "tile trace index out of range");
+  const auto& t = h->traces[idx];
+  *tag = t.tag;
+  *tiles = t.tiles;
+  if (out != nullptr) {
+    P2P_REQUIRE(max_tiles >= t.tiles, "tile trace: output too small");
+    P2P_CUDA_OK(cudaDeviceSynchronize());
+    P2P_CUDA_OK(cudaMemcpy(out, h->trace_buf + t.off, (size_t)t.tiles * kTraceStamps * sizeof(unsigned long long),
+                           cudaMemcpyDeviceToHost));
+  }
+  return 0;
+}
+
+}
diff --git a/patch2pix_b200/csrc/umma_gemm.cu b/patch2pix_b200/csrc/umma_gemm.cu
--- a/patch2pix_b200/csrc/umma_gemm.cu
+++ b/patch2pix_b200/csrc/umma_gemm.cu
@@ -131,6 +131,127 @@
         e.c[(size_t)ca * e.np2 + cb] = best * e.alpha;
         e.code[(size_t)ca * e.np2 + cb] = (uint8_t)code;
       }
+    }
+  }
+}
+
+__device__ __forceinline__ void named_bar(int id, int threads) {
+  asm volatile("bar.sync %0, %1;" ::"r"(id), "r"(threads) : "memory");
+}
+
+constexpr int kFragBox = 64 * 128;
+
+template <int H>
+__device__ __forceinline__ void reduce_scatter_half(uint32_t* m, int lane) {
+  const bool up = (lane & (H / 2)) != 0;
+#pragma unroll
+  for (int i = 0; i < H; ++i) {
+    const uint32_t give = up ? m[i] : m[i + H], keep = up ? m[i + H] : m[i];
+    m[i] = max(keep, __shfl_xor_sync(0xffffffffu, give, H / 2));
+  }
+}
+
+__device__ __forceinline__ void conv2_frag(const UmmaEpilogue& e, const float* acc, int n, int n_units, int col0,
+                                           uint32_t* red, const float* sb, int wg) {
+  const int lane = threadIdx.x & 31, wl = (threadIdx.x >> 5) & 3, fc = 2 * (lane & 3);
+  uint32_t m[64];
+#pragma unroll
+  for (int j = 0; j < 32; ++j) {
+    const float2 s = *reinterpret_cast<const float2*>(sb + col0 + 8 * j + fc);
+    const float2 b = *reinterpret_cast<const float2*>(sb + 512 + col0 + 8 * j + fc);
+    m[2 * j] = max(__float_as_uint(fmaxf(fmaf(acc[4 * j], s.x, b.x), 0.f)),
+                   __float_as_uint(fmaxf(fmaf(acc[4 * j + 2], s.x, b.x), 0.f)));
+    m[2 * j + 1] = max(__float_as_uint(fmaxf(fmaf(acc[4 * j + 1], s.y, b.y), 0.f)),
+                       __float_as_uint(fmaxf(fmaf(acc[4 * j + 3], s.y, b.y), 0.f)));
+  }
+  reduce_scatter_half<32>(m, lane);
+  reduce_scatter_half<16>(m, lane);
+  reduce_scatter_half<8>(m, lane);
+  named_bar(1 + wg, 128);
+#pragma unroll
+  for (int i = 0; i < 8; i += 2)
+    *reinterpret_cast<uint2*>(red + wl * 256 + 32 * (lane >> 2) + 4 * i + fc) = make_uint2(m[i], m[i + 1]);
+  named_bar(1 + wg, 128);
+  if (n < n_units) {
+    const int t = threadIdx.x & 127;
+    uint2 v = *reinterpret_cast<const uint2*>(red + 2 * t);
+#pragma unroll
+    for (int w = 1; w < 4; ++w) {
+      const uint2 u = *reinterpret_cast<const uint2*>(red + w * 256 + 2 * t);
+      v.x = max(v.x, u.x);
+      v.y = max(v.y, u.y);
+    }
+    unsigned int* dst = reinterpret_cast<unsigned int*>(e.pooled) + (size_t)n * 512 + col0 + 2 * t;
+    atomicMax(dst, v.x);
+    atomicMax(dst + 1, v.y);
+  }
+}
+
+template <bool SHARE>
+__device__ __forceinline__ void conv1_frag(const UmmaGemmParams& p, float* acc, int n, int n_units, int split_slot,
+                                           int split_unit, int col0, uint8_t* buf) {
+  if (n >= n_units) return;
+  const int lane = threadIdx.x & 31, wl = (threadIdx.x >> 5) & 3, fc = 2 * (lane & 3), fr = 16 * wl + (lane >> 2);
+  const int wg = threadIdx.x / 128 - 1, t = threadIdx.x & 127;
+  const WindowShare& ws = p.ws;
+  if (SHARE && ws.part_out != nullptr) {
+    float* dst = ws.part_out + part_offset(n, 0, col0);
+#pragma unroll
+    for (int j = 0; j < 32; ++j)
+#pragma unroll
+      for (int h = 0; h < 2; ++h)
+        *reinterpret_cast<float2*>(dst + (fr + 8 * h) * 256 + 8 * j + fc) = make_float2(acc[4 * j + 2 * h], acc[4 * j + 2 * h + 1]);
+    return;
+  }
+  if (SHARE && ws.part_in != nullptr) {
+    const float* src = ws.part_in + part_offset(part_unit(n, split_slot, split_unit), 0, col0);
+#pragma unroll
+    for (int j0 = 0; j0 < 32; j0 += 8) {
+      float2 a[16];
+#pragma unroll
+      for (int i = 0; i < 16; ++i)
+        a[i] = __ldg(reinterpret_cast<const float2*>(src + (fr + 8 * (i & 1)) * 256 + 8 * (j0 + (i >> 1)) + fc));
+#pragma unroll
+      for (int i = 0; i < 16; ++i) {
+        acc[4 * (j0 + (i >> 1)) + 2 * (i & 1)] += a[i].x;
+        acc[4 * (j0 + (i >> 1)) + 2 * (i & 1) + 1] += a[i].y;
+      }
+    }
+  }
+  const int r = SHARE && ws.slot_row != nullptr ? __ldg(ws.slot_row + n) : n;
+  if (p.epi.pooled != nullptr)
+    *reinterpret_cast<float2*>(p.epi.pooled + (size_t)r * 512 + col0 + 2 * t) = make_float2(0.f, 0.f);
+  const float ys = p.epi.y_scale;
+  const uint32_t sbuf = smem_u32(buf);
+  const int mi = lane >> 3, rr = lane & 7;
+  const uint32_t arow = sbuf + (uint32_t)(16 * wl + 8 * (mi & 1) + rr) * 128;
+#pragma unroll
+  for (int hf = 0; hf < 2; ++hf) {
+    if (t == 0) bulk_wait_group_read<0>();
+    named_bar(1 + wg, 128);
+#pragma unroll
+    for (int j = 16 * hf; j < 16 * hf + 16; j += 2) {
+      uint32_t hv[4];
+#pragma unroll
+      for (int q = 0; q < 2; ++q) {
+        const float2 s = __ldg(reinterpret_cast<const float2*>(p.epi.scale + col0 + 8 * (j + q) + fc));
+        const float2 b = __ldg(reinterpret_cast<const float2*>(p.epi.bias + col0 + 8 * (j + q) + fc));
+        const float* d = acc + 4 * (j + q);
+#pragma unroll
+        for (int h = 0; h < 2; ++h) {
+          const __half2 y = __floats2half2_rn(fmaf(d[2 * h], s.x, b.x) * ys, fmaf(d[2 * h + 1], s.y, b.y) * ys);
+          hv[2 * q + h] = *reinterpret_cast<const uint32_t*>(&y);
+        }
+      }
+      const int jm = j + (mi >> 1);
+      stmatrix_x4(arow + (uint32_t)((jm >> 3) & 1) * kFragBox + (uint32_t)(((jm & 7) ^ rr) << 4), hv[0], hv[1], hv[2], hv[3]);
+    }
+    fence_proxy_async();
+    named_bar(1 + wg, 128);
+    if (t == 0) {
+      tma_store_3d(&p.y_store, buf, col0 + 128 * hf, 0, r);
+      tma_store_3d(&p.y_store, buf + kFragBox, col0 + 128 * hf + 64, 0, r);
+      bulk_commit_group();
     }
   }
 }
@@ -167,10 +288,6 @@
   return q < m ? q : m;
 }
 
-__device__ __forceinline__ void named_bar(int id, int threads) {
-  asm volatile("bar.sync %0, %1;" ::"r"(id), "r"(threads) : "memory");
-}
-
 __device__ __forceinline__ int window_origin(const WindowMaps& wm, int n, int j) {
   int v;
   if (wm.is_float) v = (int)reinterpret_cast<const float*>(wm.matches)[(size_t)n * 4 + j];
@@ -191,6 +308,9 @@
   using Cfg = GemmCfg<PASSES, SEGMENTED, AMODE>;
   constexpr int STAGES = Cfg::STAGES, NOP = Cfg::NOP, STAGE_BYTES = Cfg::STAGE_BYTES;
   constexpr int BN = Cfg::BN, B_BYTES = Cfg::B_BYTES, NACC = BN / 2;
+  constexpr bool FRAG = BN == 256 && (EPI == EPI_CONV1 || EPI == EPI_CONV2);
+  static_assert(2 * kFragBox * 2 <= 2 * kEpiBytes && 3 * 1024 * 4 <= 2 * kEpiBytes && (STAGES * STAGE_BYTES) % 1024 == 0,
+                "fragment epilogue buffers");
 
   extern __shared__ uint8_t smem_raw[];
   uint8_t* smem = reinterpret_cast<uint8_t*>((reinterpret_cast<uintptr_t>(smem_raw) + 1023) & ~(uintptr_t)1023);
@@ -231,6 +351,7 @@
       tma_prefetch_desc(&p.a_main_lo);
       tma_prefetch_desc(&p.b_lo);
     }
+    if (FRAG && EPI == EPI_CONV1 && p.frag_epi) tma_prefetch_desc(&p.y_store);
   }
   if (warp == 1 && lane == 0) {
     for (int i = 0; i < STAGES; ++i) {
@@ -255,6 +376,10 @@
         const int m_tile = tile / n_col_tiles, brow = (tile - m_tile * n_col_tiles) * BN;
         const int a4 = m_tile * p.a_units_per_tile;
         const int kofs = m_tile < split_tile ? 0 : p.ws.class_steps;
+        if (p.trace != nullptr) {
+          mbar_wait(&empty_bar[it % STAGES], ((uint32_t)(it / STAGES) & 1u) ^ 1u);
+          p.trace[(size_t)tile * kTraceStamps] = globaltimer();
+        }
         if (AMODE == AMODE_WINDOW && p.ws.part_in != nullptr) {
 #pragma unroll 1
           for (int pp = 0; pp < 2; ++pp)
@@ -335,6 +460,11 @@
     const bool leader = threadIdx.x % 128 == 0;
     uint64_t* ready = AMODE == AMODE_WINDOW ? ready_bar : full_bar;
     float* stg = epi_smem + wg * (64 * kEpiPitch);
+    if (FRAG && EPI == EPI_CONV2 && p.frag_epi) {
+      const int t = threadIdx.x - 128;
+      for (int i = t; i < 1024; i += 256) epi_smem[2048 + i] = i < 512 ? __ldg(p.epi.scale + i) : __ldg(p.epi.bias + i - 512);
+      named_bar(4, 256);
+    }
     float acc[NACC];
     float tot[SEGMENTED ? NACC : 1];
     int it = 0;
@@ -343,6 +473,12 @@
       if (SEGMENTED) {
 #pragma unroll
         for (int i = 0; i < NACC; ++i) tot[i] = 0.f;
+      }
+      unsigned long long* tr = p.trace != nullptr && threadIdx.x == 128 ? p.trace + (size_t)tile * kTraceStamps : nullptr;
+      if (p.trace != nullptr) {
+        if (tr != nullptr) tr[1] = globaltimer();
+        mbar_wait(&ready[it % STAGES], (uint32_t)(it / STAGES) & 1u);
+        if (tr != nullptr) tr[2] = globaltimer();
       }
       for (int ks = 0; ks < nsteps; ++ks, ++it) {
         const int s = it % STAGES;
@@ -382,40 +518,56 @@
         mbar_arrive_if(&empty_bar[(s + STAGES - 1) % STAGES], leader && prev_pending);
         mbar_arrive_if(&empty_bar[s], leader && seg_end);
       }
+      if (tr != nullptr) tr[3] = globaltimer();
       wgmma_wait<0>();
       wgmma_fence_regs<NACC>(acc);
+      if (tr != nullptr) tr[4] = globaltimer();
       mbar_arrive_if(&empty_bar[(it + STAGES - 1) % STAGES], leader);
       if (SEGMENTED) {
 #pragma unroll
         for (int i = 0; i < NACC; ++i) tot[i] += acc[i];
       }
-      const float* res = SEGMENTED ? tot : acc;
-      const int fr = 16 * wl + (lane >> 2), fc = 2 * (lane & 3);
-      const int er = (wl & 1) * 32 + lane, ec = (wl >> 1) * 32;
-#pragma unroll
-      for (int c64 = 0; c64 < BN / 64; ++c64) {
-        named_bar(1 + wg, 128);
-#pragma unroll
-        for (int j = 0; j < 8; ++j) {
-          const float* d = res + 4 * (c64 * 8 + j);
-          float* o = stg + fr * kEpiPitch + 8 * j + fc;
-          o[0] = d[0];
-          o[1] = d[1];
-          o[8 * kEpiPitch] = d[2];
-          o[8 * kEpiPitch + 1] = d[3];
-        }
-        named_bar(1 + wg, 128);
-        if (AMODE == AMODE_WINDOW && (p.ws.part_out != nullptr || p.ws.part_in != nullptr)) {
-          share_piece(p.ws, 2 * split_tile, split_unit, n_units, m_tile, wg * 64 + er, col0 + c64 * 64 + ec,
-                      stg + er * kEpiPitch + ec);
-          if (p.ws.part_out != nullptr) continue;
-        }
-        float v[32];
-#pragma unroll
-        for (int i = 0; i < 32; ++i) v[i] = stg[er * kEpiPitch + ec + i];
-        epilogue_piece<EPI, AMODE == AMODE_WINDOW>(p.epi, p.ws, n_units, m_tile, wg * 64 + er, col0 + c64 * 64 + ec, v);
-      }
-    }
+      if (FRAG && p.frag_epi) {
+        if (EPI == EPI_CONV2)
+          conv2_frag(p.epi, acc, m_tile * 2 + wg, n_units, col0, reinterpret_cast<uint32_t*>(epi_smem) + wg * 1024,
+                     epi_smem + 2 * 1024, wg);
+        else
+          conv1_frag<AMODE == AMODE_WINDOW>(p, acc, m_tile * 2 + wg, n_units, 2 * split_tile, split_unit, col0,
+                                            reinterpret_cast<uint8_t*>(epi_smem) + wg * 2 * kFragBox);
+      } else {
+        const float* res = SEGMENTED ? tot : acc;
+        const int fr = 16 * wl + (lane >> 2), fc = 2 * (lane & 3);
+        const int er = (wl & 1) * 32 + lane, ec = (wl >> 1) * 32;
+#pragma unroll
+        for (int c64 = 0; c64 < BN / 64; ++c64) {
+          named_bar(1 + wg, 128);
+#pragma unroll
+          for (int j = 0; j < 8; ++j) {
+            const float* d = res + 4 * (c64 * 8 + j);
+            float* o = stg + fr * kEpiPitch + 8 * j + fc;
+            o[0] = d[0];
+            o[1] = d[1];
+            o[8 * kEpiPitch] = d[2];
+            o[8 * kEpiPitch + 1] = d[3];
+          }
+          named_bar(1 + wg, 128);
+          if (AMODE == AMODE_WINDOW && (p.ws.part_out != nullptr || p.ws.part_in != nullptr)) {
+            share_piece(p.ws, 2 * split_tile, split_unit, n_units, m_tile, wg * 64 + er, col0 + c64 * 64 + ec,
+                        stg + er * kEpiPitch + ec);
+            if (p.ws.part_out != nullptr) continue;
+          }
+          float v[32];
+#pragma unroll
+          for (int i = 0; i < 32; ++i) v[i] = stg[er * kEpiPitch + ec + i];
+          epilogue_piece<EPI, AMODE == AMODE_WINDOW>(p.epi, p.ws, n_units, m_tile, wg * 64 + er, col0 + c64 * 64 + ec, v);
+        }
+      }
+      if (tr != nullptr) {
+        tr[5] = globaltimer();
+        tr[6] = blockIdx.x + 1;
+      }
+    }
+    if (FRAG && EPI == EPI_CONV1 && p.frag_epi && threadIdx.x % 128 == 0) bulk_wait_group<0>();
   } else if (AMODE == AMODE_GATHER) {
     if constexpr (Cfg::AUX_REGS < Cfg::LAUNCH_REGS) setmaxnreg_dec<Cfg::AUX_REGS>();
     const int ptid = threadIdx.x - 384;
@@ -774,6 +926,11 @@
   P2P_REQUIRE(passes == 1 || passes == 3, "umma gemm: passes must be 1 or 3");
   P2P_REQUIRE(p.nsteps > 0 && p.m_tiles > 0 && p.n_tiles > 0, "umma gemm: empty problem");
   const bool seg = p.seg_len > 0 && p.seg_len < p.nsteps;
+  if (p.frag_epi) {
+    P2P_REQUIRE((epi == EPI_CONV1 || epi == EPI_CONV2) && passes == 1 && !seg && amode != AMODE_GATHER,
+                "umma gemm: the fragment epilogues serve the 256-wide conv1 / conv2 launches only");
+    P2P_REQUIRE(epi == EPI_CONV2 || p.epi.y_lo == nullptr, "umma gemm: the fragment conv1 epilogue writes y_hi only");
+  }
   if (amode != AMODE_TMA) {
     P2P_REQUIRE(epi == EPI_CONV1 && passes == 1 && !seg, "the fused A operand is available for 1-pass conv1 only");
     if (amode == AMODE_GATHER) return launch_one<1, false, EPI_CONV1, AMODE_GATHER>(p, num_sms, st);
diff --git a/patch2pix_b200/csrc/umma_gemm.h b/patch2pix_b200/csrc/umma_gemm.h
--- a/patch2pix_b200/csrc/umma_gemm.h
+++ b/patch2pix_b200/csrc/umma_gemm.h
@@ -8,6 +8,7 @@
 enum { EPI_PLAIN = 0, EPI_CONV1 = 1, EPI_CONV2 = 2, EPI_CORR = 3, EPI_FC = 4 };
 enum { AMODE_TMA = 0, AMODE_GATHER = 1, AMODE_WINDOW = 2 };
 constexpr int kMaxKSteps = 96;
+constexpr int kTraceStamps = 8;
 
 struct UmmaEpilogue {
   float* c;
@@ -51,12 +52,15 @@
 
 struct UmmaGemmParams {
   CUtensorMap a_main_hi, a_main_lo, a_rgb_hi, a_rgb_lo, b_hi, b_lo;
+  CUtensorMap y_store;
   KStep steps[kMaxKSteps];
   int nsteps;
   int m_tiles;
   int n_tiles;
   int a_units_per_tile;
   int seg_len;
+  int frag_epi;
+  unsigned long long* trace;
   const int* d_units;
   UmmaEpilogue epi;
   FusedGather fg;
diff --git a/patch2pix_b200/csrc/umma_ptx.cuh b/patch2pix_b200/csrc/umma_ptx.cuh
--- a/patch2pix_b200/csrc/umma_ptx.cuh
+++ b/patch2pix_b200/csrc/umma_ptx.cuh
@@ -103,6 +103,20 @@
 __device__ __forceinline__ void bulk_wait_group_read() {
   asm volatile("cp.async.bulk.wait_group.read %0;" ::"n"(N) : "memory");
 }
+template <int N>
+__device__ __forceinline__ void bulk_wait_group() {
+  asm volatile("cp.async.bulk.wait_group %0;" ::"n"(N) : "memory");
+}
+__device__ __forceinline__ unsigned long long globaltimer() {
+  unsigned long long t;
+  asm volatile("mov.u64 %0, %%globaltimer;" : "=l"(t));
+  return t;
+}
+__device__ __forceinline__ void stmatrix_x4(uint32_t addr, uint32_t r0, uint32_t r1, uint32_t r2, uint32_t r3) {
+  asm volatile("stmatrix.sync.aligned.m8n8.x4.shared.b16 [%0], {%1, %2, %3, %4};" ::"r"(addr), "r"(r0), "r"(r1), "r"(r2),
+               "r"(r3)
+               : "memory");
+}
 
 __device__ __forceinline__ void wgmma_fence() { asm volatile("wgmma.fence.sync.aligned;" ::: "memory"); }
 __device__ __forceinline__ void wgmma_commit() { asm volatile("wgmma.commit_group.sync.aligned;" ::: "memory"); }
```

Result: faster. 100.9 (median of 6 runs) (+9.1%).
